# rmcar17/SpectralClusterSupertree

Measured on NVIDIA B200. Metric: construct_supertree wall-time at 10k taxa/1k trees, lower is better.
Workload: dtype f64

## Files before the change

include/scs_b200.h:

```cpp
#ifndef SCS_B200_H
#define SCS_B200_H

#include <stddef.h>
#include <stdint.h>

#ifdef __cplusplus
extern "C" {
#endif

typedef struct scs_ctx scs_ctx;

typedef enum {
    SCS_OK = 0,
    SCS_ERR_INVALID = -1,
    SCS_ERR_CUDA = -2,
    SCS_ERR_NO_DEVICE = -3,
    SCS_ERR_TOO_SMALL = -4,
    SCS_ERR_NO_CONVERGE = -5,
    SCS_ERR_INPUT = -6,
    SCS_ERR_EMPTY = -7,
    SCS_ERR_PEER = -8
} scs_status;

typedef struct {
    int32_t n_components;
    int32_t contracted_size;
    int32_t spectral_ran;
    int32_t solver;
    int32_t matvecs;
    int32_t restarts;
    int32_t tie_flag;
    int32_t kmeans_stable_splits;
    double eig[3];
    double residual;
    double margin;
    double kmeans_runner_up;
} scs_node_stats;

int scs_version(void);
const char *scs_status_string(int status);
const char *scs_last_error(const scs_ctx *ctx);
int scs_ctx_create(int device, void *stream, scs_ctx **out);
int scs_ctx_destroy(scs_ctx *ctx);
int scs_ctx_synchronize(scs_ctx *ctx);
int64_t scs_ctx_launch_count(const scs_ctx *ctx);

int scs_ctx_io_bytes(const scs_ctx *ctx, int64_t *h2d, int64_t *d2h);
int scs_ctx_timer_start(scs_ctx *ctx);
int scs_ctx_timer_stop(scs_ctx *ctx, double *ms);
int scs_ctx_set_small_node_limit(scs_ctx *ctx, int limit);
int scs_ctx_set_medium_node_limit(scs_ctx *ctx, int limit);
int scs_ctx_set_device_forest(scs_ctx *ctx, int on);
int scs_ctx_set_wide_entries(scs_ctx *ctx, int on);
int scs_ctx_set_full_rows(scs_ctx *ctx, int on);
int scs_ctx_stage_seconds(scs_ctx *ctx, double *seconds8, int reset);
int scs_ctx_flush_l2(scs_ctx *ctx);
int scs_ctx_profile_enable(scs_ctx *ctx, int on);
int scs_ctx_profile_read(scs_ctx *ctx, int kind, int64_t *launches, double *ms, double *bytes, double *units);

int scs_debug_small_cycles(scs_ctx *ctx, uint64_t *cycles2, int reset);
int scs_profiler_range(int on);

int scs_bit_words(int n);
int scs_pcg_build_dev(scs_ctx *ctx, int n, int T, int64_t L, const int64_t *leaf_offsets_dev,
                      const int32_t *leaf_taxon_dev, const int32_t *adj_depth_dev,
                      const double *adj_val_dev, const int32_t *root_depth_dev,
                      const double *tree_weight_dev, double *W_dev, int32_t *C_dev,
                      int32_t *occ_dev, uint32_t *adj_bits_dev, uint32_t *max_bits_dev,
                      double *degree_dev);

int scs_pcg_build_rows_dev(scs_ctx *ctx, int n, int T, int64_t L, const int64_t *leaf_offsets_dev,
                           const int32_t *leaf_taxon_dev, const int32_t *adj_depth_dev, const double *adj_val_dev,
                           const int32_t *root_depth_dev, const double *tree_weight_dev, int row0, int row1,
                           double *W_rows_dev, int32_t *occ_dev, uint32_t *adj_bits_dev, uint32_t *max_bits_dev,
                           double *degree_dev);

int scs_components_dev(scs_ctx *ctx, int n, const uint32_t *bits_dev, int32_t *label_dev,
                       int32_t *n_components_host);

int scs_contract_dev(scs_ctx *ctx, int n, const double *W_dev, const uint32_t *adj_bits_dev,
                     const uint32_t *max_bits_dev, int32_t *group_dev, int32_t *m_host,
                     double *Wc_dev, double *degree_c_dev);

int scs_spectral_bipartition_dev(scs_ctx *ctx, int m, const double *W_dev, const double *degree_dev,
                                 uint64_t seed, int32_t *side_dev, scs_node_stats *stats_host);

int scs_normalized_matvec_dev(scs_ctx *ctx, int m, const double *W_dev,
                              const double *inv_sqrt_deg_dev, const double *x_dev, double *y_dev);

int scs_node_split_host(scs_ctx *ctx, int n, int T, int64_t L, const int64_t *leaf_offsets,
                        const int32_t *leaf_taxon, const int32_t *adj_depth, const double *adj_val,
                        const int32_t *root_depth, const double *tree_weight, int contract_edges,
                        uint64_t seed, int32_t *part, scs_node_stats *stats);
int scs_node_split_dev(scs_ctx *ctx, int n, int T, int64_t L, const int64_t *leaf_offsets_dev,
                       const int32_t *leaf_taxon_dev, const int32_t *adj_depth_dev,
                       const double *adj_val_dev, const int32_t *root_depth_dev,
                       const double *tree_weight_dev, int contract_edges, uint64_t seed,
                       int32_t *part_dev, scs_node_stats *stats_host);

int scs_node_last_buffers(scs_ctx *ctx, int *n, int *m, double **W_dev, uint32_t **adj_bits_dev,
                          uint32_t **max_bits_dev, int32_t **occ_dev, double **degree_dev,
                          double **Wc_dev, int32_t **group_dev);

int scs_dev_alloc(scs_ctx *ctx, size_t bytes, void **out);
int scs_dev_free(scs_ctx *ctx, void *ptr);
int scs_memcpy_h2d(scs_ctx *ctx, void *dev, const void *host, size_t bytes);
int scs_memcpy_d2h(scs_ctx *ctx, void *host, const void *dev, size_t bytes);

typedef struct scs_forest scs_forest;
int scs_set_host_threads(int threads);
int scs_forest_create(int T, const int64_t *node_offsets, const int32_t *parent, const double *length,
                      const double *support, const int32_t *taxon, const double *tree_weight,
                      int num_taxa, scs_forest **out);
int scs_forest_create_view(int T, const int64_t *node_offsets, const int32_t *parent, const double *length,
                           const double *support, const int32_t *taxon, const double *tree_weight, int num_taxa,
                           scs_forest **out);
const char *scs_forest_last_error(void);
int scs_forest_destroy(scs_forest *f);
int scs_forest_parse_newick(const char *text, size_t bytes, scs_forest **out, char **names, size_t *names_bytes,
                            int *num_taxa);
const char *scs_newick_last_error(void);
int scs_flat_tree_newick(int64_t num_nodes, const int32_t *parent, const int32_t *taxon, const char *names,
                         size_t names_bytes, int num_taxa, char **text, size_t *text_bytes);
int scs_flat_tree_newick_values(int64_t num_nodes, const int32_t *parent, const int32_t *taxon, const char *names,
                                size_t names_bytes, int num_taxa, const double *value, int digits, char **text,
                                size_t *text_bytes);
void scs_free(void *ptr);
int scs_forest_num_trees(const scs_forest *f);
int64_t scs_forest_num_nodes(const scs_forest *f);
int64_t scs_forest_num_leaves(const scs_forest *f);
int scs_forest_num_taxa(const scs_forest *f);
int64_t scs_forest_pair_visits(const scs_forest *f);
int scs_forest_tree_info(const scs_forest *f, int t, int64_t *num_nodes, double *weight, int32_t *source);
int scs_forest_tree(const scs_forest *f, int t, int32_t *parent, double *length, double *support,
                    int32_t *taxon);
int scs_forest_taxa(const scs_forest *f, uint8_t *present);
int scs_forest_induce(const scs_forest *f, const uint8_t *keep, scs_forest **out);
int scs_forest_induce_parts(const scs_forest *f, const int32_t *part, int count, scs_forest **out,
                            uint8_t *present);
int scs_forest_tours(const scs_forest *f, int weighting, const int32_t *local_id, int64_t *leaf_offsets,
                     int32_t *leaf_taxon, int32_t *adj_depth, double *adj_val, int32_t *root_depth,
                     double *tree_weight);
int scs_forest_split(scs_ctx *ctx, const scs_forest *f, int weighting, int contract_edges, uint64_t seed,
                     int32_t *n_out, int32_t *taxa_out, int32_t *part_out, scs_node_stats *stats);

typedef struct {
    int32_t n;
    int32_t num_trees;
    int64_t leaf_base;
    int64_t tree_base;
    int64_t vertex_base;
} scs_small_node;
int scs_nodes_split_small_host(scs_ctx *ctx, int num_nodes, const scs_small_node *nodes, int64_t L_total,
                               int64_t T_total, const int64_t *leaf_offsets, const int32_t *leaf_taxon,
                               const int32_t *adj_depth, const double *adj_val, const int32_t *root_depth,
                               const double *tree_weight, int contract_edges, int32_t *part,
                               scs_node_stats *stats);

int scs_nodes_split_small_dev(scs_ctx *ctx, int num_nodes, const scs_small_node *nodes_dev,
                              const int64_t *leaf_offsets_dev, const int32_t *leaf_taxon_dev,
                              const int32_t *adj_depth_dev, const double *adj_val_dev,
                              const int32_t *root_depth_dev, const double *tree_weight_dev,
                              int contract_edges, int32_t *part_dev, scs_node_stats *stats_dev);

int scs_nodes_split_medium_dev(scs_ctx *ctx, int num_nodes, const int32_t *node_n, const int32_t *tree_begin,
                               const int64_t *part_offset, const uint64_t *seeds, int T, int64_t L,
                               const int64_t *leaf_offsets_dev, const int32_t *leaf_taxon_dev, const int32_t *adj_depth_dev,
                               const double *adj_val_dev, const int32_t *root_depth_dev, const double *tree_weight_dev,
                               int contract_edges, int32_t *part_dev, scs_node_stats *stats, uint8_t *needs_rerun);

typedef struct scs_supertree scs_supertree;
int scs_supertree_build(scs_ctx *ctx, const scs_forest *forest, int weighting, int contract_edges,
                        uint64_t seed, int record_nodes, scs_supertree **out);
int scs_supertree_build_sharded(scs_ctx *ctx, const scs_forest *forest, int weighting, int contract_edges,
                                uint64_t seed, int record_nodes, int rank, int world, scs_supertree **out);
typedef struct scs_device_forest scs_device_forest;
int scs_device_forest_create(scs_ctx *ctx, const scs_forest *forest, int weighting, scs_device_forest **out);
int scs_device_forest_destroy(scs_device_forest *forest);
int64_t scs_device_forest_bytes(const scs_device_forest *forest);
int scs_supertree_build_resident(scs_ctx *ctx, const scs_device_forest *forest, int contract_edges, uint64_t seed,
                                 int record_nodes, int rank, int world, scs_supertree **out);
int64_t scs_supertree_shared_prefix(const scs_supertree *tree);
int64_t scs_supertree_shared_records(const scs_supertree *tree);
int scs_supertree_wave_info(const scs_supertree *tree, int32_t *tasks, int32_t *max_n);
int scs_supertree_wave_seconds(const scs_supertree *tree, double *seconds3);
int scs_supertree_destroy(scs_supertree *tree);
int64_t scs_supertree_num_nodes(const scs_supertree *tree);
int scs_supertree_nodes(const scs_supertree *tree, int32_t *parent, int32_t *taxon);
int scs_supertree_counters(const scs_supertree *tree, int64_t *nodes_small, int64_t *nodes_large,
                           int64_t *waves, int64_t *pair_visits);
int scs_supertree_seconds(const scs_supertree *tree, double *seconds4);
int scs_supertree_medium_info(const scs_supertree *tree, int64_t *nodes_medium, int64_t *nodes_rerun, double *seconds);
int64_t scs_supertree_num_records(const scs_supertree *tree);
int scs_supertree_record_size(const scs_supertree *tree, int64_t index);
int scs_supertree_record_wave(const scs_supertree *tree, int64_t index);
int scs_supertree_record(const scs_supertree *tree, int64_t index, int32_t *taxa, int32_t *part,
                         scs_node_stats *stats);

int scs_supertree_support(scs_ctx *ctx, const scs_forest *sources, int64_t num_nodes, const int32_t *parent,
                          const int32_t *taxon, int32_t *counts, double *weighted, int32_t *per_tree);

int scs_supertree_triplets(scs_ctx *ctx, const scs_forest *sources, int64_t num_nodes, const int32_t *parent,
                           const int32_t *taxon, int64_t *per_tree);

int scs_supertree_taxon_triplets(scs_ctx *ctx, const scs_forest *sources, int64_t num_nodes, const int32_t *parent,
                                 const int32_t *taxon, int64_t *per_taxon, double *weighted);

#define SCS_IPC_HANDLE_BYTES 64
int scs_shard_create(scs_ctx *ctx, int rank, int world, int n_max, unsigned char *handle_out);
int scs_shard_connect_ipc(scs_ctx *ctx, const unsigned char *handles );
int scs_shard_window(scs_ctx *ctx, void **window_dev, size_t *bytes);
int scs_shard_connect_ptrs(scs_ctx *ctx, void *const *windows );
int scs_shard_engage(scs_ctx *ctx, int on);
int scs_shard_configure(scs_ctx *ctx, int min_n, double timeout_seconds);
int scs_shard_barrier(scs_ctx *ctx);
int64_t scs_shard_nodes(const scs_ctx *ctx);
int scs_shard_destroy(scs_ctx *ctx);

#ifdef __cplusplus
}
#endif
#endif
```

spectralclustersupertree_b200/_lib.py:

```python

from __future__ import annotations

import ctypes
import os
from ctypes import POINTER, c_char_p, c_double, c_int, c_int32, c_int64, c_size_t, c_uint8, c_uint64, c_void_p
from pathlib import Path

LIB_PATH = Path(__file__).resolve().parent / "libscs_b200.so"

SCS_OK = 0
SCS_ERR_INVALID = -1
SCS_ERR_CUDA = -2
SCS_ERR_NO_DEVICE = -3
SCS_ERR_TOO_SMALL = -4
SCS_ERR_NO_CONVERGE = -5
SCS_ERR_INPUT = -6
SCS_ERR_EMPTY = -7
SCS_ERR_PEER = -8
IPC_HANDLE_BYTES = 64


class NodeStats(ctypes.Structure):

    _fields_ = [
        ("n_components", c_int32),
        ("contracted_size", c_int32),
        ("spectral_ran", c_int32),
        ("solver", c_int32),
        ("matvecs", c_int32),
        ("restarts", c_int32),
        ("tie_flag", c_int32),
        ("kmeans_stable_splits", c_int32),
        ("eig", c_double * 3),
        ("residual", c_double),
        ("margin", c_double),
        ("kmeans_runner_up", c_double),
    ]

    def as_dict(self) -> dict:
        return {
            "n_components": self.n_components,
            "contracted_size": self.contracted_size,
            "spectral_ran": bool(self.spectral_ran),
            "solver": self.solver,
            "matvecs": self.matvecs,
            "restarts": self.restarts,
            "tie_flag": self.tie_flag,
            "eig": [self.eig[0], self.eig[1], self.eig[2]],
            "residual": self.residual,
            "margin": self.margin,
            "kmeans_stable_splits": self.kmeans_stable_splits,
            "kmeans_runner_up": self.kmeans_runner_up,
        }


class LibraryMissingError(RuntimeError):
    """``libscs_b200.so`` is not built: the CUDA path is the only path."""


_P = c_void_p

SIGNATURES: dict[str, tuple] = {
    "scs_version": (c_int, []),
    "scs_status_string": (c_char_p, [c_int]),
    "scs_last_error": (c_char_p, [_P]),
    "scs_ctx_create": (c_int, [c_int, _P, POINTER(_P)]),
    "scs_ctx_destroy": (c_int, [_P]),
    "scs_ctx_synchronize": (c_int, [_P]),
    "scs_ctx_launch_count": (c_int64, [_P]),
    "scs_ctx_io_bytes": (c_int, [_P, POINTER(c_int64), POINTER(c_int64)]),
    "scs_ctx_timer_start": (c_int, [_P]),
    "scs_ctx_timer_stop": (c_int, [_P, POINTER(c_double)]),
    "scs_ctx_set_small_node_limit": (c_int, [_P, c_int]),
    "scs_ctx_set_medium_node_limit": (c_int, [_P, c_int]),
    "scs_ctx_set_device_forest": (c_int, [_P, c_int]),
    "scs_ctx_set_wide_entries": (c_int, [_P, c_int]),
    "scs_ctx_set_full_rows": (c_int, [_P, c_int]),
    "scs_ctx_stage_seconds": (c_int, [_P, _P, c_int]),
    "scs_ctx_flush_l2": (c_int, [_P]),
    "scs_ctx_profile_enable": (c_int, [_P, c_int]),
    "scs_ctx_profile_read": (c_int, [_P, c_int, POINTER(c_int64), POINTER(c_double), POINTER(c_double), POINTER(c_double)]),
    "scs_bit_words": (c_int, [c_int]),
    "scs_pcg_build_dev": (c_int, [_P, c_int, c_int, c_int64] + [_P] * 12),
    "scs_pcg_build_rows_dev": (c_int, [_P, c_int, c_int, c_int64, _P, _P, _P, _P, _P, _P, c_int, c_int, _P, _P, _P, _P, _P]),
    "scs_components_dev": (c_int, [_P, c_int, _P, _P, POINTER(c_int32)]),
    "scs_contract_dev": (c_int, [_P, c_int, _P, _P, _P, _P, POINTER(c_int32), _P, _P]),
    "scs_spectral_bipartition_dev": (c_int, [_P, c_int, _P, _P, c_uint64, _P, POINTER(NodeStats)]),
    "scs_normalized_matvec_dev": (c_int, [_P, c_int, _P, _P, _P, _P]),
    "scs_node_split_host": (
        c_int,
        [_P, c_int, c_int, c_int64, _P, _P, _P, _P, _P, _P, c_int, c_uint64, _P, POINTER(NodeStats)],
    ),
    "scs_node_split_dev": (
        c_int,
        [_P, c_int, c_int, c_int64, _P, _P, _P, _P, _P, _P, c_int, c_uint64, _P, POINTER(NodeStats)],
    ),
    "scs_node_last_buffers": (c_int, [_P, POINTER(c_int), POINTER(c_int)] + [POINTER(_P)] * 7),
    "scs_dev_alloc": (c_int, [_P, c_size_t, POINTER(_P)]),
    "scs_dev_free": (c_int, [_P, _P]),
    "scs_memcpy_h2d": (c_int, [_P, _P, _P, c_size_t]),
    "scs_memcpy_d2h": (c_int, [_P, _P, _P, c_size_t]),
    "scs_set_host_threads": (c_int, [c_int]),
    "scs_forest_create": (c_int, [c_int, _P, _P, _P, _P, _P, _P, c_int, POINTER(_P)]),
    "scs_forest_create_view": (c_int, [c_int, _P, _P, _P, _P, _P, _P, c_int, POINTER(_P)]),
    "scs_forest_destroy": (c_int, [_P]),
    "scs_forest_parse_newick": (c_int, [c_char_p, c_size_t, POINTER(_P), POINTER(_P), POINTER(c_size_t), POINTER(c_int)]),
    "scs_newick_last_error": (c_char_p, []),
    "scs_forest_last_error": (c_char_p, []),
    "scs_flat_tree_newick": (c_int, [c_int64, _P, _P, c_char_p, c_size_t, c_int, POINTER(_P), POINTER(c_size_t)]),
    "scs_flat_tree_newick_values": (
        c_int,
        [c_int64, _P, _P, c_char_p, c_size_t, c_int, _P, c_int, POINTER(_P), POINTER(c_size_t)],
    ),
    "scs_supertree_support": (c_int, [_P, _P, c_int64, _P, _P, _P, _P, _P]),
    "scs_supertree_triplets": (c_int, [_P, _P, c_int64, _P, _P, _P]),
    "scs_supertree_taxon_triplets": (c_int, [_P, _P, c_int64, _P, _P, _P, _P]),
    "scs_profiler_range": (c_int, [c_int]),
    "scs_debug_small_cycles": (c_int, [_P, _P, c_int]),
    "scs_free": (None, [_P]),
    "scs_forest_num_trees": (c_int, [_P]),
    "scs_forest_num_nodes": (c_int64, [_P]),
    "scs_forest_num_leaves": (c_int64, [_P]),
    "scs_forest_num_taxa": (c_int, [_P]),
    "scs_forest_pair_visits": (c_int64, [_P]),
    "scs_forest_tree_info": (c_int, [_P, c_int, POINTER(c_int64), POINTER(c_double), POINTER(c_int32)]),
    "scs_forest_tree": (c_int, [_P, c_int, _P, _P, _P, _P]),
    "scs_forest_taxa": (c_int, [_P, _P]),
    "scs_forest_induce": (c_int, [_P, _P, POINTER(_P)]),
    "scs_forest_induce_parts": (c_int, [_P, _P, c_int, _P, _P]),
    "scs_forest_tours": (c_int, [_P, c_int, _P, _P, _P, _P, _P, _P, _P]),
    "scs_forest_split": (
        c_int,
        [_P, _P, c_int, c_int, c_uint64, POINTER(c_int32), _P, _P, POINTER(NodeStats)],
    ),
    "scs_nodes_split_small_host": (
        c_int,
        [_P, c_int, _P, c_int64, c_int64, _P, _P, _P, _P, _P, _P, c_int, _P, _P],
    ),
    "scs_nodes_split_small_dev": (c_int, [_P, c_int, _P, _P, _P, _P, _P, _P, _P, c_int, _P, _P]),
    "scs_supertree_build": (c_int, [_P, _P, c_int, c_int, c_uint64, c_int, POINTER(_P)]),
    "scs_supertree_build_sharded": (c_int, [_P, _P, c_int, c_int, c_uint64, c_int, c_int, c_int, POINTER(_P)]),
    "scs_supertree_shared_prefix": (c_int64, [_P]),
    "scs_supertree_shared_records": (c_int64, [_P]),
    "scs_supertree_wave_info": (c_int, [_P, _P, _P]),
    "scs_supertree_wave_seconds": (c_int, [_P, _P]),
    "scs_supertree_destroy": (c_int, [_P]),
    "scs_supertree_num_nodes": (c_int64, [_P]),
    "scs_supertree_nodes": (c_int, [_P, _P, _P]),
    "scs_supertree_counters": (c_int, [_P, POINTER(c_int64), POINTER(c_int64), POINTER(c_int64), POINTER(c_int64)]),
    "scs_device_forest_create": (c_int, [_P, _P, c_int, POINTER(_P)]),
    "scs_device_forest_destroy": (c_int, [_P]),
    "scs_device_forest_bytes": (c_int64, [_P]),
    "scs_supertree_build_resident": (c_int, [_P, _P, c_int, c_uint64, c_int, c_int, c_int, POINTER(_P)]),
    "scs_supertree_record_wave": (c_int, [_P, c_int64]),
    "scs_nodes_split_medium_dev": (c_int, [_P, c_int, _P, _P, _P, _P, c_int, c_int64, _P, _P, _P, _P, _P, _P, c_int, _P, _P, _P]),
    "scs_supertree_medium_info": (c_int, [_P, POINTER(c_int64), POINTER(c_int64), POINTER(ctypes.c_double)]),
    "scs_supertree_seconds": (c_int, [_P, _P]),
    "scs_supertree_num_records": (c_int64, [_P]),
    "scs_supertree_record_size": (c_int, [_P, c_int64]),
    "scs_supertree_record": (c_int, [_P, c_int64, _P, _P, POINTER(NodeStats)]),
    "scs_shard_create": (c_int, [_P, c_int, c_int, c_int, _P]),
    "scs_shard_connect_ipc": (c_int, [_P, _P]),
    "scs_shard_window": (c_int, [_P, POINTER(_P), POINTER(c_size_t)]),
    "scs_shard_connect_ptrs": (c_int, [_P, _P]),
    "scs_shard_engage": (c_int, [_P, c_int]),
    "scs_shard_configure": (c_int, [_P, c_int, c_double]),
    "scs_shard_barrier": (c_int, [_P]),
    "scs_shard_nodes": (c_int64, [_P]),
    "scs_shard_destroy": (c_int, [_P]),
}

_LIB: ctypes.CDLL | None = None


def load() -> ctypes.CDLL:
    global _LIB
    if _LIB is not None:
        return _LIB
    if not LIB_PATH.is_file():
        msg = (
            f"{LIB_PATH} is missing: build it with `python -m spectralclustersupertree_b200.build` "
            "(there is no CPU fallback for the CUDA path)"
        )
        raise LibraryMissingError(msg)
    os.environ.setdefault("CUDA_MODULE_LOADING", "EAGER")
    os.environ.setdefault("OMP_WAIT_POLICY", "passive")
    lib = ctypes.CDLL(str(LIB_PATH))
    for name, (restype, argtypes) in SIGNATURES.items():
        fn = getattr(lib, name)
        fn.restype = restype
        fn.argtypes = argtypes
    _LIB = lib
    return lib


def ptr(array) -> int | None:
    if array is None:
        return None
    if not array.flags["C_CONTIGUOUS"]:
        msg = "array must be C-contiguous"
        raise ValueError(msg)
    return array.ctypes.data


__all__ = ["LIB_PATH", "SIGNATURES", "LibraryMissingError", "NodeStats", "c_uint8", "load", "ptr"]
```

spectralclustersupertree_b200/csrc/common.cuh:

```cuda
#pragma once

#include <cuda_runtime.h>

#include <cstdint>
#include <cstdio>
#include <cstring>
#include <string>
#include <vector>

#include "scs_b200.h"

namespace scs {

constexpr int kMediumMaxDefault = 4096;

struct DeviceBuffer {
    void *ptr = nullptr;
    size_t bytes = 0;
};

enum Slot : int {
    SLOT_TOUR_OFFSETS = 0,
    SLOT_TOUR_TAXON,
    SLOT_TOUR_DEPTH,
    SLOT_TOUR_VAL,
    SLOT_TOUR_ROOT,
    SLOT_TOUR_WEIGHT,
    SLOT_W,
    SLOT_WC,
    SLOT_OCC,
    SLOT_ADJ_BITS,
    SLOT_MAX_BITS,
    SLOT_DEGREE,
    SLOT_DEGREE_C,
    SLOT_LEAF_TREE,
    SLOT_ROW_PTR,
    SLOT_CURSOR,
    SLOT_INV,
    SLOT_INV_SORTED,
    SLOT_DEGREE_PART,
    SLOT_LINKS,
    SLOT_BUCKET_COUNT,
    SLOT_START16,
    SLOT_BUCKET_PTR,
    SLOT_ENTRIES,
    SLOT_UF_PARENT,
    SLOT_LABEL,
    SLOT_LABEL2,
    SLOT_GROUP,
    SLOT_GROUP_PTR,
    SLOT_GROUP_MEMBERS,
    SLOT_SCALARS,
    SLOT_PART,
    SLOT_ISD,
    SLOT_UVEC,
    SLOT_BASIS,
    SLOT_WORK,
    SLOT_COEF,
    SLOT_TRIDIAG,
    SLOT_RITZ,
    SLOT_EMBED,
    SLOT_SORTED,
    SLOT_SIDE,
    SLOT_SPEC_SCALARS,
    SLOT_L2_FLUSH,
    SLOT_NODE_STATS,
    SLOT_MED_NODES,
    SLOT_MED_ROW_NODE,
    SLOT_MED_TREE_NODE,
    SLOT_MED_STATE,
    SLOT_MED_VEC,
    SLOT_MED_SMALL,
    SLOT_MED_STAGE,
    SLOT_SCAN_SUMS,
    SLOT_COUNT
};

constexpr int kMaxPeers = 16;

struct ShardLayout {
    size_t vec[2] = {0, 0};
    size_t degree = 0, degree_c = 0;
    size_t adj_bits = 0, max_bits = 0;
    size_t W = 0;
    size_t total = 0;
};

struct ShardState {
    bool connected = false;
    bool engaged = false;
    int rank = 0, world = 1;
    int n_max = 0;
    int min_n = 4096;
    unsigned long long epoch = 0;
    int parity = 0;
    double timeout_s = 20.0;
    unsigned char *window = nullptr;
    unsigned char *peer[kMaxPeers] = {};
    bool opened[kMaxPeers] = {};
    ShardLayout layout;
    int64_t nodes = 0;
};

struct RowBlock {
    int row0 = 0, row1 = -1;
    bool half_window = false;
    bool sharded() const { return row1 >= 0; }
};

struct MedNode {
    int32_t n, words;
    int32_t row_base;
    int32_t tree_begin, tree_end;
    int32_t jcap;
    int32_t blk_base, pad0;
    int64_t w_off;
    int64_t bit_off;
    int64_t basis_off;
    int64_t part_off;
    uint64_t seed;
};

inline int shard_rows_per_rank(int n, int world) { return (n + world - 1) / world; }
inline RowBlock shard_block(int n, int rank, int world) {
    const int per = shard_rows_per_rank(n, world);
    RowBlock b;
    b.row0 = rank * per < n ? rank * per : n;
    b.row1 = b.row0 + per < n ? b.row0 + per : n;
    return b;
}

}

struct scs_ctx {
    int device = 0;
    cudaStream_t stream = nullptr;
    bool own_stream = false;
    int sm_count = 148;
    size_t smem_optin = 0;
    size_t smem_per_sm = 0;
    int64_t launches = 0;
    std::string last_error;
    scs::DeviceBuffer slots[scs::SLOT_COUNT];
    void *pinned = nullptr;
    size_t pinned_bytes = 0;
    void *pinned_io = nullptr;
    size_t pinned_io_bytes = 0;
    int64_t h2d_bytes = 0;
    int64_t d2h_bytes = 0;
    bool profile_on = false;
    struct ProfileRecord {
        cudaEvent_t start, stop;
        int kind;
        double bytes, units;
    };
    std::vector<ProfileRecord> profile;
    int flush_value = 0;
    double stage_seconds[8] = {0, 0, 0, 0, 0, 0, 0, 0};
    std::vector<scs_ctx *> workers;
    bool small_configured = false;
    bool batch_configured = false;
    bool tail_configured = false;
    bool rows_configured[32] = {};
    bool mirror_configured = false;
    bool contract_configured = false;
    bool kmeans_configured = false;
    bool medium_configured = false;
    bool device_forest = true;
    int medium_limit = scs::kMediumMaxDefault;
    bool wide_entries = false;
    bool full_rows = false;
    int small_limit = 32;
    double pending_units = 0.0;
    cudaEvent_t timer_start = nullptr, timer_stop = nullptr;
    int last_n = 0;
    int last_m = 0;
    scs::ShardState shard;
    void *driver_cache = nullptr;
    void (*driver_cache_release)(scs_ctx *, void *) = nullptr;
};

namespace scs {

int fail(scs_ctx *ctx, int status, const char *what, cudaError_t err = cudaSuccess);

#define SCS_CUDA(ctx, call)                                                   \
    do {                                                                      \
        cudaError_t err__ = (call);                                           \
        if (err__ != cudaSuccess) return scs::fail(ctx, SCS_ERR_CUDA, #call, err__); \
    } while (0)

#define SCS_LAUNCHED(ctx, name)                                               \
    do {                                                                      \
        cudaError_t err__ = cudaGetLastError();                               \
        if (err__ != cudaSuccess) return scs::fail(ctx, SCS_ERR_CUDA, name, err__); \
        (ctx)->launches += 1;                                                 \
    } while (0)

int reserve(scs_ctx *ctx, Slot slot, size_t bytes, void **out);

template <typename T>
inline int reserve_as(scs_ctx *ctx, Slot slot, size_t count, T **out) {
    void *p = nullptr;
    int rc = reserve(ctx, slot, count * sizeof(T), &p);
    *out = static_cast<T *>(p);
    return rc;
}

int reserve_pinned(scs_ctx *ctx, size_t bytes, void **out);

enum ProfileKind : int { PROFILE_MATVEC = 0, PROFILE_PCG_ROWS = 1, PROFILE_KINDS = 2 };
constexpr int kSmallNode = 64;
constexpr int kSmallMaxTrees = 65535;
constexpr int kProfileMinSize = 4096;

void profile_begin(scs_ctx *ctx, int kind, double bytes, double units);
void profile_end(scs_ctx *ctx);

inline int ceil_div(int64_t a, int64_t b) { return static_cast<int>((a + b - 1) / b); }

int exclusive_scan(scs_ctx *ctx, int n, const int32_t *in, int32_t *out);

#ifdef __CUDACC__
__device__ __forceinline__ unsigned long long order_key(double x) {
    const unsigned long long sign = 0x8000000000000000ull;
    unsigned long long b = static_cast<unsigned long long>(__double_as_longlong(x));
    return (b & sign) ? ~b : (b | sign);
}
__device__ __forceinline__ double order_value(unsigned long long k) {
    const unsigned long long sign = 0x8000000000000000ull;
    unsigned long long b = (k & sign) ? (k & ~sign) : ~k;
    return __longlong_as_double(static_cast<long long>(b));
}
#endif

int prewarm_node(scs_ctx *ctx, int n, int T, int64_t L);

int ensure_workers(scs_ctx *ctx, int count);

int pcg_build(scs_ctx *ctx, int n, int T, int64_t L, const int64_t *leaf_offsets,
              const int32_t *leaf_taxon, const int32_t *adj_depth, const double *adj_val,
              const int32_t *root_depth, const double *tree_weight, double *W, int32_t *C,
              int32_t *occ, uint32_t *adj_bits, uint32_t *max_bits, double *degree, RowBlock rows = RowBlock());

int pcg_fetch_transposed(scs_ctx *ctx, int n, RowBlock rows, int rows_per_rank, int world, const double *const *peer_W,
                         double *W_block);
int pcg_symmetrize_bits(scs_ctx *ctx, int n, uint32_t *adj_bits, uint32_t *max_bits);
int pcg_degree_block(scs_ctx *ctx, int n, int T, RowBlock rows, const double *W_block, double *degree);

int components(scs_ctx *ctx, int n, const uint32_t *bits, int32_t *label, int32_t *n_components_host);

int components_async(scs_ctx *ctx, int n, const uint32_t *bits, int32_t *label, int32_t *count_dev);

int tour_components_async(scs_ctx *ctx, int n, int T, int64_t L, const int64_t *leaf_offsets,
                          const int32_t *leaf_taxon, const int32_t *adj_depth, const int32_t *root_depth,
                          int32_t *label, int32_t *count_dev, int32_t *bad_dev);

int contract(scs_ctx *ctx, int n, const double *W, const uint32_t *adj_bits, const uint32_t *max_bits,
             int32_t *group, int32_t *m_host, double *Wc, double *degree_c);
int contract_with_labels(scs_ctx *ctx, int n, const double *W, const uint32_t *adj_bits, const int32_t *label, int m,
                         int32_t *group, double *Wc, double *degree_c, RowBlock rows = RowBlock());

int spectral_bipartition(scs_ctx *ctx, int m, const double *W, const double *degree, uint64_t seed,
                         int32_t *side, scs_node_stats *stats_host, RowBlock rows = RowBlock());

int normalized_matvec(scs_ctx *ctx, int m, const double *W, const double *isd, const double *x, double *y);

int pcg_build_batch(scs_ctx *ctx, int B, int blocks, int R, int T, int64_t L, int max_n, int max_trees, const MedNode *nodes_dev,
                    const int32_t *tree_node, const int32_t *row_node, const int64_t *leaf_offsets,
                    const int32_t *leaf_taxon, const int32_t *adj_depth, const double *adj_val,
                    const int32_t *root_depth, const double *tree_weight, double *W, int32_t *occ, uint32_t *adj_bits,
                    uint32_t *max_bits, double *degree, int32_t *bad_dev);

constexpr int kMediumMax = kMediumMaxDefault;

int medium_batch(scs_ctx *ctx, int B, const int32_t *node_n, const int32_t *tree_begin, const int32_t *tree_end,
                 const int64_t *part_off, const uint64_t *seeds, int T, int64_t L, const int64_t *leaf_offsets, const int32_t *leaf_taxon,
                 const int32_t *adj_depth, const double *adj_val, const int32_t *root_depth, const double *tree_weight,
                 int contract_edges, int32_t *part_dev, scs_node_stats *stats_host, uint8_t *needs_rerun);

int small_node(scs_ctx *ctx, int n, int contract_edges, const double *W, const uint32_t *adj_bits,
               const uint32_t *max_bits, int32_t *part, scs_node_stats *out_dev, int32_t *group_out,
               double *Wc_out);

int small_batch(scs_ctx *ctx, int num_nodes, const scs_small_node *nodes_dev, const int64_t *leaf_offsets,
                const int32_t *leaf_taxon, const int32_t *adj_depth, const double *adj_val, const int32_t *root_depth,
                const double *tree_weight, int contract_edges, int32_t *part_dev, scs_node_stats *stats_dev,
                int32_t *bad_dev, int absolute_offsets = 0);

int small_cycles(scs_ctx *ctx, unsigned long long *out2, int reset);

int node_split(scs_ctx *ctx, int n, int T, int64_t L, const int64_t *leaf_offsets, const int32_t *leaf_taxon,
               const int32_t *adj_depth, const double *adj_val, const int32_t *root_depth,
               const double *tree_weight, int contract_edges, uint64_t seed, int32_t *part_dev,
               int32_t *part_host, scs_node_stats *stats, bool tour_components = false);

int node_split_host(scs_ctx *ctx, int n, int T, int64_t L, const int64_t *leaf_offsets, const int32_t *leaf_taxon,
                    const int32_t *adj_depth, const double *adj_val, const int32_t *root_depth,
                    const double *tree_weight, int contract_edges, uint64_t seed, int32_t *part,
                    scs_node_stats *stats_out, bool tour_components);

bool shard_applies(const scs_ctx *ctx, int n);
int shard_barrier(scs_ctx *ctx);
int shard_push(scs_ctx *ctx, size_t offset, size_t bytes);
struct ShardMatvecTicket {
    unsigned long long epoch;
    size_t vec_offset;
    unsigned long long timeout_ns;
};
ShardMatvecTicket shard_next_matvec(scs_ctx *ctx);
int node_split_sharded(scs_ctx *ctx, int n, int T, int64_t L, const int64_t *leaf_offsets, const int32_t *leaf_taxon,
                       const int32_t *adj_depth, const double *adj_val, const int32_t *root_depth,
                       const double *tree_weight, int contract_edges, uint64_t seed, int32_t *part_dev,
                       int32_t *part_host, scs_node_stats *stats);

}
```

spectralclustersupertree_b200/csrc/context.cu:

```cuda

#include "common.cuh"

#include <chrono>
#include <cmath>

#include <cuda_profiler_api.h>

namespace scs {

int fail(scs_ctx *ctx, int status, const char *what, cudaError_t err) {
    if (ctx) {
        ctx->last_error = what ? what : "";
        if (err != cudaSuccess) {
            ctx->last_error += ": ";
            ctx->last_error += cudaGetErrorString(err);
        }
    }
    return status;
}

int reserve(scs_ctx *ctx, Slot slot, size_t bytes, void **out) {
    DeviceBuffer &buf = ctx->slots[slot];
    if (bytes == 0) bytes = 16;
    if (buf.bytes < bytes) {
        const size_t want = bytes + bytes / 4 + 256;
        if (buf.ptr) {
            SCS_CUDA(ctx, cudaFreeAsync(buf.ptr, ctx->stream));
            buf.ptr = nullptr;
            buf.bytes = 0;
        }
        cudaError_t err = cudaMallocAsync(&buf.ptr, want, ctx->stream);
        if (err != cudaSuccess) {
            buf.ptr = nullptr;
            return fail(ctx, SCS_ERR_CUDA, "cudaMallocAsync (workspace)", err);
        }
        buf.bytes = want;
    }
    *out = buf.ptr;
    return SCS_OK;
}

int reserve_pinned(scs_ctx *ctx, size_t bytes, void **out) {
    if (ctx->pinned_bytes < bytes) {
        if (ctx->pinned) {
            SCS_CUDA(ctx, cudaStreamSynchronize(ctx->stream));
            SCS_CUDA(ctx, cudaFreeHost(ctx->pinned));
            ctx->pinned = nullptr;
            ctx->pinned_bytes = 0;
        }
        size_t want = bytes < 4096 ? 4096 : 2 * bytes;
        SCS_CUDA(ctx, cudaMallocHost(&ctx->pinned, want));
        ctx->pinned_bytes = want;
    }
    *out = ctx->pinned;
    return SCS_OK;
}

int ensure_workers(scs_ctx *ctx, int count) {
    while (static_cast<int>(ctx->workers.size()) < count - 1) {
        scs_ctx *worker = nullptr;
        const int rc = scs_ctx_create(ctx->device, nullptr, &worker);
        if (rc) return fail(ctx, rc, "creating a worker context");
        worker->small_limit = ctx->small_limit;
        ctx->workers.push_back(worker);
    }
    for (scs_ctx *worker : ctx->workers) {
        worker->small_limit = ctx->small_limit;
        worker->full_rows = ctx->full_rows;
        worker->wide_entries = ctx->wide_entries;
    }
    return SCS_OK;
}

void profile_begin(scs_ctx *ctx, int kind, double bytes, double units) {
    if (!ctx->profile_on) return;
    scs_ctx::ProfileRecord rec;
    rec.kind = kind;
    rec.bytes = bytes;
    rec.units = units;
    if (cudaEventCreate(&rec.start) != cudaSuccess || cudaEventCreate(&rec.stop) != cudaSuccess) return;
    cudaEventRecord(rec.start, ctx->stream);
    ctx->profile.push_back(rec);
}

void profile_end(scs_ctx *ctx) {
    if (!ctx->profile_on || ctx->profile.empty()) return;
    cudaEventRecord(ctx->profile.back().stop, ctx->stream);
}

namespace {

struct DeviceGuard {
    int previous = -1;
    explicit DeviceGuard(int device) {
        cudaGetDevice(&previous);
        if (previous != device) cudaSetDevice(device);
    }
};

template <typename T>
int upload(scs_ctx *ctx, Slot slot, const T *host, size_t count, T **dev) {
    int rc = reserve_as(ctx, slot, count + 1, dev);
    if (rc) return rc;
    if (count) SCS_CUDA(ctx, cudaMemcpyAsync(*dev, host, count * sizeof(T), cudaMemcpyHostToDevice, ctx->stream));
    return SCS_OK;
}

__global__ void relabel_components(int n, const int32_t *__restrict__ label, const int32_t *__restrict__ rank,
                                   int32_t *__restrict__ part) {
    int v = blockIdx.x * blockDim.x + threadIdx.x;
    if (v < n) part[v] = rank[label[v]];
}

__global__ void mark_roots(int n, const int32_t *__restrict__ label, int32_t *__restrict__ flag) {
    int v = blockIdx.x * blockDim.x + threadIdx.x;
    if (v < n) flag[v] = label[v] == v;
}

__global__ void expand_sides(int n, const int32_t *__restrict__ group, const int32_t *__restrict__ side,
                             int32_t *__restrict__ part) {
    int v = blockIdx.x * blockDim.x + threadIdx.x;
    if (v < n) part[v] = side[group ? group[v] : v];
}

void clear_stats(scs_node_stats *s) {
    std::memset(s, 0, sizeof(*s));
    s->eig[0] = 0.0;
    s->eig[1] = s->eig[2] = std::nan("");
    s->residual = std::nan("");
    s->margin = std::nan("");
}

}

int node_split(scs_ctx *ctx, int n, int T, int64_t L, const int64_t *leaf_offsets, const int32_t *leaf_taxon,
               const int32_t *adj_depth, const double *adj_val, const int32_t *root_depth,
               const double *tree_weight, int contract_edges, uint64_t seed, int32_t *part_dev,
               int32_t *part_host, scs_node_stats *stats, bool tour_components) {
    auto number_components = [&](const int32_t *label) -> int {
        int32_t *flag, *rank;
        int rc;
        if ((rc = reserve_as(ctx, SLOT_GROUP_PTR, 4 * static_cast<size_t>(n) + 8, &flag))) return rc;
        rank = flag + n;
        const int blocks = ceil_div(n, 256);
        mark_roots<<<blocks, 256, 0, ctx->stream>>>(n, label, flag);
        SCS_LAUNCHED(ctx, "mark_roots");
        if ((rc = exclusive_scan(ctx, n, flag, rank))) return rc;
        relabel_components<<<blocks, 256, 0, ctx->stream>>>(n, label, rank, part_dev);
        SCS_LAUNCHED(ctx, "relabel_components");
        if (part_host) {
            SCS_CUDA(ctx, cudaMemcpyAsync(part_host, part_dev, sizeof(int32_t) * n, cudaMemcpyDeviceToHost, ctx->stream));
            ctx->d2h_bytes += static_cast<int64_t>(sizeof(int32_t)) * n;
            SCS_CUDA(ctx, cudaStreamSynchronize(ctx->stream));
        }
        return SCS_OK;
    };
    if (tour_components && n > ctx->small_limit) {
        const auto t0 = std::chrono::steady_clock::now();
        int32_t *label, *scalars;
        void *pin_v;
        int rc;
        if ((rc = reserve_as(ctx, SLOT_LABEL, static_cast<size_t>(n), &label))) return rc;
        if ((rc = reserve_as(ctx, SLOT_SCALARS, 64, &scalars))) return rc;
        if ((rc = reserve_pinned(ctx, 512, &pin_v))) return rc;
        SCS_CUDA(ctx, cudaMemsetAsync(scalars, 0, 16 * sizeof(int32_t), ctx->stream));
        if ((rc = tour_components_async(ctx, n, T, L, leaf_offsets, leaf_taxon, adj_depth, root_depth, label,
                                        scalars + 8, scalars)))
            return rc;
        int32_t *host_scalars = reinterpret_cast<int32_t *>(static_cast<unsigned char *>(pin_v) + 256);
        SCS_CUDA(ctx, cudaMemcpyAsync(host_scalars, scalars, 16 * sizeof(int32_t), cudaMemcpyDeviceToHost, ctx->stream));
        SCS_CUDA(ctx, cudaStreamSynchronize(ctx->stream));
        ctx->stage_seconds[6] += std::chrono::duration<double>(std::chrono::steady_clock::now() - t0).count();
        if (host_scalars[0] != 0) return fail(ctx, SCS_ERR_INPUT, "leaf tour: taxon id out of range");
        if (host_scalars[8] != 1) {
            stats->n_components = host_scalars[8];
            stats->contracted_size = n;
            return number_components(label);
        }
    }
    if (shard_applies(ctx, n))
        return node_split_sharded(ctx, n, T, L, leaf_offsets, leaf_taxon, adj_depth, adj_val, root_depth, tree_weight,
                                  contract_edges, seed, part_dev, part_host, stats);
    const int words = scs_bit_words(n);
    const size_t nn = static_cast<size_t>(n) * n;
    double *W, *Wc, *degree, *degree_c;
    int32_t *occ, *label, *group, *side, *scalars;
    uint32_t *adj_bits, *max_bits;
    int rc;
    if ((rc = reserve_as(ctx, SLOT_W, nn, &W))) return rc;
    if ((rc = reserve_as(ctx, SLOT_OCC, static_cast<size_t>(n), &occ))) return rc;
    if ((rc = reserve_as(ctx, SLOT_ADJ_BITS, static_cast<size_t>(n) * words, &adj_bits))) return rc;
    if ((rc = reserve_as(ctx, SLOT_MAX_BITS, static_cast<size_t>(n) * words, &max_bits))) return rc;
    if ((rc = reserve_as(ctx, SLOT_DEGREE, static_cast<size_t>(n), &degree))) return rc;
    if ((rc = reserve_as(ctx, SLOT_LABEL, static_cast<size_t>(n), &label))) return rc;
    if ((rc = reserve_as(ctx, SLOT_SCALARS, 64, &scalars))) return rc;
    ctx->last_n = n;
    ctx->last_m = 0;
    void *pin_v;
    if ((rc = reserve_pinned(ctx, 512, &pin_v))) return rc;
    unsigned char *pin = static_cast<unsigned char *>(pin_v);
    auto fetch_part = [&]() -> int {
        if (part_host) {
            SCS_CUDA(ctx, cudaMemcpyAsync(part_host, part_dev, sizeof(int32_t) * n, cudaMemcpyDeviceToHost, ctx->stream));
            ctx->d2h_bytes += static_cast<int64_t>(sizeof(int32_t)) * n;
        }
        return SCS_OK;
    };

    auto now = [] { return std::chrono::steady_clock::now(); };
    auto lap = [&](int slot, std::chrono::steady_clock::time_point &since) {
        const auto t = now();
        ctx->stage_seconds[slot] += std::chrono::duration<double>(t - since).count();
        since = t;
    };
    auto mark = now();
    if ((rc = pcg_build(ctx, n, T, L, leaf_offsets, leaf_taxon, adj_depth, adj_val, root_depth, tree_weight, W,
                        nullptr, occ, adj_bits, contract_edges ? max_bits : nullptr, degree)))
        return rc;

    if (n <= ctx->small_limit) {
        scs_node_stats *stats_dev;
        if ((rc = reserve_as(ctx, SLOT_NODE_STATS, 1, &stats_dev))) return rc;
        if ((rc = reserve_as(ctx, SLOT_WC, nn, &Wc))) return rc;
        if ((rc = reserve_as(ctx, SLOT_GROUP, static_cast<size_t>(n), &group))) return rc;
        if ((rc = small_node(ctx, n, contract_edges, W, adj_bits, max_bits, part_dev, stats_dev, group, Wc))) return rc;
        SCS_CUDA(ctx, cudaMemcpyAsync(pin, stats_dev, sizeof(scs_node_stats), cudaMemcpyDeviceToHost, ctx->stream));
        SCS_CUDA(ctx, cudaMemcpyAsync(pin + 256, scalars, sizeof(int32_t), cudaMemcpyDeviceToHost, ctx->stream));
        if ((rc = fetch_part())) return rc;
        SCS_CUDA(ctx, cudaStreamSynchronize(ctx->stream));
        if (*reinterpret_cast<int32_t *>(pin + 256) != 0)
            return fail(ctx, SCS_ERR_INPUT, "leaf tour: taxon id out of range");
        std::memcpy(stats, pin, sizeof(scs_node_stats));
        ctx->last_m = stats->contracted_size;
        if (stats->solver == -1) {
            stats->solver = 0;
            return fail(ctx, SCS_ERR_TOO_SMALL, "spectral step on a graph contracted to one vertex");
        }
        return SCS_OK;
    }

    int32_t *label2 = nullptr;
    if ((rc = components_async(ctx, n, adj_bits, label, scalars + 8))) return rc;
    if (contract_edges) {
        if ((rc = reserve_as(ctx, SLOT_LABEL2, static_cast<size_t>(n), &label2))) return rc;
        if ((rc = components_async(ctx, n, max_bits, label2, scalars + 9))) return rc;
    }
    SCS_CUDA(ctx, cudaMemcpyAsync(pin + 256, scalars, 16 * sizeof(int32_t), cudaMemcpyDeviceToHost, ctx->stream));
    lap(0, mark);
    SCS_CUDA(ctx, cudaStreamSynchronize(ctx->stream));
    lap(1, mark);
    const int32_t *host_scalars = reinterpret_cast<const int32_t *>(pin + 256);
    if (host_scalars[0] != 0) return fail(ctx, SCS_ERR_INPUT, "leaf tour: taxon id out of range");
    const int ncomp = host_scalars[8];
    stats->n_components = ncomp;
    stats->contracted_size = n;
    const int blocks = ceil_div(n, 256);

    if (ncomp != 1) return number_components(label);

    int m = n;
    const double *Wm = W;
    const double *deg_m = degree;
    const int32_t *group_m = nullptr;
    if (contract_edges) {
        m = host_scalars[9];
        if ((rc = reserve_as(ctx, SLOT_WC, nn, &Wc))) return rc;
        if ((rc = reserve_as(ctx, SLOT_DEGREE_C, static_cast<size_t>(n), &degree_c))) return rc;
        if ((rc = reserve_as(ctx, SLOT_GROUP, static_cast<size_t>(n), &group))) return rc;
        if ((rc = contract_with_labels(ctx, n, W, adj_bits, label2, m, group, Wc, degree_c))) return rc;
        if (m != n) {
            Wm = Wc;
            deg_m = degree_c;
            group_m = group;
        }
    }
    ctx->last_m = m;
    stats->contracted_size = m;
    stats->spectral_ran = 1;
    if ((rc = reserve_as(ctx, SLOT_SIDE, static_cast<size_t>(n), &side))) return rc;
    if (m < 2) {
        return fail(ctx, SCS_ERR_TOO_SMALL, "spectral step on a graph contracted to one vertex");
    }
    lap(2, mark);
    if ((rc = spectral_bipartition(ctx, m, Wm, deg_m, seed, side, stats))) return rc;
    lap(3, mark);
    expand_sides<<<blocks, 256, 0, ctx->stream>>>(n, group_m, side, part_dev);
    SCS_LAUNCHED(ctx, "expand_sides");
    if ((rc = fetch_part())) return rc;
    if (part_host) SCS_CUDA(ctx, cudaStreamSynchronize(ctx->stream));
    lap(4, mark);
    return SCS_OK;
}

}

using namespace scs;

namespace scs {
int prewarm_node(scs_ctx *ctx, int n, int T, int64_t L) {
    DeviceGuard guard(ctx->device);
    const size_t nT = static_cast<size_t>(T), nL = static_cast<size_t>(L), nn = static_cast<size_t>(n) * n;
    const size_t total = (nT + 1) * sizeof(int64_t) + nL * (sizeof(double) + 2 * sizeof(int32_t)) +
                         nT * (sizeof(double) + sizeof(int32_t)) + 64;
    if (ctx->pinned_io_bytes < total) {
        if (ctx->pinned_io) {
            SCS_CUDA(ctx, cudaStreamSynchronize(ctx->stream));
            SCS_CUDA(ctx, cudaFreeHost(ctx->pinned_io));
            ctx->pinned_io = nullptr;
            ctx->pinned_io_bytes = 0;
        }
        const size_t want = 2 * total + 4096;
        SCS_CUDA(ctx, cudaMallocHost(&ctx->pinned_io, want));
        ctx->pinned_io_bytes = want;
    }
    const size_t words = static_cast<size_t>(scs_bit_words(n));
    const size_t basis = static_cast<size_t>((n - 1 < 256 ? n - 1 : 256) + 3) * n;
    void *p;
    int rc;
    if ((rc = reserve(ctx, SLOT_TOUR_OFFSETS, total, &p))) return rc;
    if ((rc = reserve(ctx, SLOT_W, 8 * nn, &p))) return rc;
    if ((rc = reserve(ctx, SLOT_WC, 8 * nn, &p))) return rc;
    if ((rc = reserve(ctx, SLOT_ADJ_BITS, 4 * n * words, &p))) return rc;
    if ((rc = reserve(ctx, SLOT_MAX_BITS, 4 * n * words, &p))) return rc;
    if ((rc = reserve(ctx, SLOT_BASIS, 8 * basis, &p))) return rc;
    if ((rc = reserve(ctx, SLOT_LINKS, 16 * (nL + 1), &p))) return rc;
    if ((rc = reserve(ctx, SLOT_ENTRIES, 8 * (nL + 1), &p))) return rc;
    if ((rc = reserve(ctx, SLOT_BUCKET_COUNT, 448 * (nL + 1), &p))) return rc;
    if ((rc = reserve(ctx, SLOT_START16, 64 * (nL + 1), &p))) return rc;
    return SCS_OK;
}
}

namespace scs {
int node_split_host(scs_ctx *ctx, int n, int T, int64_t L, const int64_t *leaf_offsets, const int32_t *leaf_taxon,
                    const int32_t *adj_depth, const double *adj_val, const int32_t *root_depth,
                    const double *tree_weight, int contract_edges, uint64_t seed, int32_t *part,
                    scs_node_stats *stats_out, bool tour_components) {
    if (!ctx) return SCS_ERR_INVALID;
    if (n <= 0 || T < 0 || L < 0 || !part) return fail(ctx, SCS_ERR_INVALID, "node_split: bad argument");
    if (T > 0 && (!leaf_offsets || !root_depth || !tree_weight))
        return fail(ctx, SCS_ERR_INVALID, "node_split: null tour array");
    if (L > 0 && (!leaf_taxon || !adj_depth || !adj_val))
        return fail(ctx, SCS_ERR_INVALID, "node_split: null tour array");
    DeviceGuard guard(ctx->device);
    scs_node_stats local;
    scs_node_stats *stats = stats_out ? stats_out : &local;
    clear_stats(stats);

    const size_t nT = static_cast<size_t>(T), nL = static_cast<size_t>(L);
    const size_t b_off = (nT + 1) * sizeof(int64_t);
    const size_t b_val = nL * sizeof(double);
    const size_t b_w = nT * sizeof(double);
    const size_t b_tax = nL * sizeof(int32_t);
    const size_t b_dep = nL * sizeof(int32_t);
    const size_t b_root = nT * sizeof(int32_t);
    const size_t total = b_off + b_val + b_w + b_tax + b_dep + b_root + 64;
    int rc;
    if (ctx->pinned_io_bytes < total) {
        if (ctx->pinned_io) {
            SCS_CUDA(ctx, cudaStreamSynchronize(ctx->stream));
            SCS_CUDA(ctx, cudaFreeHost(ctx->pinned_io));
            ctx->pinned_io = nullptr;
            ctx->pinned_io_bytes = 0;
        }
        const size_t want = 2 * total + 4096;
        SCS_CUDA(ctx, cudaMallocHost(&ctx->pinned_io, want));
        ctx->pinned_io_bytes = want;
    }
    unsigned char *stage = static_cast<unsigned char *>(ctx->pinned_io);
    unsigned char *dev_stage;
    if ((rc = reserve_as(ctx, SLOT_TOUR_OFFSETS, total, &dev_stage))) return rc;
    size_t o_off = 0, o_val = o_off + b_off, o_w = o_val + b_val, o_tax = o_w + b_w, o_dep = o_tax + b_tax,
           o_root = o_dep + b_dep;
    if (T > 0) {
        std::memcpy(stage + o_off, leaf_offsets, b_off);
        std::memcpy(stage + o_w, tree_weight, b_w);
        std::memcpy(stage + o_root, root_depth, b_root);
    } else {
        std::memset(stage + o_off, 0, b_off);
    }
    if (L > 0) {
        std::memcpy(stage + o_val, adj_val, b_val);
        std::memcpy(stage + o_tax, leaf_taxon, b_tax);
        std::memcpy(stage + o_dep, adj_depth, b_dep);
    }
    SCS_CUDA(ctx, cudaMemcpyAsync(dev_stage, stage, total - 64, cudaMemcpyHostToDevice, ctx->stream));
    ctx->h2d_bytes += static_cast<int64_t>(total - 64);
    ctx->pending_units = 0.0;
    for (int t = 0; t < T; ++t) {
        const double k = static_cast<double>(leaf_offsets[t + 1] - leaf_offsets[t]);
        ctx->pending_units += k * (k - 1.0);
    }

    int32_t *part_dev;
    if ((rc = reserve_as(ctx, SLOT_PART, static_cast<size_t>(n), &part_dev))) return rc;
    rc = node_split(ctx, n, T, L, reinterpret_cast<const int64_t *>(dev_stage + o_off),
                    reinterpret_cast<const int32_t *>(dev_stage + o_tax),
                    reinterpret_cast<const int32_t *>(dev_stage + o_dep),
                    reinterpret_cast<const double *>(dev_stage + o_val),
                    reinterpret_cast<const int32_t *>(dev_stage + o_root),
                    reinterpret_cast<const double *>(dev_stage + o_w), contract_edges, seed, part_dev, part, stats,
                    tour_components);
    ctx->pending_units = 0.0;
    return rc;
}
}

extern "C" {

int scs_version(void) { return 100; }

const char *scs_status_string(int status) {
    switch (status) {
    case SCS_OK: return "ok";
    case SCS_ERR_INVALID: return "invalid argument";
    case SCS_ERR_CUDA: return "CUDA error";
    case SCS_ERR_NO_DEVICE: return "no usable CUDA device";
    case SCS_ERR_TOO_SMALL: return "fewer than two vertices in the spectral step";
    case SCS_ERR_NO_CONVERGE: return "eigensolver did not converge";
    case SCS_ERR_INPUT: return "malformed input";
    case SCS_ERR_EMPTY: return "there must be at least one tree to make a supertree";
    case SCS_ERR_PEER: return "a wait for a peer GPU timed out";
    default: return "unknown status";
    }
}

const char *scs_last_error(const scs_ctx *ctx) { return ctx ? ctx->last_error.c_str() : ""; }

int scs_bit_words(int n) { return (n + 31) / 32; }

int scs_ctx_create(int device, void *stream, scs_ctx **out) {
    if (!out) return SCS_ERR_INVALID;
    *out = nullptr;
    int count = 0;
    if (cudaGetDeviceCount(&count) != cudaSuccess || count <= 0) {
        cudaGetLastError();
        return SCS_ERR_NO_DEVICE;
    }
    if (device < 0 || device >= count) return SCS_ERR_INVALID;
    if (cudaSetDevice(device) != cudaSuccess) return SCS_ERR_CUDA;
    scs_ctx *ctx = new scs_ctx();
    ctx->device = device;
    cudaDeviceProp prop;
    if (cudaGetDeviceProperties(&prop, device) != cudaSuccess) {
        delete ctx;
        return SCS_ERR_CUDA;
    }
    {
        cudaMemPool_t pool;
        if (cudaDeviceGetDefaultMemPool(&pool, device) == cudaSuccess) {
            uint64_t threshold = ~0ull;
            cudaMemPoolSetAttribute(pool, cudaMemPoolAttrReleaseThreshold, &threshold);
        }
        cudaGetLastError();
    }
    ctx->sm_count = prop.multiProcessorCount;
    ctx->smem_optin = prop.sharedMemPerBlockOptin;
    ctx->smem_per_sm = prop.sharedMemPerMultiprocessor;
    if (stream) {
        ctx->stream = static_cast<cudaStream_t>(stream);
    } else {
        if (cudaStreamCreateWithFlags(&ctx->stream, cudaStreamNonBlocking) != cudaSuccess) {
            delete ctx;
            return SCS_ERR_CUDA;
        }
        ctx->own_stream = true;
    }
    *out = ctx;
    return SCS_OK;
}

int scs_ctx_destroy(scs_ctx *ctx) {
    if (!ctx) return SCS_OK;
    DeviceGuard guard(ctx->device);
    for (scs_ctx *worker : ctx->workers) scs_ctx_destroy(worker);
    ctx->workers.clear();
    cudaStreamSynchronize(ctx->stream);
    if (ctx->driver_cache && ctx->driver_cache_release) ctx->driver_cache_release(ctx, ctx->driver_cache);
    ctx->driver_cache = nullptr;
    scs_shard_destroy(ctx);
    for (auto &buf : ctx->slots)
        if (buf.ptr) cudaFreeAsync(buf.ptr, ctx->stream);
    cudaStreamSynchronize(ctx->stream);
    if (ctx->pinned) cudaFreeHost(ctx->pinned);
    if (ctx->pinned_io) cudaFreeHost(ctx->pinned_io);
    for (auto &rec : ctx->profile) {
        cudaEventDestroy(rec.start);
        cudaEventDestroy(rec.stop);
    }
    if (ctx->timer_start) cudaEventDestroy(ctx->timer_start);
    if (ctx->timer_stop) cudaEventDestroy(ctx->timer_stop);
    if (ctx->own_stream) cudaStreamDestroy(ctx->stream);
    delete ctx;
    return SCS_OK;
}

int scs_ctx_synchronize(scs_ctx *ctx) {
    if (!ctx) return SCS_ERR_INVALID;
    DeviceGuard guard(ctx->device);
    SCS_CUDA(ctx, cudaStreamSynchronize(ctx->stream));
    return SCS_OK;
}

int64_t scs_ctx_launch_count(const scs_ctx *ctx) { return ctx ? ctx->launches : 0; }

int scs_ctx_io_bytes(const scs_ctx *ctx, int64_t *h2d, int64_t *d2h) {
    if (!ctx) return SCS_ERR_INVALID;
    if (h2d) *h2d = ctx->h2d_bytes;
    if (d2h) *d2h = ctx->d2h_bytes;
    return SCS_OK;
}

int scs_ctx_timer_start(scs_ctx *ctx) {
    if (!ctx) return SCS_ERR_INVALID;
    DeviceGuard guard(ctx->device);
    if (!ctx->timer_start) {
        SCS_CUDA(ctx, cudaEventCreate(&ctx->timer_start));
        SCS_CUDA(ctx, cudaEventCreate(&ctx->timer_stop));
    }
    SCS_CUDA(ctx, cudaEventRecord(ctx->timer_start, ctx->stream));
    return SCS_OK;
}

int scs_ctx_timer_stop(scs_ctx *ctx, double *ms) {
    if (!ctx || !ms || !ctx->timer_start) return SCS_ERR_INVALID;
    DeviceGuard guard(ctx->device);
    SCS_CUDA(ctx, cudaEventRecord(ctx->timer_stop, ctx->stream));
    SCS_CUDA(ctx, cudaEventSynchronize(ctx->timer_stop));
    float t = 0.0f;
    SCS_CUDA(ctx, cudaEventElapsedTime(&t, ctx->timer_start, ctx->timer_stop));
    *ms = t;
    return SCS_OK;
}

int scs_ctx_set_small_node_limit(scs_ctx *ctx, int limit) {
    if (!ctx || limit < 0) return SCS_ERR_INVALID;
    ctx->small_limit = limit > kSmallNode ? kSmallNode : limit;
    return SCS_OK;
}

int scs_ctx_set_medium_node_limit(scs_ctx *ctx, int limit) {
    if (!ctx || limit < 0) return SCS_ERR_INVALID;
    ctx->medium_limit = limit > kMediumMax ? kMediumMax : limit;
    return SCS_OK;
}

int scs_ctx_set_device_forest(scs_ctx *ctx, int on) {
    if (!ctx) return SCS_ERR_INVALID;
    ctx->device_forest = on != 0;
    return SCS_OK;
}

int scs_ctx_set_wide_entries(scs_ctx *ctx, int on) {
    if (!ctx) return SCS_ERR_INVALID;
    ctx->wide_entries = on != 0;
    return SCS_OK;
}

int scs_ctx_set_full_rows(scs_ctx *ctx, int on) {
    if (!ctx) return SCS_ERR_INVALID;
    ctx->full_rows = on != 0;
    for (scs_ctx *worker : ctx->workers) worker->full_rows = ctx->full_rows;
    return SCS_OK;
}

int scs_ctx_stage_seconds(scs_ctx *ctx, double *seconds8, int reset) {
    if (!ctx || !seconds8) return SCS_ERR_INVALID;
    for (int i = 0; i < 8; ++i) {
        seconds8[i] = ctx->stage_seconds[i];
        if (reset) ctx->stage_seconds[i] = 0.0;
    }
    return SCS_OK;
}

int scs_ctx_flush_l2(scs_ctx *ctx) {
    if (!ctx) return SCS_ERR_INVALID;
    DeviceGuard guard(ctx->device);
    const size_t bytes = 256u << 20;
    void *buf;
    int rc = reserve(ctx, SLOT_L2_FLUSH, bytes, &buf);
    if (rc) return rc;
    ctx->flush_value += 1;
    SCS_CUDA(ctx, cudaMemsetAsync(buf, ctx->flush_value & 0xff, bytes, ctx->stream));
    SCS_CUDA(ctx, cudaStreamSynchronize(ctx->stream));
    return SCS_OK;
}

int scs_ctx_profile_enable(scs_ctx *ctx, int on) {
    if (!ctx) return SCS_ERR_INVALID;
    ctx->profile_on = on != 0;
    return SCS_OK;
}

int scs_ctx_profile_read(scs_ctx *ctx, int kind, int64_t *launches, double *ms, double *bytes, double *units) {
    if (!ctx || kind < 0 || kind >= PROFILE_KINDS) return SCS_ERR_INVALID;
    DeviceGuard guard(ctx->device);
    SCS_CUDA(ctx, cudaStreamSynchronize(ctx->stream));
    int64_t count = 0;
    double total_ms = 0.0, total_bytes = 0.0, total_units = 0.0;
    std::vector<scs_ctx::ProfileRecord> keep;
    for (auto &rec : ctx->profile) {
        if (rec.kind != kind) {
            keep.push_back(rec);
            continue;
        }
        float t = 0.0f;
        if (cudaEventElapsedTime(&t, rec.start, rec.stop) == cudaSuccess) {
            count += 1;
            total_ms += t;
            total_bytes += rec.bytes;
            total_units += rec.units;
        }
        cudaEventDestroy(rec.start);
        cudaEventDestroy(rec.stop);
    }
    cudaGetLastError();
    ctx->profile.swap(keep);
    if (launches) *launches = count;
    if (ms) *ms = total_ms;
    if (bytes) *bytes = total_bytes;
    if (units) *units = total_units;
    return SCS_OK;
}

int scs_debug_small_cycles(scs_ctx *ctx, uint64_t *cycles2, int reset) {
    if (!ctx || !cycles2) return SCS_ERR_INVALID;
    DeviceGuard guard(ctx->device);
    unsigned long long raw[2] = {0, 0};
    const int rc = small_cycles(ctx, raw, reset);
    cycles2[0] = raw[0];
    cycles2[1] = raw[1];
    return rc;
}

int scs_profiler_range(int on) {
    const cudaError_t err = on ? cudaProfilerStart() : cudaProfilerStop();
    return err == cudaSuccess ? SCS_OK : SCS_ERR_CUDA;
}

int scs_pcg_build_dev(scs_ctx *ctx, int n, int T, int64_t L, const int64_t *leaf_offsets_dev,
                      const int32_t *leaf_taxon_dev, const int32_t *adj_depth_dev, const double *adj_val_dev,
                      const int32_t *root_depth_dev, const double *tree_weight_dev, double *W_dev, int32_t *C_dev,
                      int32_t *occ_dev, uint32_t *adj_bits_dev, uint32_t *max_bits_dev, double *degree_dev) {
    if (!ctx) return SCS_ERR_INVALID;
    DeviceGuard guard(ctx->device);
    return pcg_build(ctx, n, T, L, leaf_offsets_dev, leaf_taxon_dev, adj_depth_dev, adj_val_dev, root_depth_dev,
                     tree_weight_dev, W_dev, C_dev, occ_dev, adj_bits_dev, max_bits_dev, degree_dev);
}

int scs_pcg_build_rows_dev(scs_ctx *ctx, int n, int T, int64_t L, const int64_t *leaf_offsets_dev,
                           const int32_t *leaf_taxon_dev, const int32_t *adj_depth_dev, const double *adj_val_dev,
                           const int32_t *root_depth_dev, const double *tree_weight_dev, int row0, int row1,
                           double *W_rows_dev, int32_t *occ_dev, uint32_t *adj_bits_dev, uint32_t *max_bits_dev,
                           double *degree_dev) {
    if (!ctx) return SCS_ERR_INVALID;
    DeviceGuard guard(ctx->device);
    RowBlock rows;
    rows.row0 = row0;
    rows.row1 = row1;
    return pcg_build(ctx, n, T, L, leaf_offsets_dev, leaf_taxon_dev, adj_depth_dev, adj_val_dev, root_depth_dev,
                     tree_weight_dev, W_rows_dev, nullptr, occ_dev, adj_bits_dev, max_bits_dev, degree_dev, rows);
}

int scs_components_dev(scs_ctx *ctx, int n, const uint32_t *bits_dev, int32_t *label_dev,
                       int32_t *n_components_host) {
    if (!ctx) return SCS_ERR_INVALID;
    DeviceGuard guard(ctx->device);
    return components(ctx, n, bits_dev, label_dev, n_components_host);
}

int scs_contract_dev(scs_ctx *ctx, int n, const double *W_dev, const uint32_t *adj_bits_dev,
                     const uint32_t *max_bits_dev, int32_t *group_dev, int32_t *m_host, double *Wc_dev,
                     double *degree_c_dev) {
    if (!ctx) return SCS_ERR_INVALID;
    DeviceGuard guard(ctx->device);
    return contract(ctx, n, W_dev, adj_bits_dev, max_bits_dev, group_dev, m_host, Wc_dev, degree_c_dev);
}

int scs_spectral_bipartition_dev(scs_ctx *ctx, int m, const double *W_dev, const double *degree_dev,
                                 uint64_t seed, int32_t *side_dev, scs_node_stats *stats_host) {
    if (!ctx) return SCS_ERR_INVALID;
    DeviceGuard guard(ctx->device);
    scs_node_stats local;
    scs_node_stats *stats = stats_host ? stats_host : &local;
    clear_stats(stats);
    stats->n_components = 1;
    stats->contracted_size = m;
    stats->spectral_ran = 1;
    if (m < 2) return fail(ctx, SCS_ERR_TOO_SMALL, "spectral step needs at least two vertices");
    return spectral_bipartition(ctx, m, W_dev, degree_dev, seed, side_dev, stats);
}

int scs_normalized_matvec_dev(scs_ctx *ctx, int m, const double *W_dev, const double *inv_sqrt_deg_dev,
                              const double *x_dev, double *y_dev) {
    if (!ctx) return SCS_ERR_INVALID;
    DeviceGuard guard(ctx->device);
    return normalized_matvec(ctx, m, W_dev, inv_sqrt_deg_dev, x_dev, y_dev);
}

int scs_node_split_dev(scs_ctx *ctx, int n, int T, int64_t L, const int64_t *leaf_offsets_dev,
                       const int32_t *leaf_taxon_dev, const int32_t *adj_depth_dev, const double *adj_val_dev,
                       const int32_t *root_depth_dev, const double *tree_weight_dev, int contract_edges,
                       uint64_t seed, int32_t *part_dev, scs_node_stats *stats_host) {
    if (!ctx || n <= 0 || !part_dev) return SCS_ERR_INVALID;
    DeviceGuard guard(ctx->device);
    scs_node_stats local;
    scs_node_stats *stats = stats_host ? stats_host : &local;
    clear_stats(stats);
    return node_split(ctx, n, T, L, leaf_offsets_dev, leaf_taxon_dev, adj_depth_dev, adj_val_dev, root_depth_dev,
                      tree_weight_dev, contract_edges, seed, part_dev, nullptr, stats);
}

int scs_node_split_host(scs_ctx *ctx, int n, int T, int64_t L, const int64_t *leaf_offsets,
                        const int32_t *leaf_taxon, const int32_t *adj_depth, const double *adj_val,
                        const int32_t *root_depth, const double *tree_weight, int contract_edges, uint64_t seed,
                        int32_t *part, scs_node_stats *stats_out) {
    return node_split_host(ctx, n, T, L, leaf_offsets, leaf_taxon, adj_depth, adj_val, root_depth, tree_weight,
                           contract_edges, seed, part, stats_out, false);
}

int scs_node_last_buffers(scs_ctx *ctx, int *n, int *m, double **W_dev, uint32_t **adj_bits_dev,
                          uint32_t **max_bits_dev, int32_t **occ_dev, double **degree_dev, double **Wc_dev,
                          int32_t **group_dev) {
    if (!ctx) return SCS_ERR_INVALID;
    if (n) *n = ctx->last_n;
    if (m) *m = ctx->last_m;
    if (W_dev) *W_dev = static_cast<double *>(ctx->slots[SLOT_W].ptr);
    if (adj_bits_dev) *adj_bits_dev = static_cast<uint32_t *>(ctx->slots[SLOT_ADJ_BITS].ptr);
    if (max_bits_dev) *max_bits_dev = static_cast<uint32_t *>(ctx->slots[SLOT_MAX_BITS].ptr);
    if (occ_dev) *occ_dev = static_cast<int32_t *>(ctx->slots[SLOT_OCC].ptr);
    if (degree_dev) *degree_dev = static_cast<double *>(ctx->slots[SLOT_DEGREE].ptr);
    if (Wc_dev) *Wc_dev = static_cast<double *>(ctx->slots[SLOT_WC].ptr);
    if (group_dev) *group_dev = static_cast<int32_t *>(ctx->slots[SLOT_GROUP].ptr);
    return SCS_OK;
}

int scs_memcpy_d2h(scs_ctx *ctx, void *host, const void *dev, size_t bytes) {
    if (!ctx || !host || !dev) return SCS_ERR_INVALID;
    DeviceGuard guard(ctx->device);
    SCS_CUDA(ctx, cudaMemcpyAsync(host, dev, bytes, cudaMemcpyDeviceToHost, ctx->stream));
    SCS_CUDA(ctx, cudaStreamSynchronize(ctx->stream));
    return SCS_OK;
}

int scs_memcpy_h2d(scs_ctx *ctx, void *dev, const void *host, size_t bytes) {
    if (!ctx || !host || !dev) return SCS_ERR_INVALID;
    DeviceGuard guard(ctx->device);
    SCS_CUDA(ctx, cudaMemcpyAsync(dev, host, bytes, cudaMemcpyHostToDevice, ctx->stream));
    SCS_CUDA(ctx, cudaStreamSynchronize(ctx->stream));
    return SCS_OK;
}

int scs_dev_alloc(scs_ctx *ctx, size_t bytes, void **out) {
    if (!ctx || !out) return SCS_ERR_INVALID;
    DeviceGuard guard(ctx->device);
    SCS_CUDA(ctx, cudaMalloc(out, bytes ? bytes : 16));
    return SCS_OK;
}

int scs_dev_free(scs_ctx *ctx, void *ptr) {
    if (!ctx) return SCS_ERR_INVALID;
    DeviceGuard guard(ctx->device);
    SCS_CUDA(ctx, cudaStreamSynchronize(ctx->stream));
    SCS_CUDA(ctx, cudaFree(ptr));
    return SCS_OK;
}

}
```

spectralclustersupertree_b200/csrc/medium.cu:

```cuda

#include "common.cuh"
#include "spectral_dev.cuh"
#include "uf.cuh"

#include <algorithm>
#include <vector>

namespace scs {

namespace {

using namespace specdev;

enum MedMode : int32_t { MED_DISCONNECTED = 0, MED_TOO_SMALL = 1, MED_PAIR = 2, MED_LANCZOS = 3 };
enum MedOutcome : int32_t { MED_RUNNING = 0, MED_CONVERGED = 1, MED_INVARIANT = 2, MED_OUT_OF_STEPS = 3 };

struct MedState {
    int32_t ncomp[2];
    int32_t giant[2];
    int32_t m;
    int32_t mode;
    int32_t jmax;
    int32_t outcome;
    int32_t lanczos[4];
    int32_t bad_degree;
    int32_t pad[3];
};

constexpr int kScalarStride = 3 * (kMaxBasis + 8) + 32;

struct MedBuffers {
    const MedNode *nodes;
    MedState *state;
    const int32_t *row_node;
    double *W, *Wc;
    uint32_t *adj_bits, *max_bits;
    int32_t *occ;
    double *degree, *degree_c;
    int32_t *uf_parent, *label[2];
    int32_t *group, *gptr, *members;
    double *isd, *z, *y, *yvec, *wstart, *embed;
    double *basis, *scalars;
    int32_t *side;
    int32_t *remaining;
};

__device__ __forceinline__ double *node_alpha(const MedBuffers &mb, int b) { return mb.scalars + static_cast<size_t>(b) * kScalarStride; }
__device__ __forceinline__ double *node_beta(const MedBuffers &mb, int b) { return node_alpha(mb, b) + (kMaxBasis + 8); }
__device__ __forceinline__ double *node_coef(const MedBuffers &mb, int b) { return node_alpha(mb, b) + 2 * (kMaxBasis + 8); }
__device__ __forceinline__ double *node_ritz(const MedBuffers &mb, int b) { return node_alpha(mb, b) + 3 * (kMaxBasis + 8); }

__global__ void med_fill_maps(int B, int R, int T, const MedNode *__restrict__ nodes, int32_t *__restrict__ row_node,
                              int32_t *__restrict__ tree_node) {
    const int i = blockIdx.x * blockDim.x + threadIdx.x;
    if (i < R) {
        int lo = 0, hi = B;
        while (hi - lo > 1) {
            const int mid = (lo + hi) >> 1;
            if (nodes[mid].row_base <= i) lo = mid; else hi = mid;
        }
        row_node[i] = lo;
    }
    if (i < T) {
        int lo = 0, hi = B;
        while (hi - lo > 1) {
            const int mid = (lo + hi) >> 1;
            if (nodes[mid].tree_begin <= i) lo = mid; else hi = mid;
        }
        tree_node[i] = (i >= nodes[lo].tree_begin && i < nodes[lo].tree_end) ? lo : -1;
    }
}

__global__ void med_clear_state(int B, MedState *state, int32_t *remaining) {
    const int b = blockIdx.x * blockDim.x + threadIdx.x;
    if (b == 0) *remaining = 0;
    if (b >= B) return;
    MedState s;
    memset(&s, 0, sizeof(s));
    state[b] = s;
}

__global__ void med_uf_init(int R, int32_t *parent) {
    const int i = blockIdx.x * blockDim.x + threadIdx.x;
    if (i < R) parent[i] = i;
}

constexpr int kSample = 2;
__global__ void med_uf_hook_sample(int R, const MedNode *__restrict__ nodes, const int32_t *__restrict__ row_node,
                                   const uint32_t *__restrict__ bits, int32_t *parent) {
    const int r = (blockIdx.x * blockDim.x + threadIdx.x) >> 5;
    const int lane = threadIdx.x & 31;
    if (r >= R) return;
    const MedNode &nd = nodes[row_node[r]];
    const int base = nd.row_base, n = nd.n, words = nd.words;
    const int a = r - base;
    const uint32_t *row = bits + nd.bit_off + static_cast<size_t>(a) * words;
    int found = 0;
    for (int j0 = 0; j0 < words && found < kSample; j0 += 32) {
        const int j = j0 + lane;
        uint32_t wbits = j < words ? row[j] : 0u;
        if (j == (a >> 5)) wbits &= ~(1u << (a & 31));
        unsigned active = __ballot_sync(0xffffffffu, wbits != 0u);
        while (active && found < kSample) {
            const int src = __ffs(active) - 1;
            uint32_t wsrc = __shfl_sync(0xffffffffu, wbits, src);
            while (wsrc && found < kSample) {
                const int b = ((j0 + src) << 5) + __ffs(wsrc) - 1;
                wsrc &= wsrc - 1;
                if (b < n) {
                    if (lane == 0) uf_union(parent, r, base + b);
                    ++found;
                }
            }
            active &= active - 1;
        }
    }
}

__global__ void med_uf_snapshot(int R, int32_t *parent, int32_t *snapshot) {
    const int i = blockIdx.x * blockDim.x + threadIdx.x;
    if (i >= R) return;
    int r = i;
    while (parent[r] != r) r = parent[r];
    snapshot[i] = r;
}

__global__ void __launch_bounds__(1024)
med_uf_pick_giant(const MedNode *__restrict__ nodes, const int32_t *__restrict__ snapshot, MedState *state, int which) {
    __shared__ int32_t roots[1024];
    __shared__ int best_count[32];
    __shared__ int32_t best_root[32];
    const MedNode &nd = nodes[blockIdx.x];
    const int n = nd.n, tid = threadIdx.x;
    const int samples = n < 1024 ? n : 1024;
    const int32_t mine = tid < samples ? snapshot[nd.row_base + static_cast<int64_t>(tid) * n / samples] : -1;
    roots[tid] = mine;
    __syncthreads();
    int count = 0;
    if (mine >= 0)
        for (int i = 0; i < samples; ++i) count += roots[i] == mine;
    int32_t root = mine;
    for (int off = 16; off > 0; off >>= 1) {
        const int oc = __shfl_down_sync(0xffffffffu, count, off);
        const int32_t orr = __shfl_down_sync(0xffffffffu, root, off);
        if (oc > count || (oc == count && orr >= 0 && (root < 0 || orr < root))) { count = oc; root = orr; }
    }
    if ((tid & 31) == 0) { best_count[tid >> 5] = count; best_root[tid >> 5] = root; }
    __syncthreads();
    if (tid == 0) {
        int bc = best_count[0];
        int32_t br = best_root[0];
        for (int w = 1; w < 32; ++w)
            if (best_count[w] > bc || (best_count[w] == bc && best_root[w] >= 0 && (br < 0 || best_root[w] < br))) {
                bc = best_count[w];
                br = best_root[w];
            }
        state[blockIdx.x].giant[which] = br;
    }
}

__global__ void med_uf_hook_rest(int R, const MedNode *__restrict__ nodes, const int32_t *__restrict__ row_node,
                                 const uint32_t *__restrict__ bits, const int32_t *__restrict__ snapshot,
                                 const MedState *__restrict__ state, int which, int32_t *parent) {
    const int r = (blockIdx.x * blockDim.x + threadIdx.x) >> 5;
    const int lane = threadIdx.x & 31;
    if (r >= R) return;
    const int b_node = row_node[r];
    if (snapshot[r] == state[b_node].giant[which]) return;
    const MedNode &nd = nodes[b_node];
    const int base = nd.row_base, n = nd.n, words = nd.words;
    const int a = r - base;
    const uint32_t *row = bits + nd.bit_off + static_cast<size_t>(a) * words;
    for (int j = lane; j < words; j += 32) {
        uint32_t wbits = row[j];
        const int first = j << 5;
        if (j == (a >> 5)) wbits &= ~(1u << (a & 31));
        while (wbits) {
            const int b = first + __ffs(wbits) - 1;
            wbits &= wbits - 1;
            if (b < n) uf_union(parent, r, base + b);
        }
    }
}

__global__ void med_uf_flatten(int R, const int32_t *__restrict__ row_node, int32_t *parent, int32_t *label,
                               MedState *state, int which) {
    const int i = blockIdx.x * blockDim.x + threadIdx.x;
    if (i >= R) return;
    int r = i;
    while (parent[r] != r) r = parent[r];
    label[i] = r;
    if (r == i) atomicAdd(&state[row_node[i]].ncomp[which], 1);
}

__global__ void med_decide(int B, int contract_edges, const MedNode *__restrict__ nodes, MedState *state,
                           int32_t *remaining) {
    const int b = blockIdx.x * blockDim.x + threadIdx.x;
    if (b >= B) return;
    MedState &s = state[b];
    const int n = nodes[b].n;
    const int m = contract_edges ? s.ncomp[1] : n;
    s.m = m;
    s.outcome = MED_RUNNING;
    s.lanczos[0] = s.lanczos[1] = s.lanczos[2] = s.lanczos[3] = 0;
    if (s.ncomp[0] != 1) s.mode = MED_DISCONNECTED;
    else if (m < 2) s.mode = MED_TOO_SMALL;
    else if (m == 2) s.mode = MED_PAIR;
    else {
        s.mode = MED_LANCZOS;
        s.jmax = min(m - 1, nodes[b].jcap);
        atomicAdd(remaining, 1);
    }
}

__device__ void rank_representatives(int n, int base, const int32_t *__restrict__ label, int32_t *rank_s, int32_t *warp_part,
                                     int *total_out) {
    const int tid = threadIdx.x, lane = tid & 31, warp = tid >> 5;
    int32_t v[4];
#pragma unroll
    for (int k = 0; k < 4; ++k) {
        const int i = 4 * tid + k;
        v[k] = i < n ? (label[base + i] == base + i) : 0;
    }
    const int32_t mine = v[0] + v[1] + v[2] + v[3];
    int32_t inc = mine;
    for (int off = 1; off < 32; off <<= 1) {
        const int32_t o = __shfl_up_sync(0xffffffffu, inc, off);
        if (lane >= off) inc += o;
    }
    __syncthreads();
    if (lane == 31) warp_part[warp] = inc;
    __syncthreads();
    if (warp == 0) {
        int32_t w = warp_part[lane];
        for (int off = 1; off < 32; off <<= 1) {
            const int32_t o = __shfl_up_sync(0xffffffffu, w, off);
            if (lane >= off) w += o;
        }
        warp_part[lane] = w;
    }
    __syncthreads();
    int32_t run = (warp ? warp_part[warp - 1] : 0) + inc - mine;
#pragma unroll
    for (int k = 0; k < 4; ++k) {
        const int i = 4 * tid + k;
        if (i < n) rank_s[i] = run;
        run += v[k];
    }
    if (tid == 0) *total_out = warp_part[31];
    __syncthreads();
}

__global__ void __launch_bounds__(1024)
med_ranks(int contract_edges, MedBuffers mb, int32_t *__restrict__ part) {
    extern __shared__ int32_t rank_s[];
    __shared__ int32_t warp_part[32];
    __shared__ int total;
    const int b = blockIdx.x;
    const MedNode &nd = mb.nodes[b];
    const MedState &st = mb.state[b];
    const int n = nd.n, base = nd.row_base, tid = threadIdx.x;
    if (st.mode == MED_DISCONNECTED) {
        rank_representatives(n, base, mb.label[0], rank_s, warp_part, &total);
        for (int v = tid; v < n; v += 1024) part[nd.part_off + v] = rank_s[mb.label[0][base + v] - base];
        return;
    }
    if (!contract_edges || st.m == n) {
        for (int v = tid; v < n; v += 1024) mb.group[base + v] = v;
        return;
    }
    rank_representatives(n, base, mb.label[1], rank_s, warp_part, &total);
    int32_t *count_s = rank_s + n;
    for (int v = tid; v < n; v += 1024) count_s[v] = 0;
    __syncthreads();
    for (int v = tid; v < n; v += 1024) {
        const int g = rank_s[mb.label[1][base + v] - base];
        mb.group[base + v] = g;
        atomicAdd(&count_s[g], 1);
    }
    __syncthreads();
    const int m = st.m;
    int32_t *gptr = mb.gptr + base + b;
    if (tid < 32) {
        int32_t carry = 0;
        for (int g0 = 0; g0 < m; g0 += 32) {
            const int g = g0 + tid;
            const int32_t c = g < m ? count_s[g] : 0;
            int32_t inc = c;
            for (int off = 1; off < 32; off <<= 1) {
                const int32_t o = __shfl_up_sync(0xffffffffu, inc, off);
                if (tid >= off) inc += o;
            }
            if (g < m) gptr[g] = carry + inc - c;
            carry += __shfl_sync(0xffffffffu, inc, 31);
        }
        if (tid == 0) gptr[m] = carry;
    }
    __syncthreads();
    for (int v = tid; v < n; v += 1024) count_s[v] = 0;
    __syncthreads();
    for (int v = tid; v < n; v += 1024) {
        const int g = mb.group[base + v];
        mb.members[base + gptr[g] + atomicAdd(&count_s[g], 1)] = v;
    }
}

__global__ void __launch_bounds__(256)
med_contract_rows(MedBuffers mb) {
    extern __shared__ __align__(16) unsigned char smem_raw[];
    unsigned long long *best = reinterpret_cast<unsigned long long *>(smem_raw);
    __shared__ double warp_part[8];
    const int r = blockIdx.x;
    const int b = mb.row_node[r];
    const MedState &st = mb.state[b];
    const MedNode &nd = mb.nodes[b];
    const int n = nd.n, m = st.m, base = nd.row_base;
    const int A = r - base;
    if (st.mode != MED_LANCZOS || m == n || A >= m) return;
    const int tid = threadIdx.x;
    for (int c = tid; c < m; c += 256) best[c] = 0ull;
    __syncthreads();
    const int32_t *gptr = mb.gptr + base + b;
    const int32_t *group = mb.group + base;
    const double *W = mb.W + nd.w_off;
    const uint32_t *bits = mb.adj_bits + nd.bit_off;
    for (int mi = gptr[A]; mi < gptr[A + 1]; ++mi) {
        const int u = mb.members[base + mi];
        const uint32_t *bits_u = bits + static_cast<size_t>(u) * nd.words;
        const double *W_u = W + static_cast<size_t>(u) * n;
        for (int v = tid; v < n; v += 256) {
            if ((bits_u[v >> 5] >> (v & 31)) & 1u) {
                const int Bv = group[v];
                if (Bv != A) atomicMax(&best[Bv], order_key(W_u[v]));
            }
        }
    }
    __syncthreads();
    double partial = 0.0;
    double *out = mb.Wc + nd.w_off + static_cast<size_t>(A) * m;
    for (int c = tid; c < m; c += 256) {
        const unsigned long long k = best[c];
        const double x = k ? order_value(k) : 0.0;
        out[c] = x;
        partial += x;
    }
#pragma unroll
    for (int off = 16; off > 0; off >>= 1) partial += __shfl_down_sync(0xffffffffu, partial, off);
    if ((tid & 31) == 0) warp_part[tid >> 5] = partial;
    __syncthreads();
    if (tid == 0) {
        double s = 0.0;
        for (int wi = 0; wi < 8; ++wi) s += warp_part[wi];
        mb.degree_c[base + A] = s;
    }
}

__device__ __forceinline__ const double *node_matrix(const MedBuffers &mb, const MedNode &nd, const MedState &st) {
    return (st.m == nd.n ? mb.W : mb.Wc) + nd.w_off;
}

__global__ void __launch_bounds__(kOneCta)
med_prepare(MedBuffers mb) {
    const int b = blockIdx.x;
    const MedNode &nd = mb.nodes[b];
    MedState &st = mb.state[b];
    if (st.mode != MED_LANCZOS) return;
    const int m = st.m, base = nd.row_base;
    const double *degree = (m == nd.n ? mb.degree : mb.degree_c) + base;
    double *basis = mb.basis + nd.basis_off;
    prepare_scaling_body(m, degree, mb.isd + base, basis, &st.bad_degree);
    double *w = mb.wstart + base;
    for (int i = threadIdx.x; i < m; i += kOneCta) {
        const uint64_t r = splitmix64(nd.seed * 0xD1342543DE82EF95ull + static_cast<uint64_t>(i) + 1ull);
        w[i] = 2.0 * (static_cast<double>(r >> 11) * (1.0 / 9007199254740992.0)) - 1.0;
    }
    __syncthreads();
    lanczos_tail_body(m, 0, 1, 0, 0, basis, w, mb.isd + base, node_alpha(mb, b), node_beta(mb, b), basis + m, mb.z + base,
                      st.lanczos, node_coef(mb, b), node_ritz(mb, b));
}

__global__ void __launch_bounds__(kMvThreads)
med_matvec(int R, int final, MedBuffers mb) {
    const int r = (blockIdx.x * kMvThreads + threadIdx.x) >> 5;
    const int lane = threadIdx.x & 31;
    if (r >= R) return;
    const int b = mb.row_node[r];
    const MedState &st = mb.state[b];
    if (st.mode != MED_LANCZOS || (!final && st.lanczos[1])) return;
    const MedNode &nd = mb.nodes[b];
    const int m = st.m, base = nd.row_base;
    const int A = r - base;
    if (A >= m) return;
    const double *Wm = node_matrix(mb, nd, st);
    double acc = row_dot_partial(Wm + static_cast<size_t>(A) * m, mb.z + base, m, lane, 32);
    acc = warp_sum(acc);
    if (lane == 0) mb.y[r] = mb.isd[r] * acc;
}

__global__ void __launch_bounds__(kOneCta)
med_tail(int j, MedBuffers mb) {
    const int b = blockIdx.x;
    const MedNode &nd = mb.nodes[b];
    MedState &st = mb.state[b];
    if (st.mode != MED_LANCZOS || st.lanczos[1] || j > st.jmax) return;
    const int m = st.m, base = nd.row_base;
    const int check = (j == st.jmax) || (j % 4) == 0;
    double *basis = mb.basis + nd.basis_off;
    double *ritz = node_ritz(mb, b);
    lanczos_tail_body(m, j, 1 + j, j, check, basis, mb.y + base, mb.isd + base, node_alpha(mb, b), node_beta(mb, b),
                      basis + static_cast<size_t>(j + 1) * m, mb.z + base, st.lanczos, node_coef(mb, b), ritz);
    if (threadIdx.x == 0) {
        if (st.lanczos[1]) {
            st.outcome = ritz[3] <= kBreakdown ? MED_INVARIANT : MED_CONVERGED;
            atomicSub(mb.remaining, 1);
        } else if (j == st.jmax) {
            st.outcome = MED_OUT_OF_STEPS;
            st.lanczos[1] = 1;
            st.lanczos[2] = j;
            atomicSub(mb.remaining, 1);
        }
    }
}

__global__ void __launch_bounds__(kOneCta)
med_ritz_vector(MedBuffers mb) {
    const int b = blockIdx.x;
    const MedNode &nd = mb.nodes[b];
    const MedState &st = mb.state[b];
    if (st.mode != MED_LANCZOS) return;
    const int base = nd.row_base;
    const int jdone = static_cast<int>(node_ritz(mb, b)[5]);
    ritz_vector_body(st.m, jdone, mb.basis + nd.basis_off, node_coef(mb, b), mb.isd + base, mb.yvec + base, mb.z + base);
}

__global__ void __launch_bounds__(kOneCta)
med_finish(MedBuffers mb, int32_t *__restrict__ part, scs_node_stats *__restrict__ stats) {
    const int b = blockIdx.x;
    const MedNode &nd = mb.nodes[b];
    const MedState &st = mb.state[b];
    const int n = nd.n, m = st.m, base = nd.row_base, tid = threadIdx.x;
    const double nan_v = __longlong_as_double(0x7ff8000000000000ll);
    scs_node_stats out;
    out.n_components = st.ncomp[0];
    out.contracted_size = st.mode == MED_DISCONNECTED ? n : m;
    out.spectral_ran = st.mode != MED_DISCONNECTED;
    out.solver = 0;
    out.matvecs = 0;
    out.restarts = 0;
    out.tie_flag = 0;
    out.kmeans_stable_splits = 0;
    out.eig[0] = 0.0;
    out.eig[1] = out.eig[2] = nan_v;
    out.residual = nan_v;
    out.margin = nan_v;
    out.kmeans_runner_up = 0.0;
    if (st.mode == MED_DISCONNECTED) {
        if (tid == 0) stats[b] = out;
        return;
    }
    if (st.mode == MED_TOO_SMALL) {
        out.solver = -1;
        if (tid == 0) stats[b] = out;
        return;
    }
    const int32_t *group = mb.group + base;
    if (st.mode == MED_PAIR) {
        for (int v = tid; v < n; v += kOneCta) part[nd.part_off + v] = group[v];
        out.solver = 1;
        out.eig[1] = 2.0;
        out.residual = 0.0;
        out.margin = 0.5;
        if (tid == 0) stats[b] = out;
        return;
    }
    double *ritz = node_ritz(mb, b);
    true_residual_body(m, mb.yvec + base, mb.y + base, ritz, ritz + 8);
    const int P = 1 << (32 - __clz(max(m - 1, 1)));
    two_means_1d_body<true>(m, P, mb.yvec + base, mb.isd + base, mb.embed + base, nullptr, mb.side + base, ritz + 12);
    __syncthreads();
    for (int v = tid; v < n; v += kOneCta) part[nd.part_off + v] = mb.side[base + group[v]];
    if (tid == 0) {
        const double theta1 = ritz[0], theta2 = ritz[1];
        const int steps = static_cast<int>(ritz[4]);
        out.solver = 3;
        out.matvecs = st.lanczos[2] + 1;
        out.eig[1] = 1.0 - theta1;
        out.eig[2] = 1.0 - theta2;
        out.residual = ritz[8];
        out.margin = ritz[12];
        out.kmeans_stable_splits = static_cast<int32_t>(ritz[16]);
        out.kmeans_runner_up = ritz[17];
        int flag = 0;
        if (!isnan(theta2) && (theta1 - theta2) < kGapTie) flag |= 1;
        if (!(out.margin >= kMarginTie)) flag |= 2;
        if (st.bad_degree) flag |= 8;
        if (out.kmeans_stable_splits > 1) flag |= 16;
        out.tie_flag = flag;
        if (st.outcome == MED_OUT_OF_STEPS || (st.outcome == MED_INVARIANT && steps < m - 1)) out.solver = -3;
        stats[b] = out;
    }
}

template <typename T>
int carve(unsigned char *&cursor, size_t count, T **out) {
    const size_t bytes = (count * sizeof(T) + 255) & ~static_cast<size_t>(255);
    *out = reinterpret_cast<T *>(cursor);
    cursor += bytes;
    return 0;
}

}

int medium_batch(scs_ctx *ctx, int B, const int32_t *node_n, const int32_t *tree_begin, const int32_t *tree_end,
                 const int64_t *part_off, const uint64_t *seeds, int T, int64_t L, const int64_t *leaf_offsets, const int32_t *leaf_taxon,
                 const int32_t *adj_depth, const double *adj_val, const int32_t *root_depth, const double *tree_weight,
                 int contract_edges, int32_t *part_dev, scs_node_stats *stats_host, uint8_t *needs_rerun) {
    if (B <= 0) return SCS_OK;
    if (!node_n || !tree_begin || !tree_end || !part_off || !seeds || !part_dev || !stats_host || !needs_rerun || T < 0 || L < 0)
        return fail(ctx, SCS_ERR_INVALID, "medium batch: bad argument");
    std::vector<MedNode> nodes(static_cast<size_t>(B));
    int64_t R = 0, w_total = 0, bit_total = 0, basis_total = 0, blocks = 0;
    int max_n = 0, max_trees = 0;
    for (int b = 0; b < B; ++b) {
        const int n = node_n[b];
        if (n < 1 || n > kMediumMax) return fail(ctx, SCS_ERR_INVALID, "medium batch: node size out of range");
        if (tree_begin[b] < 0 || tree_end[b] < tree_begin[b] || tree_end[b] > T || (b > 0 && tree_begin[b] < tree_end[b - 1]))
            return fail(ctx, SCS_ERR_INVALID, "medium batch: tree ranges out of order");
        MedNode &nd = nodes[b];
        nd.n = n;
        nd.words = scs_bit_words(n);
        nd.row_base = static_cast<int32_t>(R);
        nd.tree_begin = tree_begin[b];
        nd.tree_end = tree_end[b];
        nd.jcap = std::min(n - 1, kMaxBasis);
        nd.blk_base = static_cast<int32_t>(blocks);
        nd.pad0 = 0;
        blocks += (n + 31) / 32;
        nd.w_off = w_total;
        nd.bit_off = bit_total;
        nd.basis_off = basis_total;
        nd.part_off = part_off[b];
        nd.seed = seeds[b];
        R += n;
        w_total += static_cast<int64_t>(n) * n;
        bit_total += static_cast<int64_t>(n) * nd.words;
        basis_total += static_cast<int64_t>(nd.jcap + 3) * n;
        max_n = std::max(max_n, n);
        max_trees = std::max(max_trees, nd.tree_end - nd.tree_begin);
    }
    if (R >= (1ll << 31)) return fail(ctx, SCS_ERR_INVALID, "medium batch: too many rows");

    MedBuffers mb;
    int rc;
    MedNode *nodes_dev;
    int32_t *row_node, *tree_node;
    if ((rc = reserve_as(ctx, SLOT_MED_NODES, static_cast<size_t>(B), &nodes_dev))) return rc;
    if ((rc = reserve_as(ctx, SLOT_MED_ROW_NODE, static_cast<size_t>(R), &row_node))) return rc;
    if ((rc = reserve_as(ctx, SLOT_MED_TREE_NODE, static_cast<size_t>(T) + 1, &tree_node))) return rc;
    if ((rc = reserve_as(ctx, SLOT_W, static_cast<size_t>(w_total), &mb.W))) return rc;
    if ((rc = reserve_as(ctx, SLOT_WC, static_cast<size_t>(w_total), &mb.Wc))) return rc;
    if ((rc = reserve_as(ctx, SLOT_ADJ_BITS, static_cast<size_t>(bit_total), &mb.adj_bits))) return rc;
    if ((rc = reserve_as(ctx, SLOT_MAX_BITS, static_cast<size_t>(bit_total), &mb.max_bits))) return rc;
    if ((rc = reserve_as(ctx, SLOT_BASIS, static_cast<size_t>(basis_total), &mb.basis))) return rc;
    {
        const size_t rows = static_cast<size_t>(R);
        const size_t vec_bytes = 9 * (rows * sizeof(double) + 256) + static_cast<size_t>(B) * kScalarStride * sizeof(double) + 256;
        const size_t int_bytes = 9 * (rows * sizeof(int32_t) + 256) + (rows + B + 1) * sizeof(int32_t) + 256 +
                                 static_cast<size_t>(B) * sizeof(MedState) + 512;
        unsigned char *vec, *ints;
        if ((rc = reserve_as(ctx, SLOT_MED_VEC, vec_bytes, &vec))) return rc;
        if ((rc = reserve_as(ctx, SLOT_MED_STATE, int_bytes, &ints))) return rc;
        carve(vec, rows, &mb.degree);
        carve(vec, rows, &mb.degree_c);
        carve(vec, rows, &mb.isd);
        carve(vec, rows, &mb.z);
        carve(vec, rows, &mb.y);
        carve(vec, rows, &mb.yvec);
        carve(vec, rows, &mb.wstart);
        carve(vec, rows, &mb.embed);
        carve(vec, static_cast<size_t>(B) * kScalarStride, &mb.scalars);
        carve(ints, rows, &mb.occ);
        carve(ints, rows, &mb.uf_parent);
        carve(ints, rows, &mb.label[0]);
        carve(ints, rows, &mb.label[1]);
        carve(ints, rows, &mb.group);
        carve(ints, rows, &mb.members);
        carve(ints, rows, &mb.side);
        carve(ints, rows + B + 1, &mb.gptr);
        carve(ints, static_cast<size_t>(B), &mb.state);
        carve(ints, 64, &mb.remaining);
    }
    mb.nodes = nodes_dev;
    mb.row_node = row_node;
    int32_t *bad_dev = mb.remaining + 8;
    scs_node_stats *stats_dev;
    if ((rc = reserve_as(ctx, SLOT_NODE_STATS, static_cast<size_t>(B), &stats_dev))) return rc;

    void *pin_v;
    const size_t table_bytes = sizeof(MedNode) * static_cast<size_t>(B);
    if ((rc = reserve_pinned(ctx, table_bytes + 1024, &pin_v))) return rc;
    unsigned char *pin = static_cast<unsigned char *>(pin_v);
    std::memcpy(pin + 1024, nodes.data(), table_bytes);
    SCS_CUDA(ctx, cudaMemcpyAsync(nodes_dev, pin + 1024, table_bytes, cudaMemcpyHostToDevice, ctx->stream));
    ctx->h2d_bytes += static_cast<int64_t>(table_bytes);
    SCS_CUDA(ctx, cudaMemsetAsync(bad_dev, 0, sizeof(int32_t), ctx->stream));
    const int Ri = static_cast<int>(R);
    med_fill_maps<<<ceil_div(std::max<int64_t>(R, T), 256), 256, 0, ctx->stream>>>(B, Ri, T, nodes_dev, row_node, tree_node);
    SCS_LAUNCHED(ctx, "med_fill_maps");
    med_clear_state<<<ceil_div(B, 256), 256, 0, ctx->stream>>>(B, mb.state, mb.remaining);
    SCS_LAUNCHED(ctx, "med_clear_state");

    if ((rc = pcg_build_batch(ctx, B, static_cast<int>(blocks), Ri, T, L, max_n, max_trees, nodes_dev, tree_node, row_node, leaf_offsets, leaf_taxon,
                              adj_depth, adj_val, root_depth, tree_weight, mb.W, mb.occ, mb.adj_bits,
                              contract_edges ? mb.max_bits : nullptr, mb.degree, bad_dev)))
        return rc;

    const int row_blocks = ceil_div(R * 32, 256), vec_blocks = ceil_div(R, 256);
    for (int which = 0; which < (contract_edges ? 2 : 1); ++which) {
        const uint32_t *bits = which == 0 ? mb.adj_bits : mb.max_bits;
        med_uf_init<<<vec_blocks, 256, 0, ctx->stream>>>(Ri, mb.uf_parent);
        SCS_LAUNCHED(ctx, "med_uf_init");
        med_uf_hook_sample<<<row_blocks, 256, 0, ctx->stream>>>(Ri, nodes_dev, row_node, bits, mb.uf_parent);
        SCS_LAUNCHED(ctx, "med_uf_hook_sample");
        med_uf_snapshot<<<vec_blocks, 256, 0, ctx->stream>>>(Ri, mb.uf_parent, mb.label[which]);
        SCS_LAUNCHED(ctx, "med_uf_snapshot");
        med_uf_pick_giant<<<B, 1024, 0, ctx->stream>>>(nodes_dev, mb.label[which], mb.state, which);
        SCS_LAUNCHED(ctx, "med_uf_pick_giant");
        med_uf_hook_rest<<<row_blocks, 256, 0, ctx->stream>>>(Ri, nodes_dev, row_node, bits, mb.label[which], mb.state,
                                                             which, mb.uf_parent);
        SCS_LAUNCHED(ctx, "med_uf_hook_rest");
        med_uf_flatten<<<vec_blocks, 256, 0, ctx->stream>>>(Ri, row_node, mb.uf_parent, mb.label[which], mb.state, which);
        SCS_LAUNCHED(ctx, "med_uf_flatten");
    }
    med_decide<<<ceil_div(B, 256), 256, 0, ctx->stream>>>(B, contract_edges, nodes_dev, mb.state, mb.remaining);
    SCS_LAUNCHED(ctx, "med_decide");

    if (!ctx->medium_configured) {
        const int tail_smem = static_cast<int>((kMediumMax + 6 * (kMaxBasis + 8)) * sizeof(double));
        SCS_CUDA(ctx, cudaFuncSetAttribute(med_prepare, cudaFuncAttributeMaxDynamicSharedMemorySize, tail_smem));
        SCS_CUDA(ctx, cudaFuncSetAttribute(med_tail, cudaFuncAttributeMaxDynamicSharedMemorySize, tail_smem));
        SCS_CUDA(ctx, cudaFuncSetAttribute(med_finish, cudaFuncAttributeMaxDynamicSharedMemorySize, kMediumMax * 8));
        SCS_CUDA(ctx, cudaFuncSetAttribute(med_ritz_vector, cudaFuncAttributeMaxDynamicSharedMemorySize, (kMaxBasis + 8) * 8));
        SCS_CUDA(ctx, cudaFuncSetAttribute(med_ranks, cudaFuncAttributeMaxDynamicSharedMemorySize, kMediumMax * 8));
        SCS_CUDA(ctx, cudaFuncSetAttribute(med_contract_rows, cudaFuncAttributeMaxDynamicSharedMemorySize, kMediumMax * 8));
        ctx->medium_configured = true;
    }
    med_ranks<<<B, 1024, static_cast<size_t>(max_n) * 8, ctx->stream>>>(contract_edges, mb, part_dev);
    SCS_LAUNCHED(ctx, "med_ranks");
    if (contract_edges) {
        med_contract_rows<<<Ri, 256, static_cast<size_t>(max_n) * 8, ctx->stream>>>(mb);
        SCS_LAUNCHED(ctx, "med_contract_rows");
    }

    const size_t tail_smem = (static_cast<size_t>(max_n) + 6 * (kMaxBasis + 8)) * sizeof(double);
    med_prepare<<<B, kOneCta, tail_smem, ctx->stream>>>(mb);
    SCS_LAUNCHED(ctx, "med_prepare");
    const int steps_max = std::min(std::max(max_n - 1, 1), kMaxBasis);
    int32_t *pin_remaining = reinterpret_cast<int32_t *>(pin);
    cudaEvent_t probe[2] = {nullptr, nullptr};
    for (cudaEvent_t &e : probe) SCS_CUDA(ctx, cudaEventCreateWithFlags(&e, cudaEventDisableTiming));
    int j = 1, chunk = 0, pending = -1;
    bool finished = false;
    while (j <= steps_max && !finished) {
        const int chunk_end = std::min(steps_max, j == 1 ? 16 : j + 3);
        for (; j <= chunk_end; ++j) {
            med_matvec<<<row_blocks, kMvThreads, 0, ctx->stream>>>(Ri, 0, mb);
            SCS_LAUNCHED(ctx, "med_matvec");
            med_tail<<<B, kOneCta, tail_smem, ctx->stream>>>(j, mb);
            SCS_LAUNCHED(ctx, "med_tail");
        }
        SCS_CUDA(ctx, cudaMemcpyAsync(pin_remaining + (chunk & 1), mb.remaining, sizeof(int32_t), cudaMemcpyDeviceToHost, ctx->stream));
        SCS_CUDA(ctx, cudaEventRecord(probe[chunk & 1], ctx->stream));
        if (pending >= 0) {
            SCS_CUDA(ctx, cudaEventSynchronize(probe[pending & 1]));
            if (pin_remaining[pending & 1] == 0) finished = true;
        }
        pending = chunk++;
    }
    for (cudaEvent_t &e : probe) cudaEventDestroy(e);

    med_ritz_vector<<<B, kOneCta, (kMaxBasis + 8) * sizeof(double), ctx->stream>>>(mb);
    SCS_LAUNCHED(ctx, "med_ritz_vector");
    med_matvec<<<row_blocks, kMvThreads, 0, ctx->stream>>>(Ri, 1, mb);
    SCS_LAUNCHED(ctx, "med_matvec");
    int P = 1;
    while (P < max_n) P <<= 1;
    med_finish<<<B, kOneCta, static_cast<size_t>(P) * sizeof(double), ctx->stream>>>(mb, part_dev, stats_dev);
    SCS_LAUNCHED(ctx, "med_finish");

    SCS_CUDA(ctx, cudaMemcpyAsync(stats_host, stats_dev, sizeof(scs_node_stats) * B, cudaMemcpyDeviceToHost, ctx->stream));
    SCS_CUDA(ctx, cudaMemcpyAsync(pin + 512, bad_dev, sizeof(int32_t), cudaMemcpyDeviceToHost, ctx->stream));
    SCS_CUDA(ctx, cudaStreamSynchronize(ctx->stream));
    ctx->d2h_bytes += static_cast<int64_t>(sizeof(scs_node_stats)) * B;
    if (*reinterpret_cast<int32_t *>(pin + 512) != 0) return fail(ctx, SCS_ERR_INPUT, "leaf tour: taxon id out of range");
    for (int b = 0; b < B; ++b) {
        needs_rerun[b] = stats_host[b].solver == -3;
        if (stats_host[b].solver == -1) {
            stats_host[b].solver = 0;
            return fail(ctx, SCS_ERR_TOO_SMALL, "spectral step on a graph contracted to one vertex");
        }
    }
    return SCS_OK;
}

}
```

spectralclustersupertree_b200/csrc/spectral_dev.cuh:

```cuda
#pragma once

#include "common.cuh"

#include <cmath>

namespace scs {
namespace specdev {

constexpr int kMaxBasis = 256;
constexpr int kMaxRestarts = 8;
constexpr double kResidualTol = 1e-12;
constexpr double kBreakdown = 1e-11;
constexpr double kGapTie = 1e-7;
constexpr double kMarginTie = 1e-9;

constexpr int kMvThreads = 256;
constexpr int kVecThreads = 256;
constexpr int kOneCta = 1024;

__device__ __forceinline__ double warp_sum(double v) {
#pragma unroll
    for (int off = 16; off > 0; off >>= 1) v += __shfl_down_sync(0xffffffffu, v, off);
    return v;
}

__device__ __forceinline__ double block_sum(double v, double *scratch) {
    const int lane = threadIdx.x & 31, warp = threadIdx.x >> 5, nwarp = (blockDim.x + 31) >> 5;
    v = warp_sum(v);
    __syncthreads();
    if (lane == 0) scratch[warp] = v;
    __syncthreads();
    if (warp == 0) {
        double t = lane < nwarp ? scratch[lane] : 0.0;
        t = warp_sum(t);
        if (lane == 0) scratch[32] = t;
    }
    __syncthreads();
    return scratch[32];
}

__device__ __forceinline__ uint64_t splitmix64(uint64_t x) {
    x += 0x9E3779B97F4A7C15ull;
    x = (x ^ (x >> 30)) * 0xBF58476D1CE4E5B9ull;
    x = (x ^ (x >> 27)) * 0x94D049BB133111EBull;
    return x ^ (x >> 31);
}

__device__ __forceinline__ double2 load_stream(const double2 *p) {
    double2 v;
    asm volatile("ld.global.nc.L1::no_allocate.v2.f64 {%0, %1}, [%2];" : "=d"(v.x), "=d"(v.y) : "l"(p));
    return v;
}

__device__ __forceinline__ double row_dot_partial(const double *__restrict__ row, const double *__restrict__ z,
                                                  int m, int t, int nthr) {
    const int head = static_cast<int>((reinterpret_cast<uintptr_t>(row) >> 3) & 1u);
    const int nvec = (m - head) >> 1;
    const double2 *body = reinterpret_cast<const double2 *>(row + head);
    const double *zb = z + head;
    double acc0 = 0.0, acc1 = 0.0, acc2 = 0.0, acc3 = 0.0;
    int v = t;
    for (; v + 3 * nthr < nvec; v += 4 * nthr) {
        const double2 a = load_stream(body + v);
        const double2 b = load_stream(body + v + nthr);
        const double2 c = load_stream(body + v + 2 * nthr);
        const double2 d = load_stream(body + v + 3 * nthr);
        acc0 = fma(a.x, zb[2 * v], acc0);
        acc0 = fma(a.y, zb[2 * v + 1], acc0);
        acc1 = fma(b.x, zb[2 * (v + nthr)], acc1);
        acc1 = fma(b.y, zb[2 * (v + nthr) + 1], acc1);
        acc2 = fma(c.x, zb[2 * (v + 2 * nthr)], acc2);
        acc2 = fma(c.y, zb[2 * (v + 2 * nthr) + 1], acc2);
        acc3 = fma(d.x, zb[2 * (v + 3 * nthr)], acc3);
        acc3 = fma(d.y, zb[2 * (v + 3 * nthr) + 1], acc3);
    }
    if (v < nvec) {
        const int last = nvec - 1;
        const int vb = v + nthr, vc = v + 2 * nthr;
        const double mb = vb < nvec ? 1.0 : 0.0, mc = vc < nvec ? 1.0 : 0.0;
        const int ib = min(vb, last), ic = min(vc, last);
        const double2 a = load_stream(body + v);
        const double2 b = load_stream(body + ib);
        const double2 c = load_stream(body + ic);
        acc0 = fma(a.x, zb[2 * v], acc0);
        acc0 = fma(a.y, zb[2 * v + 1], acc0);
        acc1 = fma(b.x * mb, zb[2 * ib], acc1);
        acc1 = fma(b.y * mb, zb[2 * ib + 1], acc1);
        acc2 = fma(c.x * mc, zb[2 * ic], acc2);
        acc2 = fma(c.y * mc, zb[2 * ic + 1], acc2);
    }
    double acc = (acc0 + acc1) + (acc2 + acc3);
    if (t == 0) {
        if (head) acc = fma(row[0], z[0], acc);
        if ((m - head) & 1) acc = fma(row[m - 1], z[m - 1], acc);
    }
    return acc;
}

__device__ __forceinline__ int sturm_count(const double *a, const double *b2, int j, double x, double pivmin) {
    int cnt = 0;
    double q = a[1] - x;
    if (fabs(q) < pivmin) q = -pivmin;
    cnt += q < 0.0;
    for (int i = 2; i <= j; ++i) {
        q = (a[i] - x) - b2[i - 1] / q;
        if (fabs(q) < pivmin) q = -pivmin;
        cnt += q < 0.0;
    }
    return cnt;
}

__device__ inline void tridiag_solve(int jrun, const double *alpha, const double *beta, const int32_t *state, double *coef,
                              double *out, double *sm, int *counts, double *pair) {
    const int latched = state[0];
    const int j = latched > 0 && latched < jrun ? latched : jrun;
    double *a = sm;
    double *b = a + (j + 2);
    double *b2 = b + (j + 2);
    double *dplus = b2 + (j + 2);
    double *dminus = dplus + (j + 2);
    double *bounds = pair, *theta = pair + 2;
    const int tid = threadIdx.x, P = blockDim.x;
    __syncthreads();
    for (int i = tid + 1; i <= j; i += P) {
        a[i] = alpha[i];
        b[i] = beta[i];
        b2[i] = beta[i] * beta[i];
    }
    __syncthreads();
    if (tid == 0) {
        double lo = a[1], hi = a[1], bmax = 0.0;
        for (int i = 1; i <= j; ++i) {
            const double left = i > 1 ? fabs(b[i - 1]) : 0.0;
            const double right = i < j ? fabs(b[i]) : 0.0;
            lo = fmin(lo, a[i] - left - right);
            hi = fmax(hi, a[i] + left + right);
            bmax = fmax(bmax, right);
        }
        const double span = fmax(hi - lo, 1e-300);
        bounds[0] = lo - 1e-12 * span - 1e-300;
        bounds[1] = hi + 1e-12 * span + 1e-300;
    }
    __syncthreads();
    const double pivmin = 1e-290;
    const double glo = bounds[0], ghi = bounds[1];
    const int wanted = j >= 2 ? 2 : 1;
    for (int which = 0; which < wanted; ++which) {
        const int k = j - which;
        double lo = glo, hi = which == 0 ? ghi : theta[0];
        if (which == 1) hi = hi + fabs(hi) * 4.5e-16 + 1e-300;
        for (int round = 0; round < 9; ++round) {
            const double step = (hi - lo) / (P + 1);
            const double x = lo + step * (tid + 1);
            counts[tid] = sturm_count(a, b2, j, x, pivmin);
            __syncthreads();
            {
                const bool here = counts[tid] >= k;
                const bool before = tid > 0 && counts[tid - 1] >= k;
                if (here && !before) {
                    bounds[0] = tid == 0 ? lo : lo + step * tid;
                    bounds[1] = lo + step * (tid + 1);
                } else if (tid == P - 1 && !here) {
                    bounds[0] = lo + step * P;
                    bounds[1] = hi;
                }
            }
            __syncthreads();
            lo = bounds[0];
            hi = bounds[1];
            __syncthreads();
            if (!(hi > lo) || (hi - lo) <= 2.3e-16 * fmax(fabs(lo), fabs(hi))) break;
        }
        if (tid == 0) theta[which] = 0.5 * (lo + hi);
        __syncthreads();
    }
    if (tid == 0) {
        const double th = theta[0];
        double d = a[1] - th;
        if (fabs(d) < pivmin) d = pivmin;
        dplus[1] = d;
        for (int i = 2; i <= j; ++i) {
            d = (a[i] - th) - b2[i - 1] / dplus[i - 1];
            if (fabs(d) < pivmin) d = pivmin;
            dplus[i] = d;
        }
        d = a[j] - th;
        if (fabs(d) < pivmin) d = pivmin;
        dminus[j] = d;
        for (int i = j - 1; i >= 1; --i) {
            d = (a[i] - th) - b2[i] / dminus[i + 1];
            if (fabs(d) < pivmin) d = pivmin;
            dminus[i] = d;
        }
        int kbest = 1;
        double gbest = INFINITY;
        for (int i = 1; i <= j; ++i) {
            const double g = fabs(dplus[i] + dminus[i] - (a[i] - th));
            if (g < gbest) { gbest = g; kbest = i; }
        }
        double prev = 1.0;
        double norm2 = 1.0;
        b2[kbest] = 1.0;
        for (int i = kbest - 1; i >= 1; --i) {
            prev = -(b[i] / dplus[i]) * prev;
            b2[i] = prev;
            norm2 += prev * prev;
        }
        prev = 1.0;
        for (int i = kbest + 1; i <= j; ++i) {
            prev = -(b[i - 1] / dminus[i]) * prev;
            b2[i] = prev;
            norm2 += prev * prev;
        }
        const double inv = 1.0 / sqrt(norm2);
        for (int i = 1; i <= j; ++i) coef[i] = b2[i] * inv;
        for (int i = j + 1; i <= jrun; ++i) coef[i] = 0.0;
        coef[0] = 0.0;
        out[4] = static_cast<double>(j);
        out[0] = th;
        out[1] = j >= 2 ? theta[1] : nan("");
        out[2] = fabs(b[j] * b2[j] * inv);
        out[3] = b[j];
    }
    __syncthreads();
}


__device__ __forceinline__ void prepare_scaling_body(int m, const double *__restrict__ degree, double *__restrict__ isd, double *__restrict__ q0,
                int32_t *__restrict__ flags) {
    __shared__ double scratch[33];
    double vol = 0.0;
    bool bad = false;
    for (int i = threadIdx.x; i < m; i += blockDim.x) {
        const double d = degree[i];
        if (!(d >= 0.0) || isinf(d)) bad = true;
        vol += d > 0.0 ? d : 0.0;
    }
    vol = block_sum(vol, scratch);
    if (bad) flags[0] = 1;
    const double inv_norm = vol > 0.0 ? 1.0 / sqrt(vol) : 0.0;
    for (int i = threadIdx.x; i < m; i += blockDim.x) {
        const double d = degree[i];
        const double s = d > 0.0 ? sqrt(d) : 0.0;
        isd[i] = d > 0.0 ? 1.0 / s : 1.0;
        q0[i] = s * inv_norm;
    }
}

__device__ __forceinline__ void lanczos_tail_body(int m, int j, int nb, int hj, int check, const double *basis, const double *__restrict__ w_in,
             const double *__restrict__ isd, double *alpha, double *beta, double *next, double *__restrict__ z,
             int32_t *state, double *coef, double *ritz) {
    extern __shared__ double dyn[];
    double *w = dyn;
    double *h = w + m;
    double *tri = h + (kMaxBasis + 8);
    __shared__ double scratch[33];
    __shared__ int counts[kOneCta];
    __shared__ double pair[4];
    if (state[1]) return;
    const int tid = threadIdx.x, lane = tid & 31, warp = tid >> 5;
    for (int i = tid; i < m; i += kOneCta) w[i] = w_in[i];
    __syncthreads();
    double hkeep = 0.0;
    for (int pass = 0; pass < 2; ++pass) {
        for (int k = warp; k < nb; k += kOneCta / 32) {
            const double *b = basis + static_cast<size_t>(k) * m;
            double acc = 0.0;
            for (int i = lane; i < m; i += 32) acc = fma(b[i], w[i], acc);
            acc = warp_sum(acc);
            if (lane == 0) h[k] = acc;
        }
        __syncthreads();
        if (tid == 0 && j > 0) hkeep += h[hj];
        for (int i = tid; i < m; i += kOneCta) {
            double acc = w[i];
            for (int k = 0; k < nb; ++k) acc = fma(-h[k], basis[static_cast<size_t>(k) * m + i], acc);
            w[i] = acc;
        }
        __syncthreads();
    }
    double ss = 0.0;
    for (int i = tid; i < m; i += kOneCta) ss = fma(w[i], w[i], ss);
    ss = block_sum(ss, scratch);
    const double bnorm = sqrt(ss);
    if (tid == 0) {
        beta[j] = bnorm;
        if (j > 0) {
            alpha[j] = hkeep;
            if (bnorm <= kBreakdown && state[0] == 0) state[0] = j;
        } else {
            state[0] = 0;
        }
    }
    const double inv = bnorm > 0.0 ? 1.0 / bnorm : 0.0;
    for (int i = tid; i < m; i += kOneCta) {
        const double v = w[i] * inv;
        next[i] = v;
        z[i] = isd[i] * v;
    }
    __syncthreads();
    if (check && j > 0) {
        tridiag_solve(j, alpha, beta, state, coef, ritz, tri, counts, pair);
        if (tid == 0) {
            ritz[5] = static_cast<double>(j);
            if (ritz[3] <= kBreakdown || ritz[2] <= kResidualTol) {
                state[1] = 1;
                state[2] = j;
            }
        }
    }
}

__device__ __forceinline__ void ritz_vector_body(int m, int j, const double *__restrict__ basis, const double *__restrict__ coef,
            const double *__restrict__ isd, double *__restrict__ y, double *__restrict__ z) {
    __shared__ double scratch[33];
    extern __shared__ double cs[];
    for (int k = threadIdx.x; k <= j; k += blockDim.x) cs[k] = coef[k];
    __syncthreads();
    double ss = 0.0;
    for (int i = threadIdx.x; i < m; i += blockDim.x) {
        double acc = 0.0;
        for (int k = 1; k <= j; ++k) acc = fma(cs[k], basis[static_cast<size_t>(k) * m + i], acc);
        y[i] = acc;
        ss = fma(acc, acc, ss);
    }
    ss = block_sum(ss, scratch);
    const double inv = ss > 0.0 ? 1.0 / sqrt(ss) : 0.0;
    for (int i = threadIdx.x; i < m; i += blockDim.x) {
        const double v = y[i] * inv;
        y[i] = v;
        z[i] = isd[i] * v;
    }
}

__device__ __forceinline__ void true_residual_body(int m, const double *__restrict__ y, const double *__restrict__ Ny, const double *__restrict__ ritz,
              double *__restrict__ out) {
    __shared__ double scratch[33];
    const double th = ritz[0];
    double rr = 0.0, rq = 0.0;
    for (int i = threadIdx.x; i < m; i += blockDim.x) {
        const double r = Ny[i] - th * y[i];
        rr = fma(r, r, rr);
        rq = fma(y[i], Ny[i], rq);
    }
    rr = block_sum(rr, scratch);
    rq = block_sum(rq, scratch);
    if (threadIdx.x == 0) {
        out[0] = sqrt(rr);
        out[1] = rq;
    }
}

template <bool kShared, int kStage = 0>
__device__ __forceinline__ void two_means_1d_body(int m, int P, const double *__restrict__ y, const double *__restrict__ isd, double *__restrict__ u,
             double *__restrict__ sorted_g, int32_t *__restrict__ side, double *__restrict__ result) {
    extern __shared__ double sort_s[];
    __shared__ double scratch[33];
    __shared__ double best_score[32];
    __shared__ int best_index[32];
    __shared__ double bcast[4];
    __shared__ int ibcast;
    double *keys = kShared ? sort_s : sorted_g;
    const int tid = threadIdx.x, nthr = blockDim.x;
    double total = 0.0;
    if (kStage != 2) {
    double amax = -1.0;
    int imax = 0x7fffffff;
    for (int i = tid; i < m; i += nthr) {
        const double v = fabs(y[i] * isd[i]);
        if (v > amax) { amax = v; imax = i; }
    }
    for (int off = 16; off > 0; off >>= 1) {
        const double oa = __shfl_down_sync(0xffffffffu, amax, off);
        const int oi = __shfl_down_sync(0xffffffffu, imax, off);
        if (oa > amax || (oa == amax && oi < imax)) { amax = oa; imax = oi; }
    }
    if ((tid & 31) == 0) { best_score[tid >> 5] = amax; best_index[tid >> 5] = imax; }
    __syncthreads();
    if (tid == 0) {
        double ba = best_score[0];
        int bi = best_index[0];
        for (int w = 1; w < (nthr >> 5); ++w)
            if (best_score[w] > ba || (best_score[w] == ba && best_index[w] < bi)) { ba = best_score[w]; bi = best_index[w]; }
        ibcast = bi;
    }
    __syncthreads();
    const int arg = ibcast < m ? ibcast : 0;
    const double sign = y[arg] * isd[arg] < 0.0 ? -1.0 : 1.0;

    for (int i = tid; i < P; i += nthr) {
        double v = INFINITY;
        if (i < m) {
            v = sign * (y[i] * isd[i]);
            u[i] = v;
            total += v;
        }
        keys[i] = v;
    }
    if (kStage == 1) return;
    } else {
        for (int i = tid; i < m; i += nthr) total += u[i];
    }
    total = block_sum(total, scratch);
    const double mean = total / m;
    __syncthreads();

    for (int k = 2; kStage == 0 && k <= P; k <<= 1) {
        for (int jj = k >> 1; jj > 0; jj >>= 1) {
            for (int i = tid; i < P; i += nthr) {
                const int partner = i ^ jj;
                if (partner > i) {
                    const double x0 = kShared ? keys[i] : __ldcg(keys + i);
                    const double x1 = kShared ? keys[partner] : __ldcg(keys + partner);
                    const bool up = (i & k) == 0;
                    if ((x0 > x1) == up) {
                        if (kShared) { keys[i] = x1; keys[partner] = x0; }
                        else { __stcg(keys + i, x1); __stcg(keys + partner, x0); }
                    }
                }
            }
            __syncthreads();
        }
    }

    const int seg = (m + nthr - 1) / nthr;
    const int lo = min(tid * seg, m), hi = min(lo + seg, m);
    double local = 0.0;
    for (int i = lo; i < hi; ++i) local += (kShared ? keys[i] : __ldcg(keys + i)) - mean;
    double incl = local;
    for (int off = 1; off < 32; off <<= 1) {
        const double o = __shfl_up_sync(0xffffffffu, incl, off);
        if ((tid & 31) >= off) incl += o;
    }
    __syncthreads();
    if ((tid & 31) == 31) scratch[tid >> 5] = incl;
    __syncthreads();
    double before = 0.0;
    for (int w = 0; w < (tid >> 5); ++w) before += scratch[w];
    double all = 0.0;
    for (int w = 0; w < (nthr >> 5); ++w) all += scratch[w];
    double prefix = before + incl - local;
    double bscore = -1.0;
    int bidx = 0x7fffffff;
    for (int i = lo; i < hi; ++i) {
        prefix += (kShared ? keys[i] : __ldcg(keys + i)) - mean;
        const int cnt = i + 1;
        if (cnt < m) {
            const double rest = all - prefix;
            const double score = prefix * prefix / cnt + rest * rest / (m - cnt);
            if (score > bscore) { bscore = score; bidx = cnt; }
        }
    }
    for (int off = 16; off > 0; off >>= 1) {
        const double os = __shfl_down_sync(0xffffffffu, bscore, off);
        const int oi = __shfl_down_sync(0xffffffffu, bidx, off);
        if (os > bscore || (os == bscore && oi < bidx)) { bscore = os; bidx = oi; }
    }
    __syncthreads();
    if ((tid & 31) == 0) { best_score[tid >> 5] = bscore; best_index[tid >> 5] = bidx; }
    __syncthreads();
    if (tid == 0) {
        double bs = best_score[0];
        int bi = best_index[0];
        for (int w = 1; w < (nthr >> 5); ++w)
            if (best_score[w] > bs || (best_score[w] == bs && best_index[w] < bi)) { bs = best_score[w]; bi = best_index[w]; }
        if (bi >= m) bi = 1;
        ibcast = bi;
        bcast[1] = bs;
    }
    __syncthreads();
    {
        const int chosen = ibcast;
        double p2 = before + incl - local;
        double stable = 0.0, runner = -1.0;
        for (int i = lo; i < hi; ++i) {
            const double key = kShared ? keys[i] : __ldcg(keys + i);
            p2 += key - mean;
            const int cnt = i + 1;
            if (cnt < m) {
                const double rest = all - p2;
                const double mid = mean + 0.5 * (p2 / cnt + rest / (m - cnt));
                const double next = kShared ? keys[i + 1] : __ldcg(keys + i + 1);
                if (key < mid && mid < next) {
                    stable += 1.0;
                    if (cnt != chosen) runner = fmax(runner, p2 * p2 / cnt + rest * rest / (m - cnt));
                }
            }
        }
        stable = block_sum(stable, scratch);
        for (int off = 16; off > 0; off >>= 1) runner = fmax(runner, __shfl_down_sync(0xffffffffu, runner, off));
        __syncthreads();
        if ((tid & 31) == 0) best_score[tid >> 5] = runner;
        __syncthreads();
        if (tid == 0) {
            double r = best_score[0];
            for (int w = 1; w < (nthr >> 5); ++w) r = fmax(r, best_score[w]);
            result[4] = stable;
            result[5] = (r >= 0.0 && bcast[1] > 0.0) ? r / bcast[1] : 0.0;
        }
    }
    if (tid == 0) {
        const int bi = ibcast;
        double lower = 0.0;
        for (int i = 0; i < bi; ++i) lower += (kShared ? keys[i] : __ldcg(keys + i)) - mean;
        const double c0 = mean + lower / bi;
        const double c1 = mean + (all - lower) / (m - bi);
        const double mid = 0.5 * (c0 + c1);
        const double below = kShared ? keys[bi - 1] : __ldcg(keys + bi - 1);
        const double above = kShared ? keys[bi] : __ldcg(keys + bi);
        const double first = kShared ? keys[0] : __ldcg(keys);
        const double last = kShared ? keys[m - 1] : __ldcg(keys + m - 1);
        const double range = fmax(last - first, 1e-300);
        result[0] = fmin(fabs(below - mid), fabs(above - mid)) / range;
        result[1] = c0;
        result[2] = c1;
        result[3] = static_cast<double>(m - bi);
        bcast[0] = above;
    }
    __syncthreads();
    const double threshold = bcast[0];
    for (int i = tid; i < m; i += nthr) side[i] = u[i] >= threshold ? 1 : 0;
}

}
}
```

spectralclustersupertree_b200/engine.py:

```python

from __future__ import annotations

import ctypes
import os
from collections.abc import Sequence

import numpy as np

from . import _lib
from ._lib import NodeStats, ptr

WEIGHTINGS = ("one", "branch", "depth", "bootstrap")


class ScsError(RuntimeError):

    def __init__(self, status: int, detail: str = "") -> None:
        self.status = status
        text = _lib.load().scs_status_string(status).decode()
        super().__init__(f"libscs_b200: {text}" + (f" ({detail})" if detail else ""))


def _check(status: int, ctx=None) -> None:
    if status == _lib.SCS_OK:
        return
    detail = ""
    if ctx is not None:
        detail = _lib.load().scs_last_error(ctx).decode()
    raise ScsError(status, detail)


class Engine:

    def __init__(self, device: int | None = None) -> None:
        self._lib = _lib.load()
        if device is None:
            device = int(os.environ.get("SCS_B200_DEVICE", os.environ.get("LOCAL_RANK", "0")))
        handle = ctypes.c_void_p()
        status = self._lib.scs_ctx_create(device, None, ctypes.byref(handle))
        if status != _lib.SCS_OK:
            raise ScsError(status, f"scs_ctx_create(device={device}); the CUDA path has no CPU fallback")
        self._ctx = handle
        self.device = device

    def close(self) -> None:
        if getattr(self, "_ctx", None):
            self._lib.scs_ctx_destroy(self._ctx)
            self._ctx = None

    def __del__(self) -> None:
        try:
            self.close()
        except Exception:
            pass

    def __enter__(self) -> "Engine":
        return self

    def __exit__(self, *exc) -> None:
        self.close()

    @property
    def handle(self):
        return self._ctx

    @property
    def launch_count(self) -> int:
        return int(self._lib.scs_ctx_launch_count(self._ctx))

    def synchronize(self) -> None:
        _check(self._lib.scs_ctx_synchronize(self._ctx), self._ctx)

    def io_bytes(self) -> tuple[int, int]:
        h2d, d2h = ctypes.c_int64(0), ctypes.c_int64(0)
        _check(self._lib.scs_ctx_io_bytes(self._ctx, ctypes.byref(h2d), ctypes.byref(d2h)), self._ctx)
        return h2d.value, d2h.value

    def timer_start(self) -> None:
        _check(self._lib.scs_ctx_timer_start(self._ctx), self._ctx)

    def timer_stop(self) -> float:
        ms = ctypes.c_double(0.0)
        _check(self._lib.scs_ctx_timer_stop(self._ctx, ctypes.byref(ms)), self._ctx)
        return ms.value

    def set_small_node_limit(self, limit: int) -> None:
        _check(self._lib.scs_ctx_set_small_node_limit(self._ctx, limit), self._ctx)

    def set_medium_node_limit(self, limit: int) -> None:
        _check(self._lib.scs_ctx_set_medium_node_limit(self._ctx, limit), self._ctx)

    def set_device_forest(self, on: bool) -> None:
        _check(self._lib.scs_ctx_set_device_forest(self._ctx, int(bool(on))), self._ctx)

    def set_wide_entries(self, on: bool) -> None:
        _check(self._lib.scs_ctx_set_wide_entries(self._ctx, int(on)), self._ctx)

    def set_full_rows(self, on: bool) -> None:
        _check(self._lib.scs_ctx_set_full_rows(self._ctx, int(on)), self._ctx)

    def stage_seconds(self, reset: bool = True) -> dict:
        out = np.zeros(8)
        _check(self._lib.scs_ctx_stage_seconds(self._ctx, ptr(out), int(reset)), self._ctx)
        keys = ("enqueue_graph", "wait_graph", "enqueue_contract", "spectral", "result_copy", "lanczos_in_spectral",
                "tour_components")
        return dict(zip(keys, out[:7].tolist(), strict=True))

    def flush_l2(self) -> None:
        _check(self._lib.scs_ctx_flush_l2(self._ctx), self._ctx)

    def profile(self, on: bool) -> None:
        _check(self._lib.scs_ctx_profile_enable(self._ctx, int(on)), self._ctx)

    def profile_read(self, kind: int) -> dict:
        n, ms, nbytes, units = ctypes.c_int64(0), ctypes.c_double(0), ctypes.c_double(0), ctypes.c_double(0)
        status = self._lib.scs_ctx_profile_read(
            self._ctx, kind, ctypes.byref(n), ctypes.byref(ms), ctypes.byref(nbytes), ctypes.byref(units)
        )
        _check(status, self._ctx)
        return {"launches": n.value, "ms": ms.value, "bytes": nbytes.value, "units": units.value}

    def alloc(self, nbytes: int) -> int:
        out = ctypes.c_void_p()
        _check(self._lib.scs_dev_alloc(self._ctx, nbytes, ctypes.byref(out)), self._ctx)
        return out.value

    def free(self, dev: int) -> None:
        _check(self._lib.scs_dev_free(self._ctx, dev), self._ctx)

    def to_device(self, array: np.ndarray) -> int:
        array = np.ascontiguousarray(array)
        dev = self.alloc(max(array.nbytes, 16))
        if array.nbytes:
            _check(self._lib.scs_memcpy_h2d(self._ctx, dev, ptr(array), array.nbytes), self._ctx)
        return dev

    def to_host(self, dev: int, shape, dtype) -> np.ndarray:
        out = np.empty(shape, dtype=dtype)
        if out.nbytes:
            _check(self._lib.scs_memcpy_d2h(self._ctx, ptr(out), dev, out.nbytes), self._ctx)
        return out

    def node_split(self, tours, contract_edges: bool = True, seed: int = 0):
        part = np.empty(tours.n, dtype=np.int32)
        stats = NodeStats()
        status = self._lib.scs_node_split_host(
            self._ctx, tours.n, tours.num_trees, tours.num_leaves, ptr(tours.leaf_offsets), ptr(tours.leaf_taxon),
            ptr(tours.adj_depth), ptr(tours.adj_val), ptr(tours.root_depth), ptr(tours.tree_weight),
            int(bool(contract_edges)), seed & 0xFFFFFFFFFFFFFFFF, ptr(part), ctypes.byref(stats),
        )
        _check(status, self._ctx)
        return part, stats

    def forest_split(self, forest: "Forest", weighting: str, contract_edges: bool = True, seed: int = 0):
        cap = max(forest.num_taxa, 1)
        taxa = np.empty(cap, dtype=np.int32)
        part = np.empty(cap, dtype=np.int32)
        n = ctypes.c_int32(0)
        stats = NodeStats()
        status = self._lib.scs_forest_split(
            self._ctx, forest.handle, WEIGHTINGS.index(weighting), int(bool(contract_edges)),
            seed & 0xFFFFFFFFFFFFFFFF, ctypes.byref(n), ptr(taxa), ptr(part), ctypes.byref(stats),
        )
        if status == _lib.SCS_ERR_INPUT and weighting == "bootstrap":
            msg = "unsupported operand type(s) for *: 'NoneType' and 'float'"
            raise TypeError(msg)
        _check(status, self._ctx)
        return taxa[: n.value].copy(), part[: n.value].copy(), stats

    def supertree_build(self, forest: "Forest", weighting: str, contract_edges: bool = True, seed: int = 0,
                        record: bool = False, rank: int = 0, world: int = 1) -> dict:
        handle = ctypes.c_void_p()
        status = self._lib.scs_supertree_build_sharded(
            self._ctx, forest.handle, WEIGHTINGS.index(weighting), int(bool(contract_edges)),
            seed & 0xFFFFFFFFFFFFFFFF, int(bool(record)), rank, world, ctypes.byref(handle),
        )
        if status == _lib.SCS_ERR_INPUT and weighting == "bootstrap":
            msg = "unsupported operand type(s) for *: 'NoneType' and 'float'"
            raise TypeError(msg)
        if status == _lib.SCS_ERR_EMPTY:
            msg = "There must be at least one tree to make a supertree."
            raise ValueError(msg)
        _check(status, self._ctx)
        return self._collect_supertree(handle, record)

    def device_forest(self, forest: "Forest", weighting: str) -> "DeviceForest":
        handle = ctypes.c_void_p()
        _check(self._lib.scs_device_forest_create(self._ctx, forest.handle, WEIGHTINGS.index(weighting),
                                                  ctypes.byref(handle)), self._ctx)
        return DeviceForest(handle, weighting)

    def supertree_build_resident(self, resident: "DeviceForest", contract_edges: bool = True, seed: int = 0,
                                 record: bool = False, rank: int = 0, world: int = 1) -> dict:
        handle = ctypes.c_void_p()
        status = self._lib.scs_supertree_build_resident(
            self._ctx, resident.handle, int(bool(contract_edges)), seed & 0xFFFFFFFFFFFFFFFF, int(bool(record)), rank,
            world, ctypes.byref(handle),
        )
        if status == _lib.SCS_ERR_INPUT and resident.weighting == "bootstrap":
            msg = "unsupported operand type(s) for *: 'NoneType' and 'float'"
            raise TypeError(msg)
        if status == _lib.SCS_ERR_EMPTY:
            msg = "There must be at least one tree to make a supertree."
            raise ValueError(msg)
        _check(status, self._ctx)
        return self._collect_supertree(handle, record)

    def supertree_support(self, forest: "Forest", parent, taxon) -> tuple[np.ndarray, np.ndarray, np.ndarray]:
        parent = np.ascontiguousarray(parent, dtype=np.int32)
        taxon = np.ascontiguousarray(taxon, dtype=np.int32)
        n = len(parent)
        if len(taxon) != n:
            msg = "parent and taxon must have the same length"
            raise ValueError(msg)
        counts = np.zeros((n, 3), dtype=np.int32)
        weighted = np.zeros((n, 3), dtype=np.float64)
        per_tree = np.zeros((forest.num_trees, 4), dtype=np.int32)
        status = self._lib.scs_supertree_support(self._ctx, forest.handle, n, ptr(parent), ptr(taxon), ptr(counts),
                                                 ptr(weighted), ptr(per_tree))
        _check(status, self._ctx)
        return counts, weighted, per_tree

    def supertree_triplets(self, forest: "Forest", parent, taxon) -> np.ndarray:
        parent = np.ascontiguousarray(parent, dtype=np.int32)
        taxon = np.ascontiguousarray(taxon, dtype=np.int32)
        n = len(parent)
        if len(taxon) != n:
            msg = "parent and taxon must have the same length"
            raise ValueError(msg)
        per_tree = np.zeros((forest.num_trees, 5), dtype=np.int64)
        status = self._lib.scs_supertree_triplets(self._ctx, forest.handle, n, ptr(parent), ptr(taxon), ptr(per_tree))
        _check(status, self._ctx)
        return per_tree

    def supertree_taxon_triplets(self, forest: "Forest", parent, taxon) -> tuple[np.ndarray, np.ndarray]:
        parent = np.ascontiguousarray(parent, dtype=np.int32)
        taxon = np.ascontiguousarray(taxon, dtype=np.int32)
        n = len(parent)
        if len(taxon) != n:
            msg = "parent and taxon must have the same length"
            raise ValueError(msg)
        per_taxon = np.zeros((forest.num_taxa, 6), dtype=np.int64)
        weighted = np.zeros((forest.num_taxa, 3), dtype=np.float64)
        status = self._lib.scs_supertree_taxon_triplets(self._ctx, forest.handle, n, ptr(parent), ptr(taxon),
                                                        ptr(per_taxon), ptr(weighted))
        _check(status, self._ctx)
        return per_taxon, weighted

    def _collect_supertree(self, handle, record: bool) -> dict:
        try:
            count = self._lib.scs_supertree_num_nodes(handle)
            parent = np.empty(count, dtype=np.int32)
            taxon = np.empty(count, dtype=np.int32)
            _check(self._lib.scs_supertree_nodes(handle, ptr(parent), ptr(taxon)), self._ctx)
            small, large, waves, pairs = (ctypes.c_int64(0) for _ in range(4))
            self._lib.scs_supertree_counters(handle, ctypes.byref(small), ctypes.byref(large), ctypes.byref(waves),
                                             ctypes.byref(pairs))
            seconds = np.zeros(4)
            self._lib.scs_supertree_seconds(handle, ptr(seconds))
            medium, rerun, medium_s = ctypes.c_int64(0), ctypes.c_int64(0), ctypes.c_double(0.0)
            self._lib.scs_supertree_medium_info(handle, ctypes.byref(medium), ctypes.byref(rerun), ctypes.byref(medium_s))
            wave_tasks = np.zeros(max(waves.value, 1), dtype=np.int32)
            wave_max_n = np.zeros(max(waves.value, 1), dtype=np.int32)
            self._lib.scs_supertree_wave_info(handle, ptr(wave_tasks), ptr(wave_max_n))
            wave_seconds = np.zeros((max(waves.value, 1), 3))
            self._lib.scs_supertree_wave_seconds(handle, ptr(wave_seconds))
            out = {"parent": parent, "taxon": taxon, "nodes_small": small.value, "nodes_large": large.value,
                   "nodes_medium": medium.value, "nodes_rerun": rerun.value, "medium_seconds": medium_s.value,
                   "waves": waves.value, "pair_visits": pairs.value, "records": [],
                   "shared_prefix": int(self._lib.scs_supertree_shared_prefix(handle)),
                   "shared_records": int(self._lib.scs_supertree_shared_records(handle)),
                   "wave_tasks": wave_tasks[: waves.value].tolist(), "wave_max_n": wave_max_n[: waves.value].tolist(),
                   "wave_seconds": wave_seconds[: waves.value].tolist(),
                   "seconds": dict(zip(("large_nodes", "small_batches", "restrict", "tours"), seconds.tolist(), strict=True))}
            if record:
                for i in range(self._lib.scs_supertree_num_records(handle)):
                    n = self._lib.scs_supertree_record_size(handle, i)
                    taxa = np.empty(n, dtype=np.int32)
                    part = np.empty(n, dtype=np.int32)
                    stats = NodeStats()
                    self._lib.scs_supertree_record(handle, i, ptr(taxa), ptr(part), ctypes.byref(stats))
                    out["records"].append((taxa, part, stats))
                out["record_waves"] = [int(self._lib.scs_supertree_record_wave(handle, i))
                                       for i in range(len(out["records"]))]
            return out
        finally:
            self._lib.scs_supertree_destroy(handle)

    def shard_create(self, rank: int, world: int, n_max: int) -> bytes:
        handle = (ctypes.c_ubyte * _lib.IPC_HANDLE_BYTES)()
        _check(self._lib.scs_shard_create(self._ctx, rank, world, n_max, ctypes.addressof(handle)), self._ctx)
        return bytes(handle)

    def shard_connect(self, handles: Sequence[bytes]) -> None:
        blob = b"".join(handles)
        buf = (ctypes.c_ubyte * len(blob)).from_buffer_copy(blob)
        _check(self._lib.scs_shard_connect_ipc(self._ctx, ctypes.addressof(buf)), self._ctx)

    def shard_window(self) -> int:
        out, size = ctypes.c_void_p(), ctypes.c_size_t(0)
        _check(self._lib.scs_shard_window(self._ctx, ctypes.byref(out), ctypes.byref(size)), self._ctx)
        return out.value

    def shard_connect_local(self, windows: Sequence[int]) -> None:
        arr = (ctypes.c_void_p * len(windows))(*windows)
        _check(self._lib.scs_shard_connect_ptrs(self._ctx, ctypes.addressof(arr)), self._ctx)

    def shard_engage(self, on: bool = True) -> None:
        _check(self._lib.scs_shard_engage(self._ctx, int(on)), self._ctx)

    def shard_configure(self, min_n: int = 0, timeout_seconds: float = 0.0) -> None:
        _check(self._lib.scs_shard_configure(self._ctx, int(min_n), float(timeout_seconds)), self._ctx)

    def shard_barrier(self) -> None:
        _check(self._lib.scs_shard_barrier(self._ctx), self._ctx)

    @property
    def shard_nodes(self) -> int:
        return int(self._lib.scs_shard_nodes(self._ctx))

    def shard_destroy(self) -> None:
        _check(self._lib.scs_shard_destroy(self._ctx), self._ctx)

    def upload_tours(self, tours) -> dict:
        return {
            "n": tours.n, "T": tours.num_trees, "L": tours.num_leaves,
            "leaf_offsets": self.to_device(tours.leaf_offsets), "leaf_taxon": self.to_device(tours.leaf_taxon),
            "adj_depth": self.to_device(tours.adj_depth), "adj_val": self.to_device(tours.adj_val),
            "root_depth": self.to_device(tours.root_depth), "tree_weight": self.to_device(tours.tree_weight),
        }

    def free_tours(self, dev: dict) -> None:
        for key in ("leaf_offsets", "leaf_taxon", "adj_depth", "adj_val", "root_depth", "tree_weight"):
            self.free(dev[key])

    def node_split_dev(self, dev: dict, part_dev: int, contract_edges: bool = True, seed: int = 0) -> NodeStats:
        stats = NodeStats()
        status = self._lib.scs_node_split_dev(
            self._ctx, dev["n"], dev["T"], dev["L"], dev["leaf_offsets"], dev["leaf_taxon"], dev["adj_depth"],
            dev["adj_val"], dev["root_depth"], dev["tree_weight"], int(bool(contract_edges)),
            seed & 0xFFFFFFFFFFFFFFFF, part_dev, ctypes.byref(stats),
        )
        _check(status, self._ctx)
        return stats

    def pcg_build(self, tours, want_counts: bool = True) -> dict:
        n = tours.n
        words = self._lib.scs_bit_words(n)
        dev = self.upload_tours(tours)
        bufs = {
            "W": self.alloc(8 * n * n), "C": self.alloc(4 * n * n) if want_counts else None,
            "occ": self.alloc(4 * n), "adj_bits": self.alloc(4 * n * words), "max_bits": self.alloc(4 * n * words),
            "degree": self.alloc(8 * n),
        }
        try:
            poison = np.full(n * max(n, words) * 8, 0xFF, dtype=np.uint8)
            for key, nbytes in (("W", 8 * n * n), ("adj_bits", 4 * n * words), ("max_bits", 4 * n * words), ("degree", 8 * n)):
                _check(self._lib.scs_memcpy_h2d(self._ctx, bufs[key], ptr(poison), nbytes), self._ctx)
            status = self._lib.scs_pcg_build_dev(
                self._ctx, n, dev["T"], dev["L"], dev["leaf_offsets"], dev["leaf_taxon"], dev["adj_depth"],
                dev["adj_val"], dev["root_depth"], dev["tree_weight"], bufs["W"], bufs["C"], bufs["occ"],
                bufs["adj_bits"], bufs["max_bits"], bufs["degree"],
            )
            _check(status, self._ctx)
            self.synchronize()
            out = {
                "W": self.to_host(bufs["W"], (n, n), np.float64),
                "occ": self.to_host(bufs["occ"], (n,), np.int32),
                "adj_bits": self.to_host(bufs["adj_bits"], (n, words), np.uint32),
                "max_bits": self.to_host(bufs["max_bits"], (n, words), np.uint32),
                "degree": self.to_host(bufs["degree"], (n,), np.float64),
            }
            if want_counts:
                out["C"] = self.to_host(bufs["C"], (n, n), np.int32)
            return out
        finally:
            self.free_tours(dev)
            for b in bufs.values():
                if b:
                    self.free(b)

    def components(self, bits: np.ndarray, n: int) -> tuple[np.ndarray, int]:
        d_bits = self.to_device(bits)
        d_label = self.alloc(4 * n)
        count = ctypes.c_int32(0)
        try:
            _check(self._lib.scs_components_dev(self._ctx, n, d_bits, d_label, ctypes.byref(count)), self._ctx)
            return self.to_host(d_label, (n,), np.int32), count.value
        finally:
            self.free(d_bits)
            self.free(d_label)

    def contract(self, W: np.ndarray, adj_bits: np.ndarray, max_bits: np.ndarray):
        n = W.shape[0]
        d_W, d_adj, d_max = self.to_device(W), self.to_device(adj_bits), self.to_device(max_bits)
        d_group, d_Wc, d_deg = self.alloc(4 * n), self.alloc(8 * n * n), self.alloc(8 * n)
        m = ctypes.c_int32(0)
        try:
            status = self._lib.scs_contract_dev(self._ctx, n, d_W, d_adj, d_max, d_group, ctypes.byref(m), d_Wc, d_deg)
            _check(status, self._ctx)
            m = m.value
            group = self.to_host(d_group, (n,), np.int32)
            if m == n:
                return group, m, W.copy(), W.sum(axis=1)
            return group, m, self.to_host(d_Wc, (m, m), np.float64), self.to_host(d_deg, (m,), np.float64)
        finally:
            for d in (d_W, d_adj, d_max, d_group, d_Wc, d_deg):
                self.free(d)

    def spectral_bipartition(self, W: np.ndarray, seed: int = 0, degree: np.ndarray | None = None):
        W = np.ascontiguousarray(W, dtype=np.float64)
        m = W.shape[0]
        d_W = self.to_device(W)
        d_deg = None if degree is None else self.to_device(np.ascontiguousarray(degree, dtype=np.float64))
        d_side = self.alloc(4 * max(m, 1))
        stats = NodeStats()
        try:
            status = self._lib.scs_spectral_bipartition_dev(
                self._ctx, m, d_W, d_deg, seed & 0xFFFFFFFFFFFFFFFF, d_side, ctypes.byref(stats)
            )
            _check(status, self._ctx)
            return self.to_host(d_side, (m,), np.int32), stats
        finally:
            self.free(d_W)
            self.free(d_side)
            if d_deg:
                self.free(d_deg)

    def normalized_matvec(self, W: np.ndarray, inv_sqrt_deg: np.ndarray, x: np.ndarray) -> np.ndarray:
        m = W.shape[0]
        d_W, d_s, d_x, d_y = self.to_device(W), self.to_device(inv_sqrt_deg), self.to_device(x), self.alloc(8 * m)
        try:
            _check(self._lib.scs_normalized_matvec_dev(self._ctx, m, d_W, d_s, d_x, d_y), self._ctx)
            return self.to_host(d_y, (m,), np.float64)
        finally:
            for d in (d_W, d_s, d_x, d_y):
                self.free(d)

    def last_node_pointers(self) -> dict:
        n, m = ctypes.c_int(0), ctypes.c_int(0)
        ptrs = [ctypes.c_void_p() for _ in range(7)]
        _check(
            self._lib.scs_node_last_buffers(self._ctx, ctypes.byref(n), ctypes.byref(m), *[ctypes.byref(p) for p in ptrs]),
            self._ctx,
        )
        names = ("W", "adj_bits", "max_bits", "occ", "degree", "Wc", "group")
        out = {k: p.value for k, p in zip(names, ptrs, strict=True)}
        out.update({"n": n.value, "m": m.value})
        return out

    def last_node_rows(self, row_lo: int, row_hi: int) -> tuple[np.ndarray, np.ndarray]:
        p = self.last_node_pointers()
        n = p["n"]
        words = self._lib.scs_bit_words(n)
        W = self.to_host(p["W"] + 8 * row_lo * n, (row_hi - row_lo, n), np.float64)
        bits = self.to_host(p["adj_bits"] + 4 * row_lo * words, (row_hi - row_lo, words), np.uint32)
        return W, bits

    def matvec_on_device(self, m: int, W_dev: int, isd_dev: int, x: np.ndarray) -> np.ndarray:
        d_x = self.to_device(np.ascontiguousarray(x, dtype=np.float64))
        d_y = self.alloc(8 * m)
        try:
            _check(self._lib.scs_normalized_matvec_dev(self._ctx, m, W_dev, isd_dev, d_x, d_y), self._ctx)
            return self.to_host(d_y, (m,), np.float64)
        finally:
            self.free(d_x)
            self.free(d_y)

    def last_node_buffers(self) -> dict:
        n, m = ctypes.c_int(0), ctypes.c_int(0)
        ptrs = [ctypes.c_void_p() for _ in range(7)]
        _check(
            self._lib.scs_node_last_buffers(self._ctx, ctypes.byref(n), ctypes.byref(m), *[ctypes.byref(p) for p in ptrs]),
            self._ctx,
        )
        n, m = n.value, m.value
        words = self._lib.scs_bit_words(n)
        W, adj, mx, occ, deg, Wc, group = (p.value for p in ptrs)
        out = {"n": n, "m": m}
        out["W"] = self.to_host(W, (n, n), np.float64)
        out["adj_bits"] = self.to_host(adj, (n, words), np.uint32)
        out["occ"] = self.to_host(occ, (n,), np.int32)
        out["degree"] = self.to_host(deg, (n,), np.float64)
        if mx:
            out["max_bits"] = self.to_host(mx, (n, words), np.uint32)
        if m and m != n and Wc and group:
            out["Wc"] = self.to_host(Wc, (m, m), np.float64)
            out["group"] = self.to_host(group, (n,), np.int32)
        return out


def merge_sharded(parts: list[tuple[np.ndarray, np.ndarray, int]]) -> tuple[np.ndarray, np.ndarray]:
    parent0, taxon0, prefix = parts[0]
    parents = [np.asarray(parent0, dtype=np.int32)]
    taxa = [np.asarray(taxon0, dtype=np.int32)]
    head_taxon = taxa[0][:prefix].copy()
    offset = len(parent0)
    for parent, taxon, p in parts[1:]:
        if p != prefix:
            msg = f"ranks disagree on the shared prefix ({p} != {prefix})"
            raise ValueError(msg)
        parent = np.asarray(parent, dtype=np.int32)
        taxon = np.asarray(taxon, dtype=np.int32)
        head_taxon = np.maximum(head_taxon, taxon[:prefix])
        tail = parent[prefix:].copy()
        tail[tail >= prefix] += offset - prefix
        parents.append(tail)
        taxa.append(taxon[prefix:])
        offset += len(tail)
    taxa[0] = np.concatenate([head_taxon, taxa[0][prefix:]])
    return np.concatenate(parents), np.concatenate(taxa)


def set_host_threads(threads: int) -> None:
    status = _lib.load().scs_set_host_threads(int(threads))
    if status != _lib.SCS_OK:
        raise ScsError(status, "scs_set_host_threads")


_DEFAULT: Engine | None = None


_FASTFLATTEN = None


def _fastflatten():
    global _FASTFLATTEN
    if _FASTFLATTEN is None:
        try:
            from . import build as _build

            _build.build_fastflatten()
            from . import _fastflatten as module

            _FASTFLATTEN = module
        except Exception:
            _FASTFLATTEN = False
    return _FASTFLATTEN or None


def default_engine() -> Engine:
    global _DEFAULT
    if _DEFAULT is None:
        _DEFAULT = Engine()
    return _DEFAULT


def unpack_bits(bits: np.ndarray, n: int) -> np.ndarray:
    as_bytes = bits.view(np.uint8).reshape(bits.shape[0], -1)
    return np.unpackbits(as_bytes, axis=1, bitorder="little")[:, :n].astype(bool)


class DeviceForest:

    def __init__(self, handle, weighting: str) -> None:
        self._lib = _lib.load()
        self.handle = handle
        self.weighting = weighting

    @property
    def nbytes(self) -> int:
        return int(self._lib.scs_device_forest_bytes(self.handle))

    def close(self) -> None:
        if self.handle:
            self._lib.scs_device_forest_destroy(self.handle)
            self.handle = None


class Forest:

    def __init__(self, handle, names: Sequence[str]) -> None:
        self._lib = _lib.load()
        self._handle = handle
        self.names = names

    @classmethod
    def from_arrays(cls, node_offsets, parent, length, support, taxon, weights, names: Sequence[str],
                    copy: bool = False) -> "Forest":
        lib = _lib.load()
        node_offsets = np.ascontiguousarray(node_offsets, dtype=np.int64)
        parent = np.ascontiguousarray(parent, dtype=np.int32)
        taxon = np.ascontiguousarray(taxon, dtype=np.int32)
        length = None if length is None else np.ascontiguousarray(length, dtype=np.float64)
        support = None if support is None else np.ascontiguousarray(support, dtype=np.float64)
        weights = np.ascontiguousarray(weights, dtype=np.float64)
        handle = ctypes.c_void_p()
        create = lib.scs_forest_create if copy else lib.scs_forest_create_view
        status = create(
            len(weights), ptr(node_offsets), ptr(parent), ptr(length), ptr(support), ptr(taxon), ptr(weights),
            len(names), ctypes.byref(handle),
        )
        if status != _lib.SCS_OK:
            raise ScsError(status, "scs_forest_create: " + lib.scs_forest_last_error().decode())
        forest = cls(handle, names)
        if not copy:
            forest._borrowed = (parent, length, support, taxon)
        return forest

    @classmethod
    def from_trees(cls, trees: Sequence, weights: Sequence[float], names: Sequence[str] | None = None) -> "Forest":
        fast = _fastflatten()
        if fast is not None:
            raw_off, raw_par, raw_len, raw_sup, raw_tax, seen = fast.flatten(list(trees))
            if names is None:
                names = sorted(seen)
            taxon_id = {name: i for i, name in enumerate(names)}
            remap = np.fromiter((taxon_id[name] for name in seen), dtype=np.int32, count=len(seen))
            taxon = np.frombuffer(raw_tax, dtype=np.int32)
            if len(remap):
                taxon = np.where(taxon >= 0, remap[np.maximum(taxon, 0)], -1).astype(np.int32)
            return cls.from_arrays(np.frombuffer(raw_off, dtype=np.int64), np.frombuffer(raw_par, dtype=np.int32),
                                   np.frombuffer(raw_len, dtype=np.float64), np.frombuffer(raw_sup, dtype=np.float64),
                                   taxon, list(weights), names)
        if names is None:
            found: set[str] = set()
            for tree in trees:
                found.update(tree.get_tip_names())
            names = sorted(found)
        taxon_id = {name: i for i, name in enumerate(names)}
        offsets = [0]
        parent: list[int] = []
        length: list[float] = []
        support: list[float] = []
        taxon: list[int] = []
        nan = float("nan")
        for tree in trees:
            base = len(parent)
            stack = [(tree, -1)]
            while stack:
                node, up = stack.pop()
                k = len(parent) - base
                parent.append(up)
                ln, sp = node.length, getattr(node, "support", None)
                length.append(nan if ln is None else float(ln))
                support.append(nan if sp is None else float(sp))
                kids = list(node)
                if kids:
                    taxon.append(-1)
                    stack.extend((child, k) for child in reversed(kids))
                else:
                    taxon.append(taxon_id[node.name])
            offsets.append(len(parent))
        return cls.from_arrays(offsets, parent, length, support, taxon, list(weights), names)

    @classmethod
    def from_newick(cls, text: bytes | str) -> "Forest":
        from .tree import NewickError

        lib = _lib.load()
        data = text.encode("utf-8") if isinstance(text, str) else bytes(text)
        handle, names_ptr = ctypes.c_void_p(), ctypes.c_void_p()
        names_bytes, num_taxa = ctypes.c_size_t(), ctypes.c_int()
        status = lib.scs_forest_parse_newick(data, len(data), ctypes.byref(handle), ctypes.byref(names_ptr),
                                             ctypes.byref(names_bytes), ctypes.byref(num_taxa))
        if status == _lib.SCS_ERR_INPUT:
            raise NewickError(lib.scs_newick_last_error().decode())
        if status != _lib.SCS_OK:
            raise ScsError(status, "scs_forest_parse_newick")
        try:
            raw = ctypes.string_at(names_ptr, names_bytes.value)
        finally:
            lib.scs_free(names_ptr)
        names = [part.decode("utf-8") for part in raw.split(b"\0")[: num_taxa.value]]
        return cls(handle, names)

    def close(self) -> None:
        if getattr(self, "_handle", None):
            self._lib.scs_forest_destroy(self._handle)
            self._handle = None

    def __del__(self) -> None:
        try:
            self.close()
        except Exception:
            pass

    @property
    def handle(self):
        return self._handle

    @property
    def num_trees(self) -> int:
        return self._lib.scs_forest_num_trees(self._handle)

    @property
    def num_nodes(self) -> int:
        return self._lib.scs_forest_num_nodes(self._handle)

    @property
    def num_leaves(self) -> int:
        return self._lib.scs_forest_num_leaves(self._handle)

    @property
    def num_taxa(self) -> int:
        return self._lib.scs_forest_num_taxa(self._handle)

    @property
    def pair_visits(self) -> int:
        return self._lib.scs_forest_pair_visits(self._handle)

    def taxa(self) -> np.ndarray:
        present = np.zeros(max(self.num_taxa, 1), dtype=np.uint8)
        n = self._lib.scs_forest_taxa(self._handle, ptr(present))
        if n < 0:
            raise ScsError(n, "scs_forest_taxa")
        return np.flatnonzero(present[: self.num_taxa]).astype(np.int32)

    def tree_arrays(self, t: int):
        count = ctypes.c_int64(0)
        status = self._lib.scs_forest_tree_info(self._handle, t, ctypes.byref(count), None, None)
        if status != _lib.SCS_OK:
            raise ScsError(status, "scs_forest_tree_info")
        m = count.value
        parent = np.empty(m, dtype=np.int32)
        length = np.empty(m, dtype=np.float64)
        support = np.empty(m, dtype=np.float64)
        taxon = np.empty(m, dtype=np.int32)
        status = self._lib.scs_forest_tree(self._handle, t, ptr(parent), ptr(length), ptr(support), ptr(taxon))
        if status != _lib.SCS_OK:
            raise ScsError(status, "scs_forest_tree")
        return parent, length, support, taxon

    def weights(self) -> np.ndarray:
        out = np.empty(self.num_trees, dtype=np.float64)
        w = ctypes.c_double(0.0)
        for t in range(self.num_trees):
            self._lib.scs_forest_tree_info(self._handle, t, None, ctypes.byref(w), None)
            out[t] = w.value
        return out

    def induce(self, keep_ids: np.ndarray) -> "Forest":
        keep = np.zeros(max(self.num_taxa, 1), dtype=np.uint8)
        keep[keep_ids] = 1
        handle = ctypes.c_void_p()
        status = self._lib.scs_forest_induce(self._handle, ptr(keep), ctypes.byref(handle))
        if status != _lib.SCS_OK:
            raise ScsError(status, "scs_forest_induce")
        return Forest(handle, self.names)

    def induce_parts(self, part_of_taxon: np.ndarray, count: int) -> tuple[list["Forest"], np.ndarray]:
        part = np.ascontiguousarray(part_of_taxon, dtype=np.int32)
        if len(part) < self.num_taxa:
            msg = "part_of_taxon needs one entry per global taxon id"
            raise ValueError(msg)
        handles = (ctypes.c_void_p * max(count, 1))()
        present = np.zeros(max(self.num_taxa, 1), dtype=np.uint8)
        status = self._lib.scs_forest_induce_parts(self._handle, ptr(part), count, ctypes.addressof(handles), ptr(present))
        if status != _lib.SCS_OK:
            raise ScsError(status, "scs_forest_induce_parts")
        forests = [Forest(ctypes.c_void_p(handles[c]), self.names) for c in range(count)]
        return forests, np.flatnonzero(present[: self.num_taxa]).astype(np.int32)

    def tours(self, weighting: str, local_id: np.ndarray | None = None):
        from .flatten import LeafTours

        present = self.taxa()
        if local_id is None:
            local_id = np.full(max(self.num_taxa, 1), -1, dtype=np.int32)
            local_id[present] = np.arange(len(present), dtype=np.int32)
        T, L = self.num_trees, self.num_leaves
        out = LeafTours(
            n=len(present),
            leaf_offsets=np.zeros(T + 1, dtype=np.int64),
            leaf_taxon=np.zeros(L, dtype=np.int32),
            adj_depth=np.zeros(L, dtype=np.int32),
            adj_val=np.zeros(L, dtype=np.float64),
            root_depth=np.zeros(T, dtype=np.int32),
            tree_weight=np.zeros(T, dtype=np.float64),
        )
        status = self._lib.scs_forest_tours(
            self._handle, WEIGHTINGS.index(weighting), ptr(local_id), ptr(out.leaf_offsets), ptr(out.leaf_taxon),
            ptr(out.adj_depth), ptr(out.adj_val), ptr(out.root_depth), ptr(out.tree_weight),
        )
        if status == _lib.SCS_ERR_INPUT and weighting == "bootstrap":
            msg = "unsupported operand type(s) for *: 'NoneType' and 'float'"
            raise TypeError(msg)
        if status != _lib.SCS_OK:
            raise ScsError(status, "scs_forest_tours")
        return out
```

Baseline: 0.06137.

## Fuse medium-node Lanczos loop into one persistent kernel with cluster-wide CTAs

Replaces the host-driven loop of med_prepare/med_matvec/med_tail launches, with its periodic device-to-host polling of a remaining counter, by a single med_spectral kernel. Each node runs its whole Lanczos iteration, Ritz vector, and finish step on-device. Nodes of at least medium_wide_min taxa are spread over an 8-CTA thread block cluster synchronised with cluster.sync, and smaller nodes get one CTA each. This removes many launches and host round-trips, but it loses batched row parallelism across nodes and relies on cluster scheduling. It also drops __restrict__ qualifiers, since buffers are now read and written inside the same kernel.

```diff
diff --git a/include/scs_b200.h b/include/scs_b200.h
--- a/include/scs_b200.h
+++ b/include/scs_b200.h
@@ -53,6 +53,7 @@
 int scs_ctx_set_device_forest(scs_ctx *ctx, int on);
 int scs_ctx_set_wide_entries(scs_ctx *ctx, int on);
 int scs_ctx_set_full_rows(scs_ctx *ctx, int on);
+int scs_ctx_set_medium_wide_min(scs_ctx *ctx, int n);
 int scs_ctx_stage_seconds(scs_ctx *ctx, double *seconds8, int reset);
 int scs_ctx_flush_l2(scs_ctx *ctx);
 int scs_ctx_profile_enable(scs_ctx *ctx, int on);
diff --git a/spectralclustersupertree_b200/_lib.py b/spectralclustersupertree_b200/_lib.py
--- a/spectralclustersupertree_b200/_lib.py
+++ b/spectralclustersupertree_b200/_lib.py
@@ -76,6 +76,7 @@
     "scs_ctx_set_device_forest": (c_int, [_P, c_int]),
     "scs_ctx_set_wide_entries": (c_int, [_P, c_int]),
     "scs_ctx_set_full_rows": (c_int, [_P, c_int]),
+    "scs_ctx_set_medium_wide_min": (c_int, [_P, c_int]),
     "scs_ctx_stage_seconds": (c_int, [_P, _P, c_int]),
     "scs_ctx_flush_l2": (c_int, [_P]),
     "scs_ctx_profile_enable": (c_int, [_P, c_int]),
diff --git a/spectralclustersupertree_b200/csrc/common.cuh b/spectralclustersupertree_b200/csrc/common.cuh
--- a/spectralclustersupertree_b200/csrc/common.cuh
+++ b/spectralclustersupertree_b200/csrc/common.cuh
@@ -13,6 +13,7 @@
 namespace scs {
 
 constexpr int kMediumMaxDefault = 4096;
+constexpr int kMediumWideMinDefault = 512;
 
 struct DeviceBuffer {
     void *ptr = nullptr;
@@ -168,6 +169,7 @@
     bool medium_configured = false;
     bool device_forest = true;
     int medium_limit = scs::kMediumMaxDefault;
+    int medium_wide_min = scs::kMediumWideMinDefault;
     bool wide_entries = false;
     bool full_rows = false;
     int small_limit = 32;
diff --git a/spectralclustersupertree_b200/csrc/context.cu b/spectralclustersupertree_b200/csrc/context.cu
--- a/spectralclustersupertree_b200/csrc/context.cu
+++ b/spectralclustersupertree_b200/csrc/context.cu
@@ -68,6 +68,7 @@
         worker->small_limit = ctx->small_limit;
         worker->full_rows = ctx->full_rows;
         worker->wide_entries = ctx->wide_entries;
+        worker->medium_wide_min = ctx->medium_wide_min;
     }
     return SCS_OK;
 }
@@ -564,6 +565,13 @@
     return SCS_OK;
 }
 
+int scs_ctx_set_medium_wide_min(scs_ctx *ctx, int n) {
+    if (!ctx || n < 0) return SCS_ERR_INVALID;
+    ctx->medium_wide_min = n;
+    for (scs_ctx *worker : ctx->workers) worker->medium_wide_min = n;
+    return SCS_OK;
+}
+
 int scs_ctx_stage_seconds(scs_ctx *ctx, double *seconds8, int reset) {
     if (!ctx || !seconds8) return SCS_ERR_INVALID;
     for (int i = 0; i < 8; ++i) {
diff --git a/spectralclustersupertree_b200/csrc/medium.cu b/spectralclustersupertree_b200/csrc/medium.cu
--- a/spectralclustersupertree_b200/csrc/medium.cu
+++ b/spectralclustersupertree_b200/csrc/medium.cu
@@ -3,7 +3,10 @@
 #include "spectral_dev.cuh"
 #include "uf.cuh"
 
+#include <cooperative_groups.h>
+
 #include <algorithm>
+#include <cstdlib>
 #include <vector>
 
 namespace scs {
@@ -11,6 +14,7 @@
 namespace {
 
 using namespace specdev;
+namespace cg = cooperative_groups;
 
 enum MedMode : int32_t { MED_DISCONNECTED = 0, MED_TOO_SMALL = 1, MED_PAIR = 2, MED_LANCZOS = 3 };
 enum MedOutcome : int32_t { MED_RUNNING = 0, MED_CONVERGED = 1, MED_INVARIANT = 2, MED_OUT_OF_STEPS = 3 };
@@ -42,7 +46,6 @@
     double *isd, *z, *y, *yvec, *wstart, *embed;
     double *basis, *scalars;
     int32_t *side;
-    int32_t *remaining;
 };
 
 __device__ __forceinline__ double *node_alpha(const MedBuffers &mb, int b) { return mb.scalars + static_cast<size_t>(b) * kScalarStride; }
@@ -71,9 +74,8 @@
     }
 }
 
-__global__ void med_clear_state(int B, MedState *state, int32_t *remaining) {
+__global__ void med_clear_state(int B, MedState *state) {
     const int b = blockIdx.x * blockDim.x + threadIdx.x;
-    if (b == 0) *remaining = 0;
     if (b >= B) return;
     MedState s;
     memset(&s, 0, sizeof(s));
@@ -193,8 +195,7 @@
     if (r == i) atomicAdd(&state[row_node[i]].ncomp[which], 1);
 }
 
-__global__ void med_decide(int B, int contract_edges, const MedNode *__restrict__ nodes, MedState *state,
-                           int32_t *remaining) {
+__global__ void med_decide(int B, int contract_edges, const MedNode *__restrict__ nodes, MedState *state) {
     const int b = blockIdx.x * blockDim.x + threadIdx.x;
     if (b >= B) return;
     MedState &s = state[b];
@@ -209,7 +210,6 @@
     else {
         s.mode = MED_LANCZOS;
         s.jmax = min(m - 1, nodes[b].jcap);
-        atomicAdd(remaining, 1);
     }
 }
 
@@ -355,16 +355,26 @@
     }
 }
 
+constexpr int kSpectralCluster = 8;
+constexpr int kIdleCta = -1;
+
 __device__ __forceinline__ const double *node_matrix(const MedBuffers &mb, const MedNode &nd, const MedState &st) {
     return (st.m == nd.n ? mb.W : mb.Wc) + nd.w_off;
 }
 
-__global__ void __launch_bounds__(kOneCta)
-med_prepare(MedBuffers mb) {
-    const int b = blockIdx.x;
+__device__ __forceinline__ void node_matvec(const MedBuffers &mb, const MedNode &nd, const MedState &st, int first, int nwarps) {
+    const int m = st.m, base = nd.row_base, lane = threadIdx.x & 31;
+    const double *Wm = node_matrix(mb, nd, st);
+    for (int A = first; A < m; A += nwarps) {
+        double acc = row_dot_partial(Wm + static_cast<size_t>(A) * m, mb.z + base, m, lane, 32);
+        acc = warp_sum(acc);
+        if (lane == 0) mb.y[base + A] = mb.isd[base + A] * acc;
+    }
+}
+
+__device__ __forceinline__ void node_prepare(const MedBuffers &mb, int b) {
     const MedNode &nd = mb.nodes[b];
     MedState &st = mb.state[b];
-    if (st.mode != MED_LANCZOS) return;
     const int m = st.m, base = nd.row_base;
     const double *degree = (m == nd.n ? mb.degree : mb.degree_c) + base;
     double *basis = mb.basis + nd.basis_off;
@@ -379,30 +389,9 @@
                       st.lanczos, node_coef(mb, b), node_ritz(mb, b));
 }
 
-__global__ void __launch_bounds__(kMvThreads)
-med_matvec(int R, int final, MedBuffers mb) {
-    const int r = (blockIdx.x * kMvThreads + threadIdx.x) >> 5;
-    const int lane = threadIdx.x & 31;
-    if (r >= R) return;
-    const int b = mb.row_node[r];
-    const MedState &st = mb.state[b];
-    if (st.mode != MED_LANCZOS || (!final && st.lanczos[1])) return;
-    const MedNode &nd = mb.nodes[b];
-    const int m = st.m, base = nd.row_base;
-    const int A = r - base;
-    if (A >= m) return;
-    const double *Wm = node_matrix(mb, nd, st);
-    double acc = row_dot_partial(Wm + static_cast<size_t>(A) * m, mb.z + base, m, lane, 32);
-    acc = warp_sum(acc);
-    if (lane == 0) mb.y[r] = mb.isd[r] * acc;
-}
-
-__global__ void __launch_bounds__(kOneCta)
-med_tail(int j, MedBuffers mb) {
-    const int b = blockIdx.x;
+__device__ __forceinline__ void node_tail(const MedBuffers &mb, int b, int j) {
     const MedNode &nd = mb.nodes[b];
     MedState &st = mb.state[b];
-    if (st.mode != MED_LANCZOS || st.lanczos[1] || j > st.jmax) return;
     const int m = st.m, base = nd.row_base;
     const int check = (j == st.jmax) || (j % 4) == 0;
     double *basis = mb.basis + nd.basis_off;
@@ -412,37 +401,32 @@
     if (threadIdx.x == 0) {
         if (st.lanczos[1]) {
             st.outcome = ritz[3] <= kBreakdown ? MED_INVARIANT : MED_CONVERGED;
-            atomicSub(mb.remaining, 1);
         } else if (j == st.jmax) {
             st.outcome = MED_OUT_OF_STEPS;
             st.lanczos[1] = 1;
             st.lanczos[2] = j;
-            atomicSub(mb.remaining, 1);
-        }
-    }
-}
-
-__global__ void __launch_bounds__(kOneCta)
-med_ritz_vector(MedBuffers mb) {
-    const int b = blockIdx.x;
+        }
+    }
+}
+
+__device__ __forceinline__ void node_ritz_vector(const MedBuffers &mb, int b) {
     const MedNode &nd = mb.nodes[b];
     const MedState &st = mb.state[b];
-    if (st.mode != MED_LANCZOS) return;
     const int base = nd.row_base;
     const int jdone = static_cast<int>(node_ritz(mb, b)[5]);
     ritz_vector_body(st.m, jdone, mb.basis + nd.basis_off, node_coef(mb, b), mb.isd + base, mb.yvec + base, mb.z + base);
 }
 
-__global__ void __launch_bounds__(kOneCta)
-med_finish(MedBuffers mb, int32_t *__restrict__ part, scs_node_stats *__restrict__ stats) {
-    const int b = blockIdx.x;
-    const MedNode &nd = mb.nodes[b];
-    const MedState &st = mb.state[b];
-    const int n = nd.n, m = st.m, base = nd.row_base, tid = threadIdx.x;
+__device__ __forceinline__ int cta_node(const int32_t *cta_task) {
+    const int t = cta_task[blockIdx.x];
+    return t >= 0 ? t : -2 - t;
+}
+
+__device__ __forceinline__ scs_node_stats node_record(const MedNode &nd, const MedState &st) {
     const double nan_v = __longlong_as_double(0x7ff8000000000000ll);
     scs_node_stats out;
     out.n_components = st.ncomp[0];
-    out.contracted_size = st.mode == MED_DISCONNECTED ? n : m;
+    out.contracted_size = st.mode == MED_DISCONNECTED ? nd.n : st.m;
     out.spectral_ran = st.mode != MED_DISCONNECTED;
     out.solver = 0;
     out.matvecs = 0;
@@ -454,34 +438,53 @@
     out.residual = nan_v;
     out.margin = nan_v;
     out.kmeans_runner_up = 0.0;
-    if (st.mode == MED_DISCONNECTED) {
-        if (tid == 0) stats[b] = out;
-        return;
-    }
-    if (st.mode == MED_TOO_SMALL) {
-        out.solver = -1;
-        if (tid == 0) stats[b] = out;
-        return;
-    }
-    const int32_t *group = mb.group + base;
-    if (st.mode == MED_PAIR) {
-        for (int v = tid; v < n; v += kOneCta) part[nd.part_off + v] = group[v];
-        out.solver = 1;
-        out.eig[1] = 2.0;
-        out.residual = 0.0;
-        out.margin = 0.5;
-        if (tid == 0) stats[b] = out;
-        return;
-    }
-    double *ritz = node_ritz(mb, b);
-    true_residual_body(m, mb.yvec + base, mb.y + base, ritz, ritz + 8);
-    const int P = 1 << (32 - __clz(max(m - 1, 1)));
-    two_means_1d_body<true>(m, P, mb.yvec + base, mb.isd + base, mb.embed + base, nullptr, mb.side + base, ritz + 12);
-    __syncthreads();
-    for (int v = tid; v < n; v += kOneCta) part[nd.part_off + v] = mb.side[base + group[v]];
+    return out;
+}
+
+__device__ __forceinline__ void node_finish(const MedBuffers &mb, const int32_t *cta_task, int32_t *__restrict__ part,
+                                            scs_node_stats *__restrict__ stats) {
+    const int tid = threadIdx.x;
+    {
+        const int b = cta_node(cta_task);
+        const MedNode &nd = mb.nodes[b];
+        const MedState &st = mb.state[b];
+        const int n = nd.n, m = st.m, base = nd.row_base;
+        if (st.mode == MED_DISCONNECTED) {
+            if (tid == 0) stats[b] = node_record(nd, st);
+            return;
+        }
+        if (st.mode == MED_TOO_SMALL) {
+            scs_node_stats out = node_record(nd, st);
+            out.solver = -1;
+            if (tid == 0) stats[b] = out;
+            return;
+        }
+        if (st.mode == MED_PAIR) {
+            for (int v = tid; v < n; v += kOneCta) part[nd.part_off + v] = mb.group[base + v];
+            scs_node_stats out = node_record(nd, st);
+            out.solver = 1;
+            out.eig[1] = 2.0;
+            out.residual = 0.0;
+            out.margin = 0.5;
+            if (tid == 0) stats[b] = out;
+            return;
+        }
+        double *ritz = node_ritz(mb, b);
+        true_residual_body(m, mb.yvec + base, mb.y + base, ritz, ritz + 8);
+        const int P = 1 << (32 - __clz(max(m - 1, 1)));
+        two_means_1d_body<true>(m, P, mb.yvec + base, mb.isd + base, mb.embed + base, nullptr, mb.side + base, ritz + 12);
+    }
+    __syncthreads();
+    const int b = cta_node(cta_task);
+    const MedNode &nd = mb.nodes[b];
+    const MedState &st = mb.state[b];
+    const int n = nd.n, m = st.m, base = nd.row_base;
+    for (int v = tid; v < n; v += kOneCta) part[nd.part_off + v] = mb.side[base + mb.group[base + v]];
     if (tid == 0) {
+        const double *ritz = node_ritz(mb, b);
         const double theta1 = ritz[0], theta2 = ritz[1];
         const int steps = static_cast<int>(ritz[4]);
+        scs_node_stats out = node_record(nd, st);
         out.solver = 3;
         out.matvecs = st.lanczos[2] + 1;
         out.eig[1] = 1.0 - theta1;
@@ -500,6 +503,92 @@
         stats[b] = out;
     }
 }
+
+__device__ __forceinline__ bool node_done(const MedState &st) {
+    return *reinterpret_cast<const volatile int32_t *>(&st.lanczos[1]) != 0;
+}
+
+template <bool kWide>
+__device__ __forceinline__ void node_sync() {
+    if (kWide) cg::this_cluster().sync();
+    else __syncthreads();
+}
+
+template <bool kWide>
+__device__ __forceinline__ bool cta_leads() {
+    return !kWide || cg::this_cluster().block_rank() == 0;
+}
+
+template <bool kWide>
+__device__ __forceinline__ void cta_matvec(const MedBuffers &mb, const int32_t *cta_task) {
+    const int warp = threadIdx.x >> 5;
+    const int b = cta_node(cta_task);
+    if (kWide) node_matvec(mb, mb.nodes[b], mb.state[b], static_cast<int>(cg::this_cluster().block_rank()) * (kOneCta / 32) + warp,
+                           kSpectralCluster * (kOneCta / 32));
+    else node_matvec(mb, mb.nodes[b], mb.state[b], warp, kOneCta / 32);
+}
+
+template <bool kWide>
+__device__ __forceinline__ void node_spectral(const MedBuffers &mb, const int32_t *cta_task, int32_t *__restrict__ part,
+                                              scs_node_stats *__restrict__ stats) {
+    if (mb.state[cta_node(cta_task)].mode != MED_LANCZOS) {
+        if (cta_leads<kWide>()) node_finish(mb, cta_task, part, stats);
+        return;
+    }
+    if (cta_leads<kWide>()) node_prepare(mb, cta_node(cta_task));
+    node_sync<kWide>();
+    __shared__ int step_s;
+    if (threadIdx.x == 0) step_s = 1;
+    while (true) {
+        cta_matvec<kWide>(mb, cta_task);
+        node_sync<kWide>();
+        if (cta_leads<kWide>()) node_tail(mb, cta_node(cta_task), step_s);
+        node_sync<kWide>();
+        if (node_done(mb.state[cta_node(cta_task)])) break;
+        if (threadIdx.x == 0) ++step_s;
+    }
+    if (cta_leads<kWide>()) node_ritz_vector(mb, cta_node(cta_task));
+    node_sync<kWide>();
+    cta_matvec<kWide>(mb, cta_task);
+    node_sync<kWide>();
+    if (cta_leads<kWide>()) node_finish(mb, cta_task, part, stats);
+}
+
+__global__ void __cluster_dims__(kSpectralCluster, 1, 1) __launch_bounds__(kOneCta, 1)
+med_spectral(MedBuffers mb, const int32_t *cta_task, int32_t *__restrict__ part, scs_node_stats *__restrict__ stats) {
+    const int task = cta_task[blockIdx.x];
+    if (task >= 0) node_spectral<false>(mb, cta_task, part, stats);
+    else if (task != kIdleCta) node_spectral<true>(mb, cta_task, part, stats);
+}
+
+struct StageTimes {
+    static constexpr int kMarks = 7;
+    cudaEvent_t ev[kMarks] = {};
+    int marked = 0;
+    explicit StageTimes(bool on) {
+        if (!on) return;
+        for (cudaEvent_t &e : ev)
+            if (cudaEventCreate(&e) != cudaSuccess) e = nullptr;
+    }
+    ~StageTimes() {
+        for (cudaEvent_t e : ev)
+            if (e) cudaEventDestroy(e);
+    }
+    void mark(cudaStream_t s) {
+        if (marked < kMarks && ev[marked]) cudaEventRecord(ev[marked], s);
+        ++marked;
+    }
+    void print(int B, int max_n) const {
+        if (marked != kMarks) return;
+        float ms[kMarks - 1];
+        for (int k = 0; k + 1 < kMarks; ++k)
+            if (!ev[k] || !ev[k + 1] || cudaEventElapsedTime(&ms[k], ev[k], ev[k + 1]) != cudaSuccess) return;
+        std::fprintf(stderr,
+                     "[scs medium] nodes %4d max_n %5d | maps %6.3f graph %6.3f components %6.3f contraction %6.3f "
+                     "spectral %6.3f stats %6.3f ms\n",
+                     B, max_n, ms[0], ms[1], ms[2], ms[3], ms[4], ms[5]);
+    }
+};
 
 template <typename T>
 int carve(unsigned char *&cursor, size_t count, T **out) {
@@ -550,10 +639,20 @@
     }
     if (R >= (1ll << 31)) return fail(ctx, SCS_ERR_INVALID, "medium batch: too many rows");
 
+    std::vector<int32_t> order(static_cast<size_t>(B)), cta_task;
+    for (int b = 0; b < B; ++b) order[b] = b;
+    std::stable_sort(order.begin(), order.end(), [&](int32_t x, int32_t y) { return node_n[x] > node_n[y]; });
+    for (int32_t b : order)
+        if (node_n[b] >= ctx->medium_wide_min) cta_task.insert(cta_task.end(), kSpectralCluster, -2 - b);
+    for (int32_t b : order)
+        if (node_n[b] < ctx->medium_wide_min) cta_task.push_back(b);
+    while (cta_task.size() % kSpectralCluster) cta_task.push_back(kIdleCta);
+
     MedBuffers mb;
     int rc;
     MedNode *nodes_dev;
-    int32_t *row_node, *tree_node;
+    int32_t *row_node, *tree_node, *bad_dev, *cta_task_dev;
+    const size_t cta_bytes = cta_task.size() * sizeof(int32_t) + 256;
     if ((rc = reserve_as(ctx, SLOT_MED_NODES, static_cast<size_t>(B), &nodes_dev))) return rc;
     if ((rc = reserve_as(ctx, SLOT_MED_ROW_NODE, static_cast<size_t>(R), &row_node))) return rc;
     if ((rc = reserve_as(ctx, SLOT_MED_TREE_NODE, static_cast<size_t>(T) + 1, &tree_node))) return rc;
@@ -569,7 +668,7 @@
                                  static_cast<size_t>(B) * sizeof(MedState) + 512;
         unsigned char *vec, *ints;
         if ((rc = reserve_as(ctx, SLOT_MED_VEC, vec_bytes, &vec))) return rc;
-        if ((rc = reserve_as(ctx, SLOT_MED_STATE, int_bytes, &ints))) return rc;
+        if ((rc = reserve_as(ctx, SLOT_MED_STATE, int_bytes + cta_bytes, &ints))) return rc;
         carve(vec, rows, &mb.degree);
         carve(vec, rows, &mb.degree_c);
         carve(vec, rows, &mb.isd);
@@ -588,32 +687,40 @@
         carve(ints, rows, &mb.side);
         carve(ints, rows + B + 1, &mb.gptr);
         carve(ints, static_cast<size_t>(B), &mb.state);
-        carve(ints, 64, &mb.remaining);
+        carve(ints, 64, &bad_dev);
+        carve(ints, cta_task.size(), &cta_task_dev);
     }
     mb.nodes = nodes_dev;
     mb.row_node = row_node;
-    int32_t *bad_dev = mb.remaining + 8;
     scs_node_stats *stats_dev;
     if ((rc = reserve_as(ctx, SLOT_NODE_STATS, static_cast<size_t>(B), &stats_dev))) return rc;
 
     void *pin_v;
-    const size_t table_bytes = sizeof(MedNode) * static_cast<size_t>(B);
-    if ((rc = reserve_pinned(ctx, table_bytes + 1024, &pin_v))) return rc;
+    const size_t table_bytes = sizeof(MedNode) * static_cast<size_t>(B), table_span = (table_bytes + 255) & ~static_cast<size_t>(255);
+    if ((rc = reserve_pinned(ctx, 1024 + table_span + cta_bytes, &pin_v))) return rc;
     unsigned char *pin = static_cast<unsigned char *>(pin_v);
     std::memcpy(pin + 1024, nodes.data(), table_bytes);
+    std::memcpy(pin + 1024 + table_span, cta_task.data(), cta_task.size() * sizeof(int32_t));
+    static const bool trace = std::getenv("SCS_DRIVER_TRACE") != nullptr;
+    StageTimes times(trace);
+    times.mark(ctx->stream);
     SCS_CUDA(ctx, cudaMemcpyAsync(nodes_dev, pin + 1024, table_bytes, cudaMemcpyHostToDevice, ctx->stream));
-    ctx->h2d_bytes += static_cast<int64_t>(table_bytes);
+    SCS_CUDA(ctx, cudaMemcpyAsync(cta_task_dev, pin + 1024 + table_span, cta_task.size() * sizeof(int32_t), cudaMemcpyHostToDevice,
+                                  ctx->stream));
+    ctx->h2d_bytes += static_cast<int64_t>(table_bytes + cta_task.size() * sizeof(int32_t));
     SCS_CUDA(ctx, cudaMemsetAsync(bad_dev, 0, sizeof(int32_t), ctx->stream));
     const int Ri = static_cast<int>(R);
     med_fill_maps<<<ceil_div(std::max<int64_t>(R, T), 256), 256, 0, ctx->stream>>>(B, Ri, T, nodes_dev, row_node, tree_node);
     SCS_LAUNCHED(ctx, "med_fill_maps");
-    med_clear_state<<<ceil_div(B, 256), 256, 0, ctx->stream>>>(B, mb.state, mb.remaining);
+    med_clear_state<<<ceil_div(B, 256), 256, 0, ctx->stream>>>(B, mb.state);
     SCS_LAUNCHED(ctx, "med_clear_state");
+    times.mark(ctx->stream);
 
     if ((rc = pcg_build_batch(ctx, B, static_cast<int>(blocks), Ri, T, L, max_n, max_trees, nodes_dev, tree_node, row_node, leaf_offsets, leaf_taxon,
                               adj_depth, adj_val, root_depth, tree_weight, mb.W, mb.occ, mb.adj_bits,
                               contract_edges ? mb.max_bits : nullptr, mb.degree, bad_dev)))
         return rc;
+    times.mark(ctx->stream);
 
     const int row_blocks = ceil_div(R * 32, 256), vec_blocks = ceil_div(R, 256);
     for (int which = 0; which < (contract_edges ? 2 : 1); ++which) {
@@ -632,15 +739,29 @@
         med_uf_flatten<<<vec_blocks, 256, 0, ctx->stream>>>(Ri, row_node, mb.uf_parent, mb.label[which], mb.state, which);
         SCS_LAUNCHED(ctx, "med_uf_flatten");
     }
-    med_decide<<<ceil_div(B, 256), 256, 0, ctx->stream>>>(B, contract_edges, nodes_dev, mb.state, mb.remaining);
+    times.mark(ctx->stream);
+    med_decide<<<ceil_div(B, 256), 256, 0, ctx->stream>>>(B, contract_edges, nodes_dev, mb.state);
     SCS_LAUNCHED(ctx, "med_decide");
 
     if (!ctx->medium_configured) {
-        const int tail_smem = static_cast<int>((kMediumMax + 6 * (kMaxBasis + 8)) * sizeof(double));
-        SCS_CUDA(ctx, cudaFuncSetAttribute(med_prepare, cudaFuncAttributeMaxDynamicSharedMemorySize, tail_smem));
-        SCS_CUDA(ctx, cudaFuncSetAttribute(med_tail, cudaFuncAttributeMaxDynamicSharedMemorySize, tail_smem));
-        SCS_CUDA(ctx, cudaFuncSetAttribute(med_finish, cudaFuncAttributeMaxDynamicSharedMemorySize, kMediumMax * 8));
-        SCS_CUDA(ctx, cudaFuncSetAttribute(med_ritz_vector, cudaFuncAttributeMaxDynamicSharedMemorySize, (kMaxBasis + 8) * 8));
+        const int spectral_smem = static_cast<int>((kMediumMax + 6 * (kMaxBasis + 8)) * sizeof(double));
+        SCS_CUDA(ctx, cudaFuncSetAttribute(med_spectral, cudaFuncAttributeMaxDynamicSharedMemorySize, spectral_smem));
+        if (trace) {
+            cudaLaunchConfig_t cfg = {};
+            cudaLaunchAttribute cluster;
+            cluster.id = cudaLaunchAttributeClusterDimension;
+            cluster.val.clusterDim.x = kSpectralCluster;
+            cluster.val.clusterDim.y = cluster.val.clusterDim.z = 1;
+            cfg.gridDim = dim3(kSpectralCluster);
+            cfg.blockDim = dim3(kOneCta);
+            cfg.dynamicSmemBytes = static_cast<size_t>(spectral_smem);
+            cfg.attrs = &cluster;
+            cfg.numAttrs = 1;
+            int clusters = 0;
+            if (cudaOccupancyMaxActiveClusters(&clusters, med_spectral, &cfg) == cudaSuccess)
+                std::fprintf(stderr, "[scs medium] med_spectral: at most %d clusters of %d x %d threads resident (%d B of dynamic shared memory)\n",
+                             clusters, kSpectralCluster, kOneCta, spectral_smem);
+        }
         SCS_CUDA(ctx, cudaFuncSetAttribute(med_ranks, cudaFuncAttributeMaxDynamicSharedMemorySize, kMediumMax * 8));
         SCS_CUDA(ctx, cudaFuncSetAttribute(med_contract_rows, cudaFuncAttributeMaxDynamicSharedMemorySize, kMediumMax * 8));
         ctx->medium_configured = true;
@@ -651,46 +772,21 @@
         med_contract_rows<<<Ri, 256, static_cast<size_t>(max_n) * 8, ctx->stream>>>(mb);
         SCS_LAUNCHED(ctx, "med_contract_rows");
     }
+    times.mark(ctx->stream);
 
     const size_t tail_smem = (static_cast<size_t>(max_n) + 6 * (kMaxBasis + 8)) * sizeof(double);
-    med_prepare<<<B, kOneCta, tail_smem, ctx->stream>>>(mb);
-    SCS_LAUNCHED(ctx, "med_prepare");
-    const int steps_max = std::min(std::max(max_n - 1, 1), kMaxBasis);
-    int32_t *pin_remaining = reinterpret_cast<int32_t *>(pin);
-    cudaEvent_t probe[2] = {nullptr, nullptr};
-    for (cudaEvent_t &e : probe) SCS_CUDA(ctx, cudaEventCreateWithFlags(&e, cudaEventDisableTiming));
-    int j = 1, chunk = 0, pending = -1;
-    bool finished = false;
-    while (j <= steps_max && !finished) {
-        const int chunk_end = std::min(steps_max, j == 1 ? 16 : j + 3);
-        for (; j <= chunk_end; ++j) {
-            med_matvec<<<row_blocks, kMvThreads, 0, ctx->stream>>>(Ri, 0, mb);
-            SCS_LAUNCHED(ctx, "med_matvec");
-            med_tail<<<B, kOneCta, tail_smem, ctx->stream>>>(j, mb);
-            SCS_LAUNCHED(ctx, "med_tail");
-        }
-        SCS_CUDA(ctx, cudaMemcpyAsync(pin_remaining + (chunk & 1), mb.remaining, sizeof(int32_t), cudaMemcpyDeviceToHost, ctx->stream));
-        SCS_CUDA(ctx, cudaEventRecord(probe[chunk & 1], ctx->stream));
-        if (pending >= 0) {
-            SCS_CUDA(ctx, cudaEventSynchronize(probe[pending & 1]));
-            if (pin_remaining[pending & 1] == 0) finished = true;
-        }
-        pending = chunk++;
-    }
-    for (cudaEvent_t &e : probe) cudaEventDestroy(e);
-
-    med_ritz_vector<<<B, kOneCta, (kMaxBasis + 8) * sizeof(double), ctx->stream>>>(mb);
-    SCS_LAUNCHED(ctx, "med_ritz_vector");
-    med_matvec<<<row_blocks, kMvThreads, 0, ctx->stream>>>(Ri, 1, mb);
-    SCS_LAUNCHED(ctx, "med_matvec");
     int P = 1;
     while (P < max_n) P <<= 1;
-    med_finish<<<B, kOneCta, static_cast<size_t>(P) * sizeof(double), ctx->stream>>>(mb, part_dev, stats_dev);
-    SCS_LAUNCHED(ctx, "med_finish");
+    const size_t spectral_smem = std::max({tail_smem, static_cast<size_t>(P) * sizeof(double), (kMaxBasis + 8) * sizeof(double)});
+    med_spectral<<<static_cast<int>(cta_task.size()), kOneCta, spectral_smem, ctx->stream>>>(mb, cta_task_dev, part_dev, stats_dev);
+    SCS_LAUNCHED(ctx, "med_spectral");
+    times.mark(ctx->stream);
 
     SCS_CUDA(ctx, cudaMemcpyAsync(stats_host, stats_dev, sizeof(scs_node_stats) * B, cudaMemcpyDeviceToHost, ctx->stream));
     SCS_CUDA(ctx, cudaMemcpyAsync(pin + 512, bad_dev, sizeof(int32_t), cudaMemcpyDeviceToHost, ctx->stream));
+    times.mark(ctx->stream);
     SCS_CUDA(ctx, cudaStreamSynchronize(ctx->stream));
+    times.print(B, max_n);
     ctx->d2h_bytes += static_cast<int64_t>(sizeof(scs_node_stats)) * B;
     if (*reinterpret_cast<int32_t *>(pin + 512) != 0) return fail(ctx, SCS_ERR_INPUT, "leaf tour: taxon id out of range");
     for (int b = 0; b < B; ++b) {
diff --git a/spectralclustersupertree_b200/csrc/spectral_dev.cuh b/spectralclustersupertree_b200/csrc/spectral_dev.cuh
--- a/spectralclustersupertree_b200/csrc/spectral_dev.cuh
+++ b/spectralclustersupertree_b200/csrc/spectral_dev.cuh
@@ -52,7 +52,7 @@
     return v;
 }
 
-__device__ __forceinline__ double row_dot_partial(const double *__restrict__ row, const double *__restrict__ z,
+__device__ __forceinline__ double row_dot_partial(const double *__restrict__ row, const double *z,
                                                   int m, int t, int nthr) {
     const int head = static_cast<int>((reinterpret_cast<uintptr_t>(row) >> 3) & 1u);
     const int nvec = (m - head) >> 1;
@@ -226,8 +226,7 @@
 }
 
 
-__device__ __forceinline__ void prepare_scaling_body(int m, const double *__restrict__ degree, double *__restrict__ isd, double *__restrict__ q0,
-                int32_t *__restrict__ flags) {
+__device__ __forceinline__ void prepare_scaling_body(int m, const double *degree, double *isd, double *q0, int32_t *flags) {
     __shared__ double scratch[33];
     double vol = 0.0;
     bool bad = false;
@@ -247,8 +246,8 @@
     }
 }
 
-__device__ __forceinline__ void lanczos_tail_body(int m, int j, int nb, int hj, int check, const double *basis, const double *__restrict__ w_in,
-             const double *__restrict__ isd, double *alpha, double *beta, double *next, double *__restrict__ z,
+__device__ __forceinline__ void lanczos_tail_body(int m, int j, int nb, int hj, int check, const double *basis, const double *w_in,
+             const double *isd, double *alpha, double *beta, double *next, double *z,
              int32_t *state, double *coef, double *ritz) {
     extern __shared__ double dyn[];
     double *w = dyn;
@@ -311,8 +310,8 @@
     }
 }
 
-__device__ __forceinline__ void ritz_vector_body(int m, int j, const double *__restrict__ basis, const double *__restrict__ coef,
-            const double *__restrict__ isd, double *__restrict__ y, double *__restrict__ z) {
+__device__ __forceinline__ void ritz_vector_body(int m, int j, const double *basis, const double *coef,
+            const double *isd, double *y, double *z) {
     __shared__ double scratch[33];
     extern __shared__ double cs[];
     for (int k = threadIdx.x; k <= j; k += blockDim.x) cs[k] = coef[k];
@@ -333,8 +332,8 @@
     }
 }
 
-__device__ __forceinline__ void true_residual_body(int m, const double *__restrict__ y, const double *__restrict__ Ny, const double *__restrict__ ritz,
-              double *__restrict__ out) {
+__device__ __forceinline__ void true_residual_body(int m, const double *y, const double *Ny, const double *ritz,
+              double *out) {
     __shared__ double scratch[33];
     const double th = ritz[0];
     double rr = 0.0, rq = 0.0;
@@ -352,8 +351,8 @@
 }
 
 template <bool kShared, int kStage = 0>
-__device__ __forceinline__ void two_means_1d_body(int m, int P, const double *__restrict__ y, const double *__restrict__ isd, double *__restrict__ u,
-             double *__restrict__ sorted_g, int32_t *__restrict__ side, double *__restrict__ result) {
+__device__ __forceinline__ void two_means_1d_body(int m, int P, const double *y, const double *isd, double *u,
+             double *sorted_g, int32_t *side, double *result) {
     extern __shared__ double sort_s[];
     __shared__ double scratch[33];
     __shared__ double best_score[32];
diff --git a/spectralclustersupertree_b200/engine.py b/spectralclustersupertree_b200/engine.py
--- a/spectralclustersupertree_b200/engine.py
+++ b/spectralclustersupertree_b200/engine.py
@@ -98,6 +98,9 @@
 
     def set_full_rows(self, on: bool) -> None:
         _check(self._lib.scs_ctx_set_full_rows(self._ctx, int(on)), self._ctx)
+
+    def set_medium_wide_min(self, n: int) -> None:
+        _check(self._lib.scs_ctx_set_medium_wide_min(self._ctx, int(n)), self._ctx)
 
     def stage_seconds(self, reset: bool = True) -> dict:
         out = np.zeros(8)
```

Measured after the change: 0.06754, median of 6. +10.1%, slower.
